# projecthorus/radiosonde_auto_rx

Measured on AMD Instinct MI355X. Metric: IQ Msamples/s (RS41 --IQ --lpIQ demod + framesync + ECC), concurrent real-time 2.4 Msps channels = value/2.4, higher is better.
Workload: dtype f32; 1 GPU; RS41 2.4 Msps cs16 IQ, rs41mod --ecc2 --IQ fq --lpIQ (BASELINE configs[1]) x 512 channels per GPU (per-GPU share of configs[4]), 1 s of signal per channel per step, input resident in HBM; channels_per_gpu=512, frames_decoded=507392, frames_ecc_ok=457842, frames_ecc_failed=49550, frames_repaired=200182, symbols_repaired=1815512

## Files before the change

### include/sonde_hip.h

```cpp
#ifndef SONDE_HIP_H
#define SONDE_HIP_H

#include <stdint.h>
#include <stddef.h>

#ifdef __cplusplus
extern "C" {
#endif

#define SONDE_ABI_VERSION 3

#define SONDE_E_ARG      (-1)
#define SONDE_E_NOGPU    (-2)
#define SONDE_E_NOMEM    (-3)
#define SONDE_E_RANGE    (-4)
#define SONDE_E_OVERFLOW (-5)

#define SONDE_RS41  41
#define SONDE_FRONTEND 0
#define SONDE_DFM09  9
#define SONDE_M10    10
#define SONDE_M20    20

#define SONDE_RD94RD41 94
#define SONDE_LMS6   6
#define SONDE_RS92   92
#define SONDE_IMET54 54
#define SONDE_MIXED  100
#define SONDE_GENERIC 99

#define SONDE_IN_IQ    0
#define SONDE_IN_AUDIO 1
#define SONDE_IN_IFIQ0 2
#define SONDE_IN_IFIQ2 3
#define SONDE_IN_IFIQ3 4

#define SONDE_LP_IQ 1
#define SONDE_LP_FM 2

#define SONDE_TAP_DECIM 0
#define SONDE_TAP_IFIQ  1
#define SONDE_TAP_FM    2
#define SONDE_TAP_BUFS  3
#define SONDE_TAP_CORR  4

typedef struct sonde_engine sonde_engine_t;

typedef struct {
    int32_t abi_version;
    int32_t device;
    int32_t n_channels;
    int32_t sample_rate;
    int32_t bits;
    int32_t sonde_type;
    int32_t opt_lp;
    int32_t opt_dc;
    int32_t opt_min;
    int32_t lpiq_bw;
    int32_t ecc_level;
    float   thres;
    int32_t max_chunk;
    int32_t max_frames;
    int32_t keep_soft;
    int32_t pipeline;
    int32_t input;
    int32_t audio_channels;
    int32_t audio_select;
    int32_t if_rate;
    int32_t opt_iqdc;
    int32_t opt_inv;
    int32_t opt_nolut;
    int32_t m10_noskip;
    int32_t opt_auto;
    int32_t if_tune;
} sonde_cfg_t;

typedef struct {
    int32_t  channel;
    int32_t  len;
    int32_t  ecc;
    uint32_t mv_pos;
    float    mv;
    int32_t  nbytes;
    uint8_t  frame[518];
    uint8_t  pad[2];
} sonde_frame_t;

typedef struct {
    int32_t  channel;
    int32_t  frame_in_hit;
    int32_t  ecc[3];
    uint32_t mv_pos;
    float    mv;
    uint8_t  conf[7], dat1[13], dat2[13];
    uint8_t  pad[3];
    float    frm_count;
    int32_t  inv;
    uint8_t  rawbits[35];
    uint8_t  pad2;
} sonde_dfm_frame_t;

typedef struct {
    int32_t if_sr, decM, dectaps, lut_len, lpiq_taps, lpfm_taps;
    int32_t L, M, K, N, delay;
    float   sps;
    int32_t ring_len;
    int32_t reserved[3];
} sonde_info_t;

int  sonde_engine_create(const sonde_cfg_t *cfg, const double *fq, sonde_engine_t **out);
typedef struct {
    char    header[68];
    float   baud, bt, h;
    int32_t symlen, symhd;
    int32_t hdmax, bitofs;
    int32_t nbits, skip_bits;
    float   l_win;
    int32_t lpiq_bw, lpfm_bw;
    float   slice_baud;
    int32_t reserved[3];
} sonde_generic_t;
int  sonde_engine_create_generic(const sonde_cfg_t *cfg, const double *fq, const sonde_generic_t *gen, sonde_engine_t **out);
typedef struct {
    int32_t sonde_type;
    int32_t ecc_level;
    int32_t lpiq_bw, opt_inv, opt_auto, m10_noskip;
    float   thres;
    int32_t reserved;
} sonde_group_t;
int  sonde_engine_create_mixed(const sonde_cfg_t *cfg, const double *fq, const sonde_group_t *groups, int32_t n_groups, const int32_t *group_of_channel, sonde_engine_t **out);
int  sonde_engine_group_info(const sonde_engine_t *e, int32_t channel, int32_t *sonde_type, sonde_info_t *info);
void sonde_engine_destroy(sonde_engine_t *e);
int  sonde_engine_info(const sonde_engine_t *e, sonde_info_t *info);

int  sonde_engine_process_device(sonde_engine_t *e, const void *d_iq, int64_t ch_stride, int32_t n_samples);
int  sonde_engine_process_host(sonde_engine_t *e, const void *h_iq, int64_t ch_stride, int32_t n_samples);
int64_t sonde_engine_samples_to_dc_boundary(const sonde_engine_t *e);
int  sonde_engine_sync(sonde_engine_t *e);

typedef struct {
    uint32_t channel_id;
    uint8_t  type;
    uint8_t  inverted;
    uint16_t reserved;
    float    score;
    float    freq_offset_hz;
    uint64_t sample_pos;
    uint32_t frames;
    uint32_t frames_clean;
} sonde_summary_t;
int  sonde_engine_set_summary(sonde_engine_t *e, void *d_summary, uint32_t channel_base);
int  sonde_engine_set_summary_snapshots(sonde_engine_t *e, void *d_snap);

int  sonde_engine_fetch_frames(sonde_engine_t *e, sonde_frame_t *out, int32_t max);
int  sonde_engine_overflowed(sonde_engine_t *e);
long long sonde_engine_host_ecc_frames(sonde_engine_t *e);
int  sonde_engine_set_device_ecc(sonde_engine_t *e, int32_t on);
int  sonde_engine_set_search_rounds(sonde_engine_t *e, int32_t on);
int  sonde_engine_count_windows(sonde_engine_t *e, int32_t on, int64_t *out);
int  sonde_engine_tail_residency(sonde_engine_t *e, int32_t *out);
int  sonde_engine_read_sync_state(sonde_engine_t *e, uint32_t *out, int32_t max_channels);
int  sonde_engine_fetch_frames_lagged(sonde_engine_t *e, sonde_frame_t *out, int32_t max, int32_t lag);

typedef struct {
    int32_t  channel;
    int32_t  nbits;
    uint32_t mv_pos;
    float    mv;
} sonde_hit_t;
int  sonde_engine_fetch_hits(sonde_engine_t *e, sonde_hit_t *out, int32_t max, int32_t finish);
int  sonde_engine_set_sync(sonde_engine_t *e, int32_t hdmax, int32_t bitofs);
int  sonde_engine_fetch_soft1(sonde_engine_t *e, float *soft, int32_t max_frames);
int  sonde_engine_set_threshold(sonde_engine_t *e, float thres);

int  sonde_engine_fetch_dfm(sonde_engine_t *e, sonde_dfm_frame_t *out, int32_t max, int32_t finish);
int  sonde_engine_fetch_dfm_lagged(sonde_engine_t *e, sonde_dfm_frame_t *out, int32_t max, int32_t lag);
typedef struct {
    int32_t  channel;
    int32_t  nbits;
    int32_t  len;
    int32_t  cs_ok;
    uint32_t cs_calc;
    uint32_t mv_pos;
    float    mv;
    uint8_t  frame[124];
} sonde_m10_frame_t;
int  sonde_engine_fetch_m10(sonde_engine_t *e, sonde_m10_frame_t *out, int32_t max, int32_t finish);
int  sonde_engine_fetch_m10_lagged(sonde_engine_t *e, sonde_m10_frame_t *out, int32_t max, int32_t lag);
int  sonde_engine_set_m10_chk3(sonde_engine_t *e, int32_t on);
#define SONDE_M10_COLOR 0x100
int  sonde_m10_rawline(const sonde_m10_frame_t *f, int verbose, char *buf, size_t buflen);

typedef struct {
    int32_t  channel;
    int32_t  nbits;
    int32_t  len;
    int32_t  cs_ok;
    uint32_t cs_calc;
    int32_t  blk_ok;
    int32_t  fw;
    uint32_t mv_pos;
    float    mv;
    uint8_t  frame[172];
} sonde_m20_frame_t;
int  sonde_engine_fetch_m20(sonde_engine_t *e, sonde_m20_frame_t *out, int32_t max, int32_t finish);
int  sonde_m10_frame_finish(sonde_m10_frame_t *f);
int  sonde_m20_frame_finish(sonde_m20_frame_t *f);
#define SONDE_M20_COLOR 0x100
int  sonde_m20_rawline(const sonde_m20_frame_t *f, int verbose, char *buf, size_t buflen);

int  sonde_dfm_rawline(const sonde_dfm_frame_t *f, int ecc_level, char *buf, size_t buflen);

int  sonde_engine_finish(sonde_engine_t *e, sonde_frame_t *out, int32_t max);
int  sonde_engine_finish_channel(sonde_engine_t *e, int32_t channel);
int  sonde_engine_tune_channel(sonde_engine_t *e, int32_t channel, double fq);
int  sonde_engine_restart_channel(sonde_engine_t *e, int32_t channel);
int  sonde_engine_fetch_soft(sonde_engine_t *e, float *soft, int32_t max_frames);

int  sonde_engine_read_tap(sonde_engine_t *e, int32_t channel, int32_t tap, int64_t first, int32_t count, float *out);

void *sonde_engine_stream(sonde_engine_t *e);
int  sonde_engine_profile(sonde_engine_t *e, int enable);
int  sonde_engine_kernel_ms(sonde_engine_t *e, const char *kernel, double *avg_ms, int64_t *launches);

typedef struct sonde_softin sonde_softin_t;
int  sonde_softin_create(int32_t sonde_type, int32_t ecc_level, int32_t invert_stream, int32_t opt_inv, int32_t opt_auto, sonde_softin_t **out);
void sonde_softin_destroy(sonde_softin_t *s);
int  sonde_softin_push(sonde_softin_t *s, const float *soft, int32_t n);
int  sonde_softin_push_bits(sonde_softin_t *s, const uint8_t *bits, int32_t n);
int  sonde_softin_push_frame(sonde_softin_t *s, const uint8_t *bytes, int32_t len, int32_t xorhex);
int  sonde_softin_push_hexline(sonde_softin_t *s, const char *line, int32_t xorhex);
int  sonde_softin_finish(sonde_softin_t *s);
int  sonde_softin_fetch(sonde_softin_t *s, sonde_frame_t *out, int32_t max);
int  sonde_softin_fetch_soft(sonde_softin_t *s, float *soft, int32_t *nbits, int32_t *inv, int32_t max);
int  sonde_softin_fetch_dfm(sonde_softin_t *s, sonde_dfm_frame_t *out, int32_t max);
int  sonde_softin_push_dfm_rawhex(sonde_softin_t *s, const char *text, int32_t n);
int  sonde_softin_fetch_m10(sonde_softin_t *s, sonde_m10_frame_t *out, int32_t max);
int  sonde_softin_fetch_m20(sonde_softin_t *s, sonde_m20_frame_t *out, int32_t max);
int  sonde_softin_set_m10_skip(sonde_softin_t *s, int32_t skip);

int  sonde_rs41_rawline(const sonde_frame_t *f, char *buf, size_t buflen);

int  sonde_rs255_encode(uint8_t cw[255]);
int  sonde_rs255_decode(uint8_t cw[255]);
int  sonde_rs41_ecc_device(uint8_t *frames, const int32_t *flen, int32_t n, int32_t level, int32_t *ecc, int32_t *codes, uint8_t *synd);
int  sonde_crc16(const uint8_t *data, int len);

int  sonde_probe_read_gbps(const void *d_buf, size_t bytes, int32_t reps, double *gbps);

const char *sonde_strerror(int code);

#ifdef __cplusplus
}
#endif
#endif
```

### radiosonde_auto_rx_amd/csrc/sonde_dev.h

```cpp
#ifndef SONDE_DEV_H
#define SONDE_DEV_H
#include <hip/hip_runtime.h>
#include <stdint.h>
#include "../../include/sonde_hip.h"

struct MixDecArgs {
    const int16_t *iq;
    long long ch_stride;
    int n_ch, nblocks;
    int D, Q;
    int G;
    int wgs_per_ch;
    float wtab[64 * 8];
    const double *chan_f0;
    int lut_len;
    uint32_t lut_phase;
    const float2 *dc_avg;
    long long *dc_sums;
    const float2 *ptail_in;
    float2 *ptail_out;
    float2 *y;
    int ring_len;
    uint32_t m0;
    const float *wtab_g;
    int wtab_scaled;
    int DS;
    int phase_f64;
    double nd_base;
    const float2 *etab; int etab_len;
    const float2 *dc_avg_prev;
    int dc_since;
    const uint32_t *epoch_phase;
    const int32_t *dc_since_ch;
    const float2 *dc_seg; int dc_seg_n, dc_seg_off, dc_seg_blocks;
    int2 *bsum; long long bsum_stride;
    const int32_t *in_row;
};
struct ScanEdgeArgs {
    int n_ch, nblocks, D, Q, nseg;
    const float2 *dc_seg; int dc_seg_n, dc_seg_off, dc_seg_blocks;
    const float2 *dc_prev;
    int etab_len; uint32_t e0;
    const double *chan_f0; const float *wtab;
    float2 *corr;
};
extern "C" int  sonde_launch_mix_decimate50r(const MixDecArgs *a, hipStream_t s);
extern "C" void sonde_launch_dc_rows_to_segments(const int2 *bsum, long long bsum_stride, int n_ch, int nblocks, int seg_off, int seg_blocks, float maxcnt,
                                                 long long *seg_sums, long long *dc_sums, float2 *dc_avg, const float2 *dc_prev, float2 *dc_prev_out, float2 *dc_seg, int dc_seg_n, hipStream_t s);
extern "C" void sonde_launch_scan_dc_edges(const ScanEdgeArgs *a, hipStream_t s);
extern "C" void sonde_launch_md_etable64(const double *chan_f0, const float *wtab, int D, int Q, int P, int n_ch, float2 *etab, hipStream_t s);
extern "C" void sonde_launch_dc_segments(const int16_t *iq, long long ch_stride, int n_ch, int n_samples, unsigned dc_cnt0, unsigned dc_max,
                                         long long *seg_sums, long long *dc_sums, float2 *dc_avg, float2 *dc_seg, int dc_seg_n, hipStream_t s);

struct AfcState {
    double Df;
    double dc;
    int locked;
    uint32_t pad;
};

struct MixF32Args {
    const float2 *x; long long ch_stride; int n_ch, n;
    const double *chan_f0; int lut_len; uint32_t lut_phase; int phase_f64; double nd_base;
    const float2 *dc_avg; double *dc_sums;
    float2 *z; uint32_t zmask; uint64_t n0;
    int mix;
    const uint32_t *epoch;
    const float2 *dc_seg; int dc_seg_n; uint32_t dc_seg_off, dc_seg_len;
};
struct DecF32Args {
    const float2 *z; uint32_t zmask; uint64_t n0;
    const float *taps; int T, D, n_ch, nblocks;
    float2 *y; int ring_len; uint32_t m0;
};

struct AfcRotArgs {
    const float2 *y; float2 *yrot; const AfcState *afc; const uint32_t *start;
    int n_ch, ring_len, sr; uint32_t m_end;
};

struct IfArgs {
    const float2 *y; float2 *tap_ifiq; float *fm; float *bufs;
    const AfcState *afc; const uint32_t *start; float *fmraw; const float *w_iq0;
    int n_ch, ring_len, n; uint32_t m0;
    int lpiq_on, lpiq_taps, lpfm_on, lpfm_taps, tone_on, nwin;
    int fm_on;
    const float *w_iq, *w_fm;
    double rho;
    float sps;
    const uint32_t *epoch;
};

struct AudioChainArgs {
    const float *raw; float *fm, *bufs; const float *w;
    int n_ch, ring_len, n, taps; uint32_t m0;
};

struct SyncState {
    uint32_t s_in, k, mv_pos, mode;
    float mv; uint32_t inv;
    uint32_t pad[2];
};

struct WinItem {
    uint32_t pos;
    int32_t  state;
    int32_t  rc;
    float    mv; uint32_t mpos;
    uint32_t pad[3];
};
struct WinPlanArgs {
    const SyncState *state; WinItem *items;
    int n_ch, stride, W, K, L, delay; uint32_t frame_samples, avail;
    const uint32_t *epoch;
    uint32_t *work, *work_count; int round_parity;
};
struct WinFftArgs {
    const float *bufs; WinItem *items; const float2 *Fm, *tws;
    int n_ch, stride, W, K, L, ring_len;
    const uint32_t *work, *work_count; int round_parity;
    unsigned long long *prof;
};

struct CorrArgs {
    const float *bufs; float *corr; const float *match;
    const SyncState *state;
    const uint32_t *start;
    int delay; uint32_t frame_samples;
    uint32_t limit;
    int n_ch, ring_len, n, L; uint32_t m0;
    int ntypes, isps, nsym;
    const float *shapes;
    const int *sym_type;
    const float *sym_sign;
};

struct FrameRec {
    int32_t channel, len, nbytes; uint32_t mv_pos; float mv;
    int32_t ecc, ecc_done;
    uint8_t synd[48];
    uint8_t frame[520];
};

struct SyncArgs {
    const float *bufs, *corr; SyncState *state; FrameRec *frames; unsigned *frame_count; float *soft;
    float *soft1;
    const uint8_t *hdr, *hdr_bytes, *mask, *gf_exp, *gf_log;
    const uint4 *bitwin;
    const uint32_t *bitend;
    int n_ch, ring_len, max_frames; uint32_t avail;
    int K, L, delay, hdrlen, symhd, symlen, hdmax, bitofs, nbits; uint32_t frame_samples;
    float sps, thres, l_win;
    int rs41;
    int ecc_level;
    uint32_t *ecc_list; unsigned *ecc_count;
    int eof;
    int eof_ch;
    const uint32_t *epoch;
    int opt_auto;
    int opt_dc, opt_iq, lpiq_on, lpfm_taps, N, sr;
    float match_sum;
    const float *fm, *corr2; float2 *ifiq;
    AfcState *afc; uint32_t *start; unsigned *pending;
    sonde_summary_t *summary; uint32_t summary_base; int summary_type; uint64_t summary_epoch;
    const int32_t *summary_map;
    const WinItem *win; int win_W;
    uint32_t corr_limit;
    unsigned long long *prof;
};

struct SearchSyncArgs {
    SyncArgs sync;
    WinFftArgs win;
    unsigned long long *wcount;
};

#define SONDE_MAX_GROUPS 6
extern "C" {
int  sonde_launch_if_chain_multi(const IfArgs *a, int n_groups, hipStream_t s);
int  sonde_launch_sync_plan_multi(const WinPlanArgs *a, int n_groups, hipStream_t s);
int  sonde_launch_sync_window_fft_multi(const WinFftArgs *a, int n_groups, hipStream_t s);
int  sonde_launch_framesync_multi(const SyncArgs *a, int n_groups, hipStream_t s);
int  sonde_launch_mix_decimate(const MixDecArgs *a, hipStream_t s);
void sonde_launch_dc_update(int n_ch, long long *sums, float2 *avg, float maxcnt, hipStream_t s);
void sonde_launch_dc_update_keep(int n_ch, long long *sums, float2 *avg, float2 *avg_prev, float maxcnt, hipStream_t s);
void sonde_launch_publish_u32(const unsigned *src, unsigned *dst_mapped, hipStream_t s);
void sonde_launch_dc_update_pcs(int n_ch, long long *sums, float2 *avg, float2 *avg_prev, uint32_t *cnt, uint32_t *max, uint32_t lim, int32_t *since,
                                uint32_t n_samples, int nblocks, hipStream_t s);
void sonde_launch_md_etable(const double *chan_f0, const float *wtab, int D, int Q, int P, int n_ch, float2 *etab, hipStream_t s);
void sonde_launch_if_chain(const IfArgs *a, hipStream_t s);
void sonde_launch_mix_f32(const MixF32Args *a, hipStream_t s);
void sonde_launch_dc_segments_f32(const float2 *x, long long ch_stride, int n_ch, int n_samples, unsigned dc_cnt0, unsigned dc_max,
                                  double *seg_sums, double *dc_sums, float2 *dc_avg, float2 *dc_seg, int dc_seg_n, hipStream_t s);
void sonde_launch_decimate_f32(const DecF32Args *a, hipStream_t s);
void sonde_launch_dc_update_f64(int n_ch, double *sums, float2 *avg, float maxcnt, hipStream_t s);
void sonde_launch_afc_rotate(const AfcRotArgs *a, hipStream_t s, int n_max);
void sonde_launch_fill_u32(uint32_t *p, uint32_t v, int n, hipStream_t s);
void sonde_launch_audio_chain(const AudioChainArgs *a, hipStream_t s);
void sonde_launch_u8_to_s16(const uint8_t *in, long long in_stride, int16_t *out, long long out_stride, int n_ch, int n_bytes, hipStream_t s);
void sonde_launch_header_corr(const CorrArgs *a, hipStream_t s);
void sonde_launch_sync_plan(const WinPlanArgs *a, hipStream_t s);
void sonde_launch_sync_window_fft(const WinFftArgs *a, hipStream_t s);
void sonde_launch_framesync(const SyncArgs *a, hipStream_t s);
void sonde_launch_search_sync(const SearchSyncArgs *a, hipStream_t s);
int  sonde_if_chain_residency(const IfArgs *a);
int  sonde_search_sync_residency(void);
size_t sonde_if_chain_lds_bytes(int T1, int T2, int nwin, int tone_on, int fm_on, int *overlay);
int  sonde_if_chain_reserve(const IfArgs *a, int device);
}
#endif
```

### radiosonde_auto_rx_amd/csrc/sonde_engine.cpp

```cpp
#include "../../include/sonde_hip.h"
#include "sonde_dev.h"
#include "sonde_host.h"
#include "sonde_scan_dev.h"
#include <algorithm>
#include <cmath>
#include <cstdio>
#include <cstring>
#include <map>
#include <string>
#include <vector>

using namespace sonde;

#define HIPCHK(x) do { hipError_t e_ = (x); if (e_ != hipSuccess) { fprintf(stderr, "libsonde_hip: %s failed: %s\n", #x, hipGetErrorString(e_)); return SONDE_E_NOGPU; } } while (0)

struct KernelStat { double ms = 0; int64_t n = 0; };
struct PendingEvt { hipEvent_t a, b; const char *name; };

struct sonde_engine {
    sonde_cfg_t cfg{};
    sonde_info_t info{};
    hipStream_t stream = nullptr;
    hipStream_t stream_b = nullptr;
    unsigned long long *d_wfprof = nullptr;
    hipStream_t stream_c = nullptr;
    hipStream_t stream_e = nullptr;
    hipEvent_t ev_s = nullptr;
    sonde_dfm_frame_t *d_dfm_out = nullptr; sonde_m10_frame_t *d_m10_out = nullptr; unsigned *d_blk_done = nullptr; char *d_m10_bits = nullptr;
    std::vector<sonde_dfm_frame_t> h_dfm; std::vector<sonde_m10_frame_t> h_m10; bool soft_lazy = false; unsigned soft_lazy_start = 0;
    uint32_t *d_ecc_list = nullptr; unsigned *d_ecc_cnt = nullptr;
    hipEvent_t ev_a[4] = {}, ev_b[4] = {}, ev_if[4] = {};
    unsigned *h_count = nullptr;
    unsigned *h_count_dev = nullptr;
    FrameRec *h_recs = nullptr;
    int64_t call = 0;
    unsigned read_idx = 0;
    bool eof_pending = false;
    Decimator dec; int Q = 0, G = 8, DS = 0; float *d_wtab = nullptr;
    float2 *d_etab = nullptr, *d_dcavg_prev = nullptr; int etab_len = 0; int dc_since = 1 << 20;
    std::vector<float> w_iq, w_fm, match, wtab;
    float sps = 0, sps_design = 0, baud = 0, bt = 0, hmod = 0, thres = 0, l_win = -1;
    int symlen = 1, symhd = 1, hdmax = 0, bitofs = 0, nbits = 0, hdrlen = 0;
    uint32_t frame_samples = 0;
    double rho = 0;
    float *d_Bop = nullptr; double *d_chanf0 = nullptr; int lut_len = 0;
    float2 *d_dcavg = nullptr; long long *d_dcsums = nullptr;
    float2 *d_ptail[2] = { nullptr, nullptr }; int ptail_cur = 0;
    float2 *d_y = nullptr, *d_ifiq = nullptr; float *d_fm = nullptr, *d_bufs = nullptr, *d_corr = nullptr, *d_raw = nullptr;
    float *d_wiq = nullptr, *d_wfm = nullptr, *d_match = nullptr;
    uint32_t corr_limit = 0;
    WinItem *d_win = nullptr; float2 *d_Fm = nullptr, *d_tws = nullptr; int win_W = 0;
    uint32_t *d_work = nullptr, *d_work_count = nullptr; int sync_rounds = 0;
    bool search_rounds = false;
    bool count_windows = false; unsigned long long *d_wcount = nullptr; long long wcount_rounds[2] = { 0, 0 };
    sonde_summary_t *d_summary = nullptr; uint32_t summary_base = 0;
    sonde_summary_t *d_summary_snap = nullptr;
    int corr_types = 0, corr_isps = 0; float *d_shapes = nullptr, *d_symsign = nullptr; int *d_symtype = nullptr;
    SyncState *d_state = nullptr; FrameRec *d_frames = nullptr; unsigned *d_fcount = nullptr; float *d_soft = nullptr, *d_soft1 = nullptr;
    uint4 *d_bitwin = nullptr; uint32_t *d_bitend = nullptr;
    uint8_t *d_consts = nullptr;
    int16_t *d_stage = nullptr; size_t stage_bytes = 0;
    bool ifiq = false;
    int opt_iq = 5; float match_sum = 0.f;
    std::vector<float> w_iq0; float *d_wiq0 = nullptr;
    float2 *d_yrot = nullptr; float *d_fmraw = nullptr, *d_corr2 = nullptr;
    AfcState *d_afc = nullptr; uint32_t *d_start = nullptr; unsigned *d_pending = nullptr, *h_pending = nullptr;
    double *d_dcsums_f = nullptr; float2 *d_zring = nullptr; float *d_taps_f = nullptr; uint32_t zmask = 0;
    hipEvent_t ev_copy = nullptr;
    int16_t *d_conv = nullptr;
    float2 *d_conv32 = nullptr; bool f32_path = false, conv32 = false;
    int ring_len = 0, max_frames = 0;
    uint64_t samples_in = 0;
    uint32_t m_out = 0;
    uint32_t dc_cnt = 0, dc_max = 0, dc_lim = 0;
    bool pcs = false; std::vector<uint32_t> pcs_cnt, pcs_max; uint32_t dc_max0 = 0;
    uint32_t *d_epoch_phase = nullptr, *d_pcs_cnt = nullptr, *d_pcs_max = nullptr; int32_t *d_pcs_since = nullptr;
    std::vector<float> last_soft, last_soft1; int last_n = 0;
    std::vector<uint8_t> last_frame;
    std::vector<char> m10_bits;
    bool overflow = false;
    bool in_call = false, ecc_listed = false;
    bool dev_ecc = true;
    long long host_ecc_frames = 0;
    bool m10_chk3 = false;
    std::vector<uint32_t> epoch; uint32_t *d_epoch = nullptr; int eof_ch = -1;
    bool prof = false, prof_skip = false; int prof_level = 2; std::map<std::string, KernelStat> stats; std::vector<PendingEvt> pend;
    std::vector<sonde_engine *> groups; std::vector<int32_t> grp_of_ch, row_of_ch; std::vector<std::vector<int32_t>> ch_of_grp; int32_t *d_in_row = nullptr;
    bool front_only = false; int64_t snap_calls = 0;
    sonde_engine *front = nullptr; int front_row = 0; int32_t *d_sum_map = nullptr; bool is_group = false;
    bool merged = false, borrowed_b = false;
};
struct CreateLink { bool is_group, front_only; int min_ring; hipStream_t shared_b; };

template <class T> static int dalloc(T **p, size_t n, bool zero = true) {
    HIPCHK(hipMalloc((void **)p, n * sizeof(T)));
    if (zero) HIPCHK(hipMemset(*p, 0, n * sizeof(T)));
    return 0;
}

static void prof_begin(sonde_engine *e, const char *name, hipStream_t s) {
    if (!e->prof || (e->prof_level == 1 && strcmp(name, "mix_decimate") != 0)) { e->prof_skip = true; return; }
    e->prof_skip = false;
    PendingEvt p; p.name = name;
    hipEventCreate(&p.a); hipEventCreate(&p.b);
    hipEventRecord(p.a, s);
    e->pend.push_back(p);
}
static void prof_end(sonde_engine *e, hipStream_t s) { if (e->prof && !e->prof_skip) hipEventRecord(e->pend.back().b, s); }
static void prof_collect(sonde_engine *e) {
    for (auto &p : e->pend) {
        float ms = 0; hipEventSynchronize(p.b); hipEventElapsedTime(&ms, p.a, p.b);
        auto &s = e->stats[p.name]; s.ms += ms; s.n += 1;
        hipEventDestroy(p.a); hipEventDestroy(p.b);
    }
    e->pend.clear();
}

static int collect_records(sonde_engine *e, int lag, std::vector<FrameRec> &recs, std::vector<float> *soft, int max_take) {
    unsigned count = 0;
    if (lag > 0) {
        const int64_t target = e->call - 1 - lag;
        if (target < 0) { recs.clear(); if (soft) soft->clear(); return 0; }
        if (hipEventSynchronize(e->ev_b[target & 3]) != hipSuccess) return SONDE_E_NOGPU;
        count = e->h_count[target & 3];
    } else {
        if (hipStreamSynchronize(e->stream_b) != hipSuccess) return SONDE_E_NOGPU;
        if (e->stream_e && hipStreamSynchronize(e->stream_e) != hipSuccess) return SONDE_E_NOGPU;
        if (e->call > 0 && !e->eof_pending) count = e->h_count[(e->call - 1) & 3];
        else if (hipMemcpy(&count, e->d_fcount, sizeof count, hipMemcpyDeviceToHost) != hipSuccess) return SONDE_E_NOGPU;
        e->eof_pending = false;
        prof_collect(e);
    }
    if ((int32_t)(count - e->read_idx) < 0) count = e->read_idx;
    hipStream_t cs = (lag > 0 && e->stream_c) ? e->stream_c : e->stream_b;
    unsigned n = count - e->read_idx;
    if (n > (unsigned)e->max_frames) { e->overflow = true; e->read_idx = count - (unsigned)e->max_frames; n = (unsigned)e->max_frames; }
    if (max_take >= 0 && n > (unsigned)max_take) n = (unsigned)max_take;
    recs.resize(n);
    if (soft) soft->resize((size_t)n * e->nbits);
    unsigned done = 0;
    while (done < n) {
        const unsigned idx = (e->read_idx + done) % (unsigned)e->max_frames;
        const unsigned run = std::min<unsigned>(n - done, (unsigned)e->max_frames - idx);
        if (hipMemcpyAsync(e->h_recs + done, e->d_frames + idx, (size_t)run * sizeof(FrameRec), hipMemcpyDeviceToHost, cs) != hipSuccess) return SONDE_E_NOGPU;
        if (soft && e->d_soft && hipMemcpyAsync(soft->data() + (size_t)done * e->nbits, e->d_soft + (size_t)idx * e->nbits,
                                                (size_t)run * e->nbits * sizeof(float), hipMemcpyDeviceToHost, cs) != hipSuccess) return SONDE_E_NOGPU;
        done += run;
    }
    if (n && hipStreamSynchronize(cs) != hipSuccess) return SONDE_E_NOGPU;
    if (n) memcpy(recs.data(), e->h_recs, (size_t)n * sizeof(FrameRec));
    e->read_idx += n;
    return (int)n;
}

static void launch_framesync_impl(sonde_engine *e, int eof);
static SyncArgs fill_sync(sonde_engine *e, int eof);
static void fill_round(sonde_engine *e, int W, WinPlanArgs &p, WinFftArgs &f);
static inline uint32_t rel_pos(const sonde_engine *e, const FrameRec &r) { return e->epoch.empty() ? r.mv_pos : r.mv_pos - e->epoch[r.channel]; }
extern "C" void sonde_launch_dfm_hits(const FrameRec *frames, const float *soft, int nbits, int max_frames, const unsigned *fcount, unsigned *done, sonde_dfm_frame_t *out,
                                      int ecc_level, int grid, hipStream_t s);
extern "C" void sonde_launch_m10_hits(const FrameRec *frames, const float *soft, const float *soft1, int chk3, int nbits, int max_frames, const unsigned *fcount, unsigned *done,
                                      char *chan_bits, sonde_m10_frame_t *out, int grid, hipStream_t s);
static bool blockcodes_on_device(const sonde_engine *e);
static void launch_blockcodes(sonde_engine *e) {
    if (!blockcodes_on_device(e)) return;
    const int grid = std::max(1, std::min(e->cfg.n_channels, 1024));
    if (e->cfg.sonde_type == SONDE_DFM09)
        sonde_launch_dfm_hits(e->d_frames, e->d_soft, e->nbits, e->max_frames, e->d_fcount, e->d_blk_done, e->d_dfm_out, e->cfg.ecc_level, grid, e->stream_b);
    else
        sonde_launch_m10_hits(e->d_frames, e->d_soft, e->d_soft1, e->m10_chk3 ? 1 : 0, e->nbits, e->max_frames, e->d_fcount, e->d_blk_done, e->d_m10_bits, e->d_m10_out, grid, e->stream_b);
}
static void launch_framesync(sonde_engine *e, int eof) { launch_framesync_impl(e, eof); launch_blockcodes(e); if (eof) e->eof_pending = true; }
static void sync_round(sonde_engine *e, int W);
static void launch_search_sync(sonde_engine *e);

static bool blockcodes_on_device(const sonde_engine *e) {
    return e->dev_ecc && e->d_soft && e->d_blk_done && ((e->cfg.sonde_type == SONDE_DFM09 && e->d_dfm_out) || (e->cfg.sonde_type == SONDE_M10 && e->d_m10_out));
}
template <class T> static int copy_decoded(sonde_engine *e, const T *d_out, std::vector<T> &h, unsigned start, int n, int per, int lag = 0) {
    h.resize((size_t)n * per);
    hipStream_t cs = (lag > 0 && e->stream_c) ? e->stream_c : e->stream_b;
    unsigned done = 0;
    while (done < (unsigned)n) {
        const unsigned idx = (start + done) % (unsigned)e->max_frames;
        const unsigned run = std::min<unsigned>((unsigned)n - done, (unsigned)e->max_frames - idx);
        if (hipMemcpyAsync(h.data() + (size_t)done * per, d_out + (size_t)idx * per, (size_t)run * per * sizeof(T), hipMemcpyDeviceToHost, cs) != hipSuccess) return SONDE_E_NOGPU;
        done += run;
    }
    if (n && hipStreamSynchronize(cs) != hipSuccess) return SONDE_E_NOGPU;
    return 0;
}

template <class F, class FN> static int mixed_fetch(sonde_engine *e, int type, F *out, int32_t max, int lag, FN fn) {
    if (!e || !out || max < 0) return SONDE_E_ARG;
    if (lag > 0 && e->snap_calls > 0) {
        const int64_t target = e->call - 1 - lag;
        if (target >= 0 && target < e->snap_calls && hipEventSynchronize(e->ev_b[target & 3]) != hipSuccess) return SONDE_E_NOGPU;
    }
    int n = 0;
    for (size_t gi = 0; gi < e->groups.size(); gi++) {
        sonde_engine *g = e->groups[gi];
        if (g->cfg.sonde_type != type) continue;
        const int k = fn(g, out + n, max - n);
        if (k < 0) return k;
        for (int i = 0; i < k; i++) out[n + i].channel = e->ch_of_grp[gi][(size_t)out[n + i].channel];
        n += k;
    }
    return n;
}

extern "C" {

const char *sonde_strerror(int code) {
    switch (code) {
        case 0: return "ok";
        case SONDE_E_ARG: return "bad argument or unsupported option";
        case SONDE_E_NOGPU: return "HIP device/runtime error";
        case SONDE_E_NOMEM: return "out of memory";
        case SONDE_E_RANGE: return "chunk size out of range or not a multiple of the decimation";
        case SONDE_E_OVERFLOW: return "frame queue overflow";
        default: return "unknown error";
    }
}

extern "C" void sonde_launch_rs41_ecc_frames(FrameRec *frames, const uint32_t *list, unsigned *count, unsigned *done, int max_frames, int level,
                                             const uint8_t *gf_exp, const uint8_t *gf_log, int grid, hipStream_t s);
extern "C" void sonde_launch_rs41_ecc_batch(uint8_t *frames, const int32_t *flen, int n, int level, int32_t *ecc, int32_t *codes, uint8_t *synd,
                                            const uint8_t *gf_exp, const uint8_t *gf_log, hipStream_t s);

int sonde_rs41_ecc_device(uint8_t *frames, const int32_t *flen, int32_t n, int32_t level, int32_t *ecc, int32_t *codes, uint8_t *synd) {
    if (!frames || !flen || !ecc || n < 0 || level < 1 || level > 2) return SONDE_E_ARG;
    if (n == 0) return 0;
    for (int i = 0; i < n; i++) if (flen[i] < 0 || flen[i] > 518) return SONDE_E_ARG;
    uint8_t *d_fr = nullptr, *d_syn = nullptr, *d_gf = nullptr; int32_t *d_len = nullptr, *d_ecc = nullptr, *d_codes = nullptr;
    int rc = 0;
    auto ok = [&](hipError_t e) { if (e != hipSuccess && rc == 0) { fprintf(stderr, "libsonde_hip: sonde_rs41_ecc_device: %s\n", hipGetErrorString(e)); rc = SONDE_E_NOGPU; } return rc == 0; };
    if (ok(hipMalloc((void **)&d_fr, (size_t)n * 518)) && ok(hipMalloc((void **)&d_syn, (size_t)n * 48)) && ok(hipMalloc((void **)&d_gf, 768))
        && ok(hipMalloc((void **)&d_len, (size_t)n * 4)) && ok(hipMalloc((void **)&d_ecc, (size_t)n * 4)) && ok(hipMalloc((void **)&d_codes, (size_t)n * 8))
        && ok(hipMemcpy(d_fr, frames, (size_t)n * 518, hipMemcpyHostToDevice)) && ok(hipMemcpy(d_len, flen, (size_t)n * 4, hipMemcpyHostToDevice))
        && ok(hipMemcpy(d_gf, gf_exp_table(), 512, hipMemcpyHostToDevice)) && ok(hipMemcpy(d_gf + 512, gf_log_table(), 256, hipMemcpyHostToDevice))) {
        sonde_launch_rs41_ecc_batch(d_fr, d_len, n, level, d_ecc, d_codes, d_syn, d_gf, d_gf + 512, nullptr);
        ok(hipGetLastError());
        ok(hipMemcpy(frames, d_fr, (size_t)n * 518, hipMemcpyDeviceToHost));
        ok(hipMemcpy(ecc, d_ecc, (size_t)n * 4, hipMemcpyDeviceToHost));
        if (codes) ok(hipMemcpy(codes, d_codes, (size_t)n * 8, hipMemcpyDeviceToHost));
        if (synd) ok(hipMemcpy(synd, d_syn, (size_t)n * 48, hipMemcpyDeviceToHost));
    }
    hipFree(d_fr); hipFree(d_syn); hipFree(d_gf); hipFree(d_len); hipFree(d_ecc); hipFree(d_codes);
    return rc;
}

int sonde_engine_create(const sonde_cfg_t *cfg, const double *fq, sonde_engine_t **out) { return sonde_engine_create_generic(cfg, fq, nullptr, out); }

static int create_impl(const sonde_cfg_t *cfg, const double *fq, const sonde_generic_t *gen, const CreateLink *lk, sonde_engine_t **out);
static int fetch_dfm_impl(sonde_engine_t *e, sonde_dfm_frame_t *out, int32_t max, int32_t finish, int lag);
static int fetch_m10_impl(sonde_engine_t *e, sonde_m10_frame_t *out, int32_t max, int32_t finish, int lag);
int sonde_engine_create_generic(const sonde_cfg_t *cfg, const double *fq, const sonde_generic_t *gen, sonde_engine_t **out) { return create_impl(cfg, fq, gen, nullptr, out); }

}

static IfArgs fill_if(sonde_engine *e, int n_if, uint32_t m_first);
static int create_impl(const sonde_cfg_t *cfg, const double *fq, const sonde_generic_t *gen, const CreateLink *lk, sonde_engine_t **out) {
    if (!cfg || !fq || !out || cfg->abi_version != SONDE_ABI_VERSION) return SONDE_E_ARG;
    if (cfg->sonde_type == SONDE_GENERIC && !gen) return SONDE_E_ARG;
    float baud_override = 0.f;
    if (gen && cfg->sonde_type != SONDE_GENERIC) { if (!(gen->baud > 0.f)) return SONDE_E_ARG; baud_override = gen->baud; gen = nullptr; }
    if (gen) {
        const size_t hl = strnlen(gen->header, sizeof gen->header);
        if (hl < 8 || hl > 64 || !(gen->baud > 0.f) || !(gen->bt > 0.f) || !(gen->h > 0.f) || gen->symlen < 1 || gen->symlen > 2 || gen->symhd < 1 || gen->symhd > gen->symlen ||
            hl % gen->symhd || gen->hdmax < 0 || gen->bitofs < -8 || gen->bitofs > 64 || gen->nbits < 1 || gen->nbits > 8192 || gen->skip_bits < 0 || gen->slice_baud < 0.f) return SONDE_E_ARG;
    }
    if (cfg->n_channels < 1 || cfg->sample_rate < 1 || (cfg->bits != 16 && cfg->bits != 8 && cfg->bits != 32)) return SONDE_E_ARG;
    sonde_cfg_t cfg_own = *cfg;
    if (cfg->input == SONDE_IN_IQ && cfg->opt_dc && cfg->sonde_type != SONDE_FRONTEND) cfg_own.opt_lp |= SONDE_LP_FM;
    cfg = &cfg_own;
    if ((cfg->sonde_type != SONDE_RS41 && cfg->sonde_type != SONDE_DFM09 && cfg->sonde_type != SONDE_M10 && cfg->sonde_type != SONDE_M20 && cfg->sonde_type != SONDE_FRONTEND && cfg->sonde_type != SONDE_GENERIC) ) return SONDE_E_ARG;
    if (cfg->opt_dc && cfg->sonde_type == SONDE_FRONTEND) return SONDE_E_ARG;
    if (cfg->opt_nolut && (cfg->opt_dc || cfg->input != SONDE_IN_IQ)) return SONDE_E_ARG;
    if (cfg->if_tune && (cfg->input < SONDE_IN_IFIQ0 || cfg->bits != 32 || cfg->opt_dc)) return SONDE_E_ARG;
    if (cfg->sonde_type == SONDE_FRONTEND && cfg->input != SONDE_IN_IQ) return SONDE_E_ARG;
    if (cfg->input < SONDE_IN_IQ || cfg->input > SONDE_IN_IFIQ3) return SONDE_E_ARG;
    int ndev = 0;
    if (hipGetDeviceCount(&ndev) != hipSuccess || ndev < 1 || cfg->device >= ndev) {
        fprintf(stderr, "libsonde_hip: no usable HIP device (the engine has no CPU fallback)\n");
        return SONDE_E_NOGPU;
    }
    HIPCHK(hipSetDevice(cfg->device));
    sonde_engine *e = new sonde_engine();
    e->cfg = *cfg;
    const int C = cfg->n_channels;
    const bool is_group = lk && lk->is_group, front_only = lk && lk->front_only;
    e->is_group = is_group; e->front_only = front_only;

    std::string header;
    int lpiq_def, lpfm_bw;
    int skip_last = -1;
    if (gen) {
        e->baud = gen->baud; e->bt = gen->bt; e->hmod = gen->h; e->symlen = gen->symlen; e->symhd = gen->symhd; e->hdmax = gen->hdmax; e->bitofs = gen->bitofs;
        e->nbits = gen->nbits; e->l_win = gen->l_win > 0.f ? gen->l_win : -1.0f; e->thres = cfg->thres > 0 ? cfg->thres : 0.7f;
        header = std::string(gen->header, strnlen(gen->header, sizeof gen->header)); lpiq_def = gen->lpiq_bw; lpfm_bw = gen->lpfm_bw;
        if (gen->skip_bits > gen->nbits) skip_last = gen->skip_bits - 1;
    } else if (cfg->sonde_type == SONDE_RS41 || cfg->sonde_type == SONDE_FRONTEND) {
        e->baud = 4800.f; e->bt = 0.5f; e->hmod = 0.6f; e->symlen = 1; e->symhd = 1; e->hdmax = 4; e->bitofs = 2;
        e->nbits = 510 * 8; e->l_win = 2.0f; e->thres = cfg->thres > 0 ? cfg->thres : 0.7f;
        header = kRs41Header; lpiq_def = 7400; lpfm_bw = 6000;
    } else if (cfg->sonde_type == SONDE_M10) {
        e->baud = 9615.f; e->bt = 1.8f; e->hmod = 0.9f; e->symlen = 2; e->symhd = 1; e->hdmax = 2; e->bitofs = 0;
        e->nbits = (101 + 20) * 8; e->l_win = 4.0f; e->thres = cfg->thres > 0 ? cfg->thres : 0.76f;
        header = kM10RawHeader; lpiq_def = 24000; lpfm_bw = 10000;
    } else if (cfg->sonde_type == SONDE_M20) {
        e->baud = 9600.f; e->bt = 1.8f; e->hmod = 0.9f; e->symlen = 2; e->symhd = 1; e->hdmax = 2; e->bitofs = 0;
        e->nbits = (101 + 64) * 8; e->l_win = 4.0f; e->thres = cfg->thres > 0 ? cfg->thres : 0.76f;
        header = kM10RawHeader; lpiq_def = 24000; lpfm_bw = 10000;
    } else {
        e->baud = 2500.f; e->bt = 0.5f; e->hmod = 1.8f; e->symlen = 2; e->symhd = 2; e->hdmax = 2; e->bitofs = 2;
        e->nbits = 264 + 7 * 280; e->l_win = 4.0f; e->thres = cfg->thres > 0 ? cfg->thres : 0.65f;
        header = kDfmRawHeader; lpiq_def = 12000; lpfm_bw = 4000;
    }
    if (baud_override > 0.f) e->baud = baud_override;
    e->hdrlen = (int)header.size();
    const int lpiq_bw = cfg->lpiq_bw > 0 ? cfg->lpiq_bw : lpiq_def;

    const bool audio = cfg->input == SONDE_IN_AUDIO;
    const bool ifiq = cfg->input >= SONDE_IN_IFIQ0;
    if (audio) { e->dec.if_sr = cfg->sample_rate; e->dec.decM = 1; e->l_win = -1.0f; }
    else if (ifiq) { e->dec.if_sr = cfg->sample_rate; e->dec.decM = 1; if (cfg->input != SONDE_IN_IFIQ3) e->l_win = -1.0f; }
    else if (cfg->sonde_type == SONDE_FRONTEND) e->dec = design_decimator_if(cfg->sample_rate, cfg->if_rate > 0 ? cfg->if_rate : 48000, cfg->opt_min != 0);
    else e->dec = design_decimator(cfg->sample_rate, cfg->opt_min != 0);
    const int D = e->dec.decM, sr = e->dec.if_sr;
    if (D == 1) e->dec.taps.assign(1, 1.0f);
    const int T = (int)e->dec.taps.size();
    e->sps = (float)cfg->sample_rate / e->baud;
    e->sps /= (float)D;
    e->Q = (T + D - 1) / D;
    const bool wide = e->Q > 8;
    if (D > 1024 || (wide && (audio || ifiq || lk || cfg->input != SONDE_IN_IQ))) { delete e; return SONDE_E_ARG; }
    e->f32_path = cfg->bits == 32 || wide; e->conv32 = wide && cfg->bits != 32;
    if ((cfg->opt_lp & SONDE_LP_IQ) && !audio) {
        float f_lp = (float)(24e3 / (float)sr / 2.0);
        if (lpiq_bw) f_lp = (float)(lpiq_bw / (float)sr / 2.0);
        int taps = (int)(4 * sr / 4e3); if (taps % 2 == 0) taps++;
        e->w_iq = design_lowpass(f_lp, taps);
        if (cfg->opt_dc) e->w_iq0 = design_lowpass((float)(1.5 * f_lp), taps);
    }
    if (cfg->opt_lp & SONDE_LP_FM) {
        float f_lp = (float)(10e3 / (float)sr);
        if (lpfm_bw > 0) f_lp = lpfm_bw / (float)sr;
        int taps = (int)(4 * sr / 2e3); if (taps % 2 == 0) taps++;
        e->w_fm = design_lowpass(f_lp, taps);
    }
    e->match = design_match(header, e->sps, e->bt);
    const int L = (int)e->match.size();
    int M = 3 * L, p2 = 1;
    const int delay = L / 16;
    while (p2 < M) p2 <<= 1;
    while (p2 < 0x2000) p2 <<= 1;
    M = p2;
    const int K = M - L - delay;
    { const float nh = -e->hmod; const float hs = nh * sr; const double f1 = hs / (2.0 * e->sps); e->rho = -f1 / (double)sr; }
    e->sps_design = e->sps;
    if (gen && gen->slice_baud > 0.f) {
        e->sps = (float)sr / gen->slice_baud;
    }
    {
        const int last = skip_last >= 0 ? skip_last : ((cfg->sonde_type == SONDE_M10 || cfg->sonde_type == SONDE_M20) && !cfg->m10_noskip) ? 5 * 808 - 1 : e->nbits - 1;
        uint32_t q0, q1; double mid; bit_window(last, e->symlen - 1, e->symlen, e->sps, q0, q1, mid); e->frame_samples = q1;
    }

    if (!audio && !front_only) {
        const IfArgs ia = fill_if(e, 0, 0);
        const int rc = sonde_if_chain_reserve(&ia, cfg->device);
        if (rc) { delete e; return rc == -1 ? SONDE_E_ARG : SONDE_E_NOGPU; }
    }

    const int max_if = (cfg->max_chunk + D - 1) / D;
    int ring = 1; while (ring < max_if + (int)e->frame_samples + 2 * M + 4096 || ring < 4 * M || (cfg->pipeline && ring < 2 * max_if + 4096)) ring <<= 1;
    if (lk && ring < lk->min_ring) ring = lk->min_ring;
    e->ring_len = ring;
    e->max_frames = cfg->max_frames > 0 ? cfg->max_frames : 4 * C;

    sonde_info_t &I = e->info;
    I.if_sr = sr; I.decM = D; I.dectaps = (D == 1) ? 0 : T; I.lpiq_taps = (int)e->w_iq.size(); I.lpfm_taps = (int)e->w_fm.size();
    I.L = L; I.M = M; I.K = K; I.N = M; I.delay = delay; I.sps = e->sps_design; I.ring_len = ring;

    if (wide) e->wtab.assign((size_t)std::max(64, D) * 8, 0.f);
    else {
        const int pad = e->Q * D - T;
        std::vector<float> wpad((size_t)e->Q * D, 0.f);
        for (int k = 0; k < T; k++) wpad[pad + k] = e->dec.taps[k];
        e->wtab.assign((size_t)std::max(64, D) * 8, 0.f);
        for (int r = 0; r < D; r++) for (int q = 0; q < e->Q; q++) e->wtab[(size_t)r * 8 + q] = wpad[(size_t)D * q + r];
        if (D > 64) {
            for (int k = 64; k >= 4; k--) if (D % k == 0) { e->DS = k; break; }
            if (!e->DS || e->Q < 5) { delete e; return SONDE_E_ARG; }
        }
        {
            std::vector<float> both(e->wtab);
            if (D <= 64) for (size_t i = 0; i < e->wtab.size(); i++) both.push_back(e->wtab[i] * 3.0517578125e-05f);
            if (dalloc(&e->d_wtab, both.size(), false)) { delete e; return SONDE_E_NOMEM; }
            HIPCHK(hipMemcpy(e->d_wtab, both.data(), both.size() * sizeof(float), hipMemcpyHostToDevice));
        }
    }
    {
        std::vector<double> f0s(C);
        for (int c = 0; c < C; c++) {
            const Mixer m = design_mixer(-std::max(-0.5, std::min(0.5, fq[c])), cfg->sample_rate);
            f0s[c] = m.f0; e->lut_len = m.lut_len;
            if (cfg->opt_nolut || cfg->if_tune) f0s[c] = -std::max(-0.5, std::min(0.5, fq[c]));
        }
        I.lut_len = e->lut_len;
        if (dalloc(&e->d_chanf0, (size_t)C, false)) { delete e; return SONDE_E_NOMEM; }
        HIPCHK(hipMemcpy(e->d_chanf0, f0s.data(), f0s.size() * sizeof(double), hipMemcpyHostToDevice));
    }
    if (D == 50 && e->Q == 7 && !audio && cfg->bits != 32 && cfg->sonde_type != SONDE_FRONTEND && !cfg->opt_nolut && e->lut_len % D == 0
        && cfg->input == SONDE_IN_IQ && !is_group) {
        e->etab_len = e->lut_len / D;
        if (dalloc(&e->d_etab, (size_t)C * e->etab_len, false) || dalloc(&e->d_dcavg_prev, C)) { sonde_engine_destroy(e); return SONDE_E_NOMEM; }
        sonde_launch_md_etable(e->d_chanf0, e->d_wtab, D, e->Q, e->etab_len, C, e->d_etab, nullptr);
        HIPCHK(hipDeviceSynchronize());
    }
    int bad = 0;
    bad |= dalloc(&e->d_dcavg, C); bad |= dalloc(&e->d_dcsums, 2 * (size_t)C);
    bad |= dalloc(&e->d_ptail[0], (size_t)C * 64); bad |= dalloc(&e->d_ptail[1], (size_t)C * 64);
    if (audio) bad |= dalloc(&e->d_raw, (size_t)C * ring);
    else { if (!is_group) bad |= dalloc(&e->d_y, (size_t)C * ring); if (!front_only) bad |= dalloc(&e->d_ifiq, (size_t)C * ring); }
    if (!front_only) { bad |= dalloc(&e->d_fm, (size_t)C * ring); bad |= dalloc(&e->d_bufs, (size_t)C * ring); bad |= dalloc(&e->d_corr, (size_t)C * ring); }
    bad |= dalloc(&e->d_state, C); bad |= dalloc(&e->d_frames, e->max_frames); bad |= dalloc(&e->d_fcount, 1 + 4);
    if (cfg->keep_soft || cfg->sonde_type != SONDE_RS41) bad |= dalloc(&e->d_soft, (size_t)e->max_frames * e->nbits);
    if (cfg->keep_soft == 2) bad |= dalloc(&e->d_soft1, (size_t)e->max_frames * e->nbits);
    if (cfg->sonde_type == SONDE_DFM09) { bad |= dalloc(&e->d_dfm_out, (size_t)e->max_frames * 8); bad |= dalloc(&e->d_blk_done, 2); }
    if (cfg->sonde_type == SONDE_M10) { bad |= dalloc(&e->d_m10_out, (size_t)e->max_frames); bad |= dalloc(&e->d_blk_done, 2); bad |= dalloc(&e->d_m10_bits, (size_t)C * ((101 + 20) * 8 + 8)); }
    bad |= dalloc(&e->d_match, L, false);
    if (!e->w_iq.empty()) bad |= dalloc(&e->d_wiq, e->w_iq.size(), false);
    if (!e->w_fm.empty()) bad |= dalloc(&e->d_wfm, e->w_fm.size(), false);
    bad |= dalloc(&e->d_consts, 1024, true);
    if (bad) { sonde_engine_destroy(e); return SONDE_E_NOMEM; }
    HIPCHK(hipMemcpy(e->d_match, e->match.data(), L * sizeof(float), hipMemcpyHostToDevice));
    e->dev_ecc = getenv("SONDE_HOST_ECC") == nullptr;
    {
        if (!cfg->opt_dc && M == 8192 && K + L <= M) {
            std::vector<float> m(2 * (size_t)M, 0.f);
            for (int i = 0; i < L; i++) m[2 * (size_t)(L - 1 - i)] = e->match[i];
            ref_dft_8192(m);
            const std::vector<float> tw = ref_twiddle_table();
            e->win_W = 8;
            m.resize(4 * (size_t)M);
            for (int i = 0; i < M; i++) {
                int r = 0; for (int b = 0; b < 13; b++) if (i >> b & 1) r |= 1 << (12 - b);
                m[2 * (size_t)(M + i)] = m[2 * (size_t)r]; m[2 * (size_t)(M + i) + 1] = m[2 * (size_t)r + 1];
            }
            if (dalloc(&e->d_Fm, 2 * (size_t)M, false) || dalloc(&e->d_tws, tw.size() / 2, false) || dalloc(&e->d_win, (size_t)C * e->win_W) ||
                dalloc(&e->d_work, (size_t)C * e->win_W) || dalloc(&e->d_work_count, 2)) { sonde_engine_destroy(e); return SONDE_E_NOMEM; }
            HIPCHK(hipMemcpy(e->d_Fm, m.data(), m.size() * sizeof(float), hipMemcpyHostToDevice));
            HIPCHK(hipMemcpy(e->d_tws, tw.data(), tw.size() * sizeof(float), hipMemcpyHostToDevice));
        }
    }
    if (e->d_wiq) HIPCHK(hipMemcpy(e->d_wiq, e->w_iq.data(), e->w_iq.size() * sizeof(float), hipMemcpyHostToDevice));
    if (e->d_wfm) HIPCHK(hipMemcpy(e->d_wfm, e->w_fm.data(), e->w_fm.size() * sizeof(float), hipMemcpyHostToDevice));
    {
        uint8_t cb[1024]; memset(cb, 0, sizeof cb);
        memcpy(cb, header.data(), header.size()); memcpy(cb + 64, kRs41HeaderBytes, 8); memcpy(cb + 72, kRs41Mask, 64);
        memcpy(cb + 136, gf_exp_table(), 512); memcpy(cb + 648, gf_log_table(), 256);
        HIPCHK(hipMemcpy(e->d_consts, cb, sizeof cb, hipMemcpyHostToDevice));
    }
    {
        const int isps = (int)e->sps_design, nsym = e->hdrlen / e->symhd;
        if ((float)isps == e->sps_design && e->symhd == 1 && isps * nsym == L && isps >= 2 && isps <= 16 && isps % 2 == 0) {
            std::vector<float> shapes; std::vector<int> type(nsym); std::vector<float> sign(nsym);
            std::vector<int> key;
            bool ok = true;
            for (int k = 0; k < nsym && ok; k++) {
                const int b = (header[k] & 1) ? 1 : -1;
                const int l = (k > 0) ? ((header[k - 1] & 1) ? 1 : -1) * b : 0;
                const int r = (k < nsym - 1) ? ((header[k + 1] & 1) ? 1 : -1) * b : 0;
                const int ky = (l + 1) * 3 + (r + 1);
                int t = -1;
                for (size_t q = 0; q < key.size(); q++) if (key[q] == ky) t = (int)q;
                if (t < 0) {
                    t = (int)key.size(); key.push_back(ky);
                    for (int d = 0; d < isps; d++) shapes.push_back((float)b * e->match[(size_t)isps * k + d]);
                } else {
                    for (int d = 0; d < isps; d++) ok &= (shapes[(size_t)t * isps + d] == (float)b * e->match[(size_t)isps * k + d]);
                }
                type[k] = t; sign[k] = (float)b;
            }
            if (ok && key.size() <= 9) {
                e->corr_types = (int)key.size(); e->corr_isps = isps;
                bad = 0;
                bad |= dalloc(&e->d_shapes, shapes.size(), false); bad |= dalloc(&e->d_symtype, nsym, false); bad |= dalloc(&e->d_symsign, nsym, false);
                if (bad) { sonde_engine_destroy(e); return SONDE_E_NOMEM; }
                HIPCHK(hipMemcpy(e->d_shapes, shapes.data(), shapes.size() * sizeof(float), hipMemcpyHostToDevice));
                HIPCHK(hipMemcpy(e->d_symtype, type.data(), nsym * sizeof(int), hipMemcpyHostToDevice));
                HIPCHK(hipMemcpy(e->d_symsign, sign.data(), nsym * sizeof(float), hipMemcpyHostToDevice));
            }
        }
    }
    {
        std::vector<uint32_t> win((size_t)e->nbits * 4), end(e->nbits);
        for (int bp = 0; bp < e->nbits; bp++) {
            uint32_t q0, q1, qa, qb; double mid;
            if (e->symlen == 2) { bit_window(bp, 0, 2, e->sps, q0, q1, mid); slice_range(q0, q1, mid, e->l_win, qa, qb); }
            else { qa = qb = 0; }
            win[4 * bp] = qa; win[4 * bp + 1] = qb;
            bit_window(bp, e->symlen - 1, e->symlen, e->sps, q0, q1, mid);
            slice_range(q0, q1, mid, e->l_win, qa, qb);
            win[4 * bp + 2] = qa; win[4 * bp + 3] = qb; end[bp] = q1;
        }
        bad = 0;
        bad |= dalloc(&e->d_bitwin, (size_t)e->nbits, false); bad |= dalloc(&e->d_bitend, (size_t)e->nbits, false);
        if (bad) { sonde_engine_destroy(e); return SONDE_E_NOMEM; }
        HIPCHK(hipMemcpy(e->d_bitwin, win.data(), win.size() * sizeof(uint32_t), hipMemcpyHostToDevice));
        HIPCHK(hipMemcpy(e->d_bitend, end.data(), end.size() * sizeof(uint32_t), hipMemcpyHostToDevice));
    }
    e->dc_lim = (uint32_t)sr; e->dc_max = e->dc_lim / 32;
    if (D > 1) { e->dc_lim *= D; e->dc_max *= D; }
    if (e->dc_max == 0 || e->dc_max % D) { sonde_engine_destroy(e); return SONDE_E_ARG; }
    e->dc_max0 = e->dc_max;
    e->ifiq = ifiq;
    if (e->f32_path) {
        bad = dalloc(&e->d_dcsums_f, 2 * (size_t)C);
        if (e->conv32) bad |= dalloc(&e->d_conv32, (size_t)C * (size_t)cfg->max_chunk, false);
        if (!audio && !ifiq) {
            uint32_t zl = 1; while (zl < (uint32_t)cfg->max_chunk + (uint32_t)T + (uint32_t)D + 64u) zl <<= 1;
            e->zmask = zl - 1;
            bad |= dalloc(&e->d_zring, (size_t)C * zl); bad |= dalloc(&e->d_taps_f, (size_t)T, false);
            if (!bad) HIPCHK(hipMemcpy(e->d_taps_f, e->dec.taps.data(), (size_t)T * sizeof(float), hipMemcpyHostToDevice));
        }
        if (bad) { sonde_engine_destroy(e); return SONDE_E_NOMEM; }
    }
    if (cfg->opt_inv) {
        std::vector<SyncState> st0(C); for (auto &q : st0) { memset(&q, 0, sizeof q); q.inv = 1; }
        HIPCHK(hipMemcpy(e->d_state, st0.data(), st0.size() * sizeof(SyncState), hipMemcpyHostToDevice));
    }
    e->opt_iq = audio ? 0 : ifiq ? (cfg->input == SONDE_IN_IFIQ0 ? 1 : cfg->input == SONDE_IN_IFIQ2 ? 2 : 3) : 5;
    { double sm = 0.0; for (float v : e->match) sm += (double)v; e->match_sum = (float)sm; }
    if (cfg->opt_dc) {
        bad = 0;
        bad |= dalloc(&e->d_afc, C); bad |= dalloc(&e->d_start, C); bad |= dalloc(&e->d_pending, 1);
        if (!audio) { bad |= dalloc(&e->d_yrot, (size_t)C * ring); bad |= dalloc(&e->d_fmraw, (size_t)C * ring); }
        if (e->opt_iq >= 2) bad |= dalloc(&e->d_corr2, (size_t)C * ring);
        if (!e->w_iq0.empty()) bad |= dalloc(&e->d_wiq0, e->w_iq0.size(), false);
        if (bad) { sonde_engine_destroy(e); return SONDE_E_NOMEM; }
        if (e->d_wiq0) HIPCHK(hipMemcpy(e->d_wiq0, e->w_iq0.data(), e->w_iq0.size() * sizeof(float), hipMemcpyHostToDevice));
        HIPCHK(hipHostMalloc((void **)&e->h_pending, sizeof(unsigned), hipHostMallocDefault));
    }
    e->last_frame.assign((size_t)C * 518, 0);
    for (int c = 0; c < C; c++) memcpy(e->last_frame.data() + (size_t)c * 518, kRs41HeaderBytes, 8);
    HIPCHK(hipStreamCreateWithFlags(&e->stream, hipStreamNonBlocking));
    if (cfg->pipeline && audio) { sonde_engine_destroy(e); return SONDE_E_ARG; }
    if (lk && lk->shared_b) { e->stream_b = lk->shared_b; e->borrowed_b = is_group; }
    else if (cfg->pipeline) {
        int lo = 0, hi = 0;
        if (hipDeviceGetStreamPriorityRange(&lo, &hi) == hipSuccess && hi != lo)
            HIPCHK(hipStreamCreateWithPriority(&e->stream_b, hipStreamNonBlocking, hi));
        else HIPCHK(hipStreamCreateWithFlags(&e->stream_b, hipStreamNonBlocking));
    }
    else e->stream_b = e->stream;
    HIPCHK(hipStreamCreateWithFlags(&e->stream_c, hipStreamNonBlocking));
    if (cfg->sonde_type == SONDE_RS41 && cfg->ecc_level >= 1 && cfg->ecc_level <= 2 && getenv("SONDE_ECC_INLINE") == nullptr) {
        int lo = 0, hi = 0;
        if (hipDeviceGetStreamPriorityRange(&lo, &hi) == hipSuccess && hi != lo) HIPCHK(hipStreamCreateWithPriority(&e->stream_e, hipStreamNonBlocking, hi));
        else HIPCHK(hipStreamCreateWithFlags(&e->stream_e, hipStreamNonBlocking));
    }
    HIPCHK(hipEventCreateWithFlags(&e->ev_s, hipEventDisableTiming));
    if (cfg->sonde_type == SONDE_RS41) {
        HIPCHK(hipMalloc((void **)&e->d_ecc_list, 2 * (size_t)e->max_frames * sizeof(uint32_t)));
        HIPCHK(hipMalloc((void **)&e->d_ecc_cnt, 4 * sizeof(unsigned)));
        HIPCHK(hipMemset(e->d_ecc_cnt, 0, 4 * sizeof(unsigned)));
    }
    for (int i = 0; i < 4; i++) { HIPCHK(hipEventCreateWithFlags(&e->ev_a[i], hipEventDisableTiming)); HIPCHK(hipEventCreateWithFlags(&e->ev_b[i], hipEventDisableTiming)); HIPCHK(hipEventCreateWithFlags(&e->ev_if[i], hipEventDisableTiming)); }
    HIPCHK(hipEventCreateWithFlags(&e->ev_copy, hipEventDisableTiming));
    HIPCHK(hipHostMalloc((void **)&e->h_count, 4 * sizeof(unsigned), hipHostMallocMapped));
    memset(e->h_count, 0, 4 * sizeof(unsigned));
    HIPCHK(hipHostGetDevicePointer((void **)&e->h_count_dev, e->h_count, 0));
    HIPCHK(hipHostMalloc((void **)&e->h_recs, (size_t)e->max_frames * sizeof(FrameRec), hipHostMallocDefault));
    *out = e;
    return 0;
}

extern "C" {

void sonde_engine_destroy(sonde_engine_t *e) {
    if (!e) return;
    for (sonde_engine *g : e->groups) sonde_engine_destroy(g);
    e->groups.clear();
    if (e->is_group) e->d_y = nullptr;
    if (e->stream) hipStreamSynchronize(e->stream);
    if (e->stream_b) hipStreamSynchronize(e->stream_b);
    if (e->stream_e) hipStreamSynchronize(e->stream_e);
    prof_collect(e);
    if (e->d_wfprof) {
        unsigned long long h[32] = {0};
        if (hipMemcpy(h, e->d_wfprof, sizeof h, hipMemcpyDeviceToHost) == hipSuccess && h[31]) {
            static const char *nm[7] = {"setup", "search", "headcmp", "slot", "slice", "syndromes+record", "exit"};
            unsigned long long tot = 0; for (int i = 0; i < 7; i++) tot += h[16 + i];
            fprintf(stderr, "framesync prof (channel 0, %llu launches, %llu frames, %.0f cycles per launch):", h[31], h[30], (double)tot / (double)h[31]);
            for (int i = 0; i < 7; i++) fprintf(stderr, " %s %.1f%%", nm[i], 100.0 * (double)h[16 + i] / (double)std::max(1ull, tot));
            fprintf(stderr, "\n");
        }
        if (h[15]) {
            static const char *nm[6] = {"load", "fft1", "mul", "fft2", "argmax", "norm"};
            unsigned long long tot = 0; for (int i = 0; i < 6; i++) tot += h[i];
            fprintf(stderr, "window fft prof (workgroup 0, %llu windows, %.0f cycles each):", h[15], (double)tot / (double)h[15]);
            for (int i = 0; i < 6; i++) fprintf(stderr, " %s %.1f%%", nm[i], 100.0 * (double)h[i] / (double)std::max(1ull, tot));
            fprintf(stderr, "\n");
        }
        hipFree(e->d_wfprof);
    }
    { hipStream_t sa = e->stream; if (sa) hipStreamDestroy(sa); }
    if (e->stream_b && e->stream_b != e->stream && !e->borrowed_b) hipStreamDestroy(e->stream_b);
    if (e->stream_c) hipStreamDestroy(e->stream_c);
    if (e->stream_e) hipStreamDestroy(e->stream_e);
    if (e->ev_s) hipEventDestroy(e->ev_s);
    hipFree(e->d_dfm_out); hipFree(e->d_m10_out); hipFree(e->d_blk_done); hipFree(e->d_m10_bits);
    hipFree(e->d_ecc_list); hipFree(e->d_ecc_cnt);
    for (int i = 0; i < 4; i++) { if (e->ev_a[i]) hipEventDestroy(e->ev_a[i]); if (e->ev_b[i]) hipEventDestroy(e->ev_b[i]); if (e->ev_if[i]) hipEventDestroy(e->ev_if[i]); }
    if (e->ev_copy) hipEventDestroy(e->ev_copy);
    if (e->h_pending) hipHostFree(e->h_pending);
    if (e->h_count) hipHostFree(e->h_count);
    if (e->h_recs) hipHostFree(e->h_recs);
    void *ptrs[] = { e->d_Bop, e->d_chanf0, e->d_dcavg, e->d_dcsums, e->d_ptail[0], e->d_ptail[1], e->d_y, e->d_ifiq, e->d_fm,
                     e->d_bufs, e->d_corr, e->d_wiq, e->d_wfm, e->d_match, e->d_state, e->d_frames, e->d_fcount, e->d_soft, e->d_soft1,
                     e->d_epoch, e->d_work, e->d_work_count, e->d_consts, e->d_stage, e->d_shapes, e->d_symtype, e->d_symsign, e->d_bitwin, e->d_bitend, e->d_raw, e->d_wtab, e->d_conv, e->d_conv32,
                     e->d_dcsums_f, e->d_zring, e->d_taps_f, e->d_wiq0, e->d_yrot, e->d_fmraw, e->d_corr2, e->d_afc, e->d_start, e->d_pending,
                     e->d_etab, e->d_dcavg_prev, e->d_win, e->d_Fm, e->d_tws, e->d_epoch_phase, e->d_pcs_cnt, e->d_pcs_max, e->d_pcs_since, e->d_in_row, e->d_sum_map, e->d_wcount };
    for (void *p : ptrs) if (p) hipFree(p);
    delete e;
}

int sonde_engine_info(const sonde_engine_t *e, sonde_info_t *info) {
    if (!e || !info) return SONDE_E_ARG;
    *info = e->info;
    return 0;
}

static uint32_t pcs_room(const sonde_engine *e) {
    uint32_t r = 0xffffffffu;
    for (size_t c = 0; c < e->pcs_cnt.size(); c++) r = std::min(r, e->pcs_max[c] - e->pcs_cnt[c]);
    return r;
}
int64_t sonde_engine_samples_to_dc_boundary(const sonde_engine_t *e) {
    if (!e) return SONDE_E_ARG;
    return e->pcs ? (int64_t)pcs_room(e) : (int64_t)(e->dc_max - e->dc_cnt);
}

void *sonde_engine_stream(sonde_engine_t *e) { return e ? (void *)e->stream : nullptr; }

}

static void tail_begin(sonde_engine *t, hipStream_t fs) {
    t->in_call = true; t->ecc_listed = false;
    if (t->stream_e && t->call >= 2) hipStreamWaitEvent(t->stream_b, t->ev_b[(t->call - 2) & 3], 0);
    if (t->d_ecc_cnt) { hipMemsetAsync(t->d_ecc_cnt + (t->call & 1), 0, sizeof(unsigned), t->stream_b); hipMemsetAsync(t->d_ecc_cnt + 2 + (t->call & 1), 0, sizeof(unsigned), t->stream_b); }
    if (t->stream_b != fs && t->call >= 2) hipStreamWaitEvent(fs, t->ev_if[(t->call - 2) & 3], 0);
}
static int tail_enqueue(sonde_engine *e, int32_t n_samples, uint32_t m_first, hipStream_t fs, hipEvent_t front_done);
static int tail_enqueue_merged(sonde_engine *e, int32_t n_samples, uint32_t m_first);
static int tail_finish(sonde_engine *e);
static int sync_rounds_of(const sonde_engine *e, int n_if);
static IfArgs fill_if(sonde_engine *e, int n_if, uint32_t m_first);

extern "C" {

int sonde_engine_process_device(sonde_engine_t *e, const void *d_iq, int64_t ch_stride, int32_t n_samples) {
    if (!e || !d_iq || e->is_group) return SONDE_E_ARG;
    const int D = e->info.decM, C = e->cfg.n_channels;
    if (n_samples <= 0 || n_samples > e->cfg.max_chunk || n_samples % D || (ch_stride != 0 && ch_stride < n_samples)) return SONDE_E_RANGE;
    if (e->cfg.bits == 8) {
        const int epf = e->cfg.input == SONDE_IN_AUDIO ? std::max(1, e->cfg.audio_channels) : 2;
        if (!e->d_conv) HIPCHK(hipMalloc((void **)&e->d_conv, (size_t)C * e->cfg.max_chunk * epf * 2));
        sonde_launch_u8_to_s16((const uint8_t *)d_iq, ch_stride * epf, e->d_conv, (long long)n_samples * epf, ch_stride == 0 ? 1 : C, n_samples * epf, e->stream);
        d_iq = e->d_conv; if (ch_stride != 0) ch_stride = n_samples;
    }
    const uint32_t m_first = e->m_out;
    int done = 0;
    const bool mixed = !e->groups.empty();
    if (mixed) { for (sonde_engine *g : e->groups) tail_begin(g, e->stream); }
    else tail_begin(e, e->stream);
    if (e->cfg.input == SONDE_IN_AUDIO) {
        AudioConvArgs c0{}; c0.pcm = (const int16_t *)d_iq; c0.ch_stride = ch_stride; c0.n_ch = C; c0.n = n_samples;
        c0.nch = std::max(1, e->cfg.audio_channels); c0.sel = std::min(std::max(0, e->cfg.audio_select), c0.nch - 1);
        c0.fm = e->d_raw; c0.ring_len = e->ring_len; c0.m0 = e->m_out; c0.f32 = (e->cfg.bits == 32);
        sonde_launch_audio_convert(&c0, e->stream);
        AudioChainArgs c1{}; c1.raw = e->d_raw; c1.fm = e->d_fm; c1.bufs = e->d_bufs; c1.w = e->d_wfm; c1.n_ch = C; c1.ring_len = e->ring_len;
        c1.n = n_samples; c1.taps = (int)e->w_fm.size(); c1.m0 = e->m_out;
        prof_begin(e, "if_chain", e->stream); sonde_launch_audio_chain(&c1, e->stream); prof_end(e, e->stream);
        e->samples_in += (uint64_t)n_samples; e->m_out += (uint32_t)n_samples; done = n_samples;
    }
    if (e->conv32) {
        sonde_launch_s16_to_f32((const int16_t *)d_iq, ch_stride, e->d_conv32, (long long)n_samples, ch_stride == 0 ? 1 : C, n_samples, e->stream);
        d_iq = e->d_conv32; if (ch_stride != 0) ch_stride = n_samples;
    }
    while (done < n_samples && e->f32_path && e->cfg.input != SONDE_IN_AUDIO) {
        const bool dc = !e->ifiq || e->cfg.opt_iqdc != 0;
        const int take = dc ? (int)std::min<uint32_t>((uint32_t)(n_samples - done), e->dc_max - e->dc_cnt) : n_samples - done;
        MixF32Args a{}; a.x = (const float2 *)d_iq + (size_t)done; a.ch_stride = ch_stride; a.n_ch = C; a.n = take;
        a.chan_f0 = e->d_chanf0; a.lut_len = e->lut_len; a.lut_phase = (uint32_t)(e->samples_in % (uint64_t)e->lut_len);
        a.phase_f64 = (e->cfg.sonde_type == SONDE_FRONTEND); a.dc_avg = e->d_dcavg; a.dc_sums = e->d_dcsums_f;
        if (e->cfg.opt_nolut) { a.phase_f64 = 1; a.lut_len = 1 << 30; a.lut_phase = 0; a.nd_base = (double)e->samples_in; }
        if (e->ifiq) {
            a.mix = 0; a.z = e->d_y; a.zmask = (uint32_t)e->ring_len - 1; a.n0 = e->m_out;
            if (e->cfg.if_tune) {
                a.mix = 1; a.phase_f64 = 1; a.lut_len = 1 << 30; a.lut_phase = 0; a.nd_base = (double)e->samples_in; a.epoch = e->d_epoch;
            }
        }
        else { a.mix = 1; a.z = e->d_zring; a.zmask = e->zmask; a.n0 = e->samples_in; }
        prof_begin(e, "mix_decimate", e->stream);
        sonde_launch_mix_f32(&a, e->stream);
        if (!e->ifiq) {
            DecF32Args d{}; d.z = e->d_zring; d.zmask = e->zmask; d.n0 = e->samples_in; d.taps = e->d_taps_f; d.T = (int)e->dec.taps.size(); d.D = D;
            d.n_ch = C; d.nblocks = take / D; d.y = e->d_y; d.ring_len = e->ring_len; d.m0 = e->m_out;
            sonde_launch_decimate_f32(&d, e->stream);
        }
        prof_end(e, e->stream);
        e->samples_in += (uint64_t)take; e->m_out += (uint32_t)(take / D); done += take;
        if (dc) {
            e->dc_cnt += (uint32_t)take;
            if (e->dc_cnt == e->dc_max) {
                sonde_launch_dc_update_f64(C, e->d_dcsums_f, e->d_dcavg, (float)e->dc_max, e->stream);
                e->dc_cnt = 0;
                if (e->dc_max < e->dc_lim) e->dc_max *= 2;
            }
        }
    }
    while (done < n_samples && e->ifiq) {
        const bool dc = e->cfg.opt_iqdc != 0;
        const int take = dc ? (int)std::min<uint32_t>((uint32_t)(n_samples - done), e->dc_max - e->dc_cnt) : n_samples - done;
        IqConvArgs a{}; a.iq = (const int16_t *)d_iq + 2 * (size_t)done; a.ch_stride = ch_stride; a.n_ch = C; a.n = take;
        a.dc_avg = e->d_dcavg; a.dc_sums = e->d_dcsums; a.y = e->d_y; a.ring_len = e->ring_len; a.m0 = e->m_out;
        prof_begin(e, "iq_convert", e->stream); sonde_launch_iq_convert(&a, e->stream); prof_end(e, e->stream);
        e->samples_in += (uint64_t)take; e->m_out += (uint32_t)take; done += take;
        if (dc) {
            e->dc_cnt += (uint32_t)take;
            if (e->dc_cnt == e->dc_max) {
                sonde_launch_dc_update(C, e->d_dcsums, e->d_dcavg, (float)e->dc_max, e->stream);
                e->dc_cnt = 0;
                if (e->dc_max < e->dc_lim) e->dc_max *= 2;
            }
        }
    }
    while (done < n_samples) {
        const int take = (int)std::min<uint32_t>((uint32_t)(n_samples - done), e->pcs ? pcs_room(e) : e->dc_max - e->dc_cnt);
        MixDecArgs a{};
        a.iq = (const int16_t *)d_iq + 2 * (size_t)done; a.ch_stride = ch_stride; a.n_ch = C; a.nblocks = take / D;
        a.D = D; a.Q = e->Q; a.G = e->G;
        memcpy(a.wtab, e->wtab.data(), sizeof a.wtab); a.wtab_g = e->d_wtab; a.DS = e->DS; a.chan_f0 = e->d_chanf0; a.lut_len = e->lut_len;
        a.lut_phase = (uint32_t)(e->samples_in % (uint64_t)e->lut_len);
        a.dc_avg = e->d_dcavg; a.dc_sums = e->d_dcsums;
        a.ptail_in = e->d_ptail[e->ptail_cur]; a.ptail_out = e->d_ptail[e->ptail_cur ^ 1];
        a.y = e->d_y; a.ring_len = e->ring_len; a.m0 = e->m_out;
        a.phase_f64 = (e->cfg.sonde_type == SONDE_FRONTEND);
        if (e->cfg.opt_nolut) { a.phase_f64 = 1; a.lut_len = 1 << 30; a.lut_phase = 0; a.nd_base = (double)e->samples_in; }
        { long long tiles = (long long)C * ((a.nblocks + 63) / 64); int G = (int)(tiles / 12288); a.G = G < 1 ? 1 : (G > 16 ? 16 : G); }
        {
            const char *g = getenv("SONDE_MD_G"); const int gv = g ? atoi(g) : 0; if (gv >= 1 && gv <= 16) a.G = gv;
        }
        a.etab = e->d_etab; a.etab_len = e->etab_len; a.in_row = e->d_in_row;
        a.dc_avg_prev = (e->d_etab && e->dc_since < e->Q - 1) ? e->d_dcavg_prev : nullptr; a.dc_since = e->dc_since;
        if (e->dc_since < (1 << 20)) e->dc_since += take / D;
        if (e->pcs) { a.epoch_phase = e->d_epoch_phase; a.dc_since_ch = e->d_pcs_since; a.dc_avg_prev = e->d_etab ? e->d_dcavg_prev : nullptr; }
        prof_begin(e, "mix_decimate", e->stream); const int lrc = sonde_launch_mix_decimate(&a, e->stream); prof_end(e, e->stream);
        if (lrc < 0) { e->in_call = false; e->ecc_listed = false; for (sonde_engine *g : e->groups) { g->in_call = false; g->ecc_listed = false; } return lrc == -2 ? SONDE_E_NOGPU : SONDE_E_ARG; }
        e->ptail_cur ^= 1;
        e->samples_in += (uint64_t)take; e->m_out += (uint32_t)(take / D); e->dc_cnt += (uint32_t)take; done += take;
        if (e->pcs) {
            sonde_launch_dc_update_pcs(C, e->d_dcsums, e->d_dcavg, e->d_dcavg_prev, e->d_pcs_cnt, e->d_pcs_max, e->dc_lim, e->d_pcs_since, (uint32_t)take, take / D, e->stream);
            for (int c2 = 0; c2 < C; c2++) {
                e->pcs_cnt[c2] += (uint32_t)take;
                if (e->pcs_cnt[c2] >= e->pcs_max[c2]) { e->pcs_cnt[c2] = 0; if (e->pcs_max[c2] < e->dc_lim) e->pcs_max[c2] *= 2; }
            }
            e->dc_cnt = 0;
            continue;
        }
        if (e->dc_cnt == e->dc_max) {
            if (e->d_etab) e->dc_since = 0;
            sonde_launch_dc_update_keep(C, e->d_dcsums, e->d_dcavg, e->d_etab ? e->d_dcavg_prev : nullptr, (float)e->dc_max, e->stream);
            e->dc_cnt = 0;
            if (e->dc_max < e->dc_lim) e->dc_max *= 2;
        }
    }
    const int slot = (int)(e->call & 3);
    int rc = 0;
    if (mixed) {
        hipEventRecord(e->ev_a[slot], e->stream);
        for (sonde_engine *g : e->groups) { g->samples_in = e->samples_in; g->m_out = e->m_out; }
        if (e->merged) rc = tail_enqueue_merged(e, n_samples, m_first);
        else for (sonde_engine *g : e->groups) {
            const int r2 = tail_enqueue(g, n_samples, m_first, e->stream, e->ev_a[slot]);
            if (r2 && !rc) rc = r2;
        }
        if (e->d_summary && e->d_summary_snap) {
            for (sonde_engine *g : e->groups) hipStreamWaitEvent(e->stream_b, g->ev_b[slot], 0);
            hipMemcpyAsync(e->d_summary_snap + (size_t)(e->call & 1) * C, e->d_summary, (size_t)C * sizeof(sonde_summary_t), hipMemcpyDeviceToDevice, e->stream_b);
            hipEventRecord(e->ev_b[slot], e->stream_b);
            e->snap_calls = e->call + 1;
        }
        e->call += 1;
    } else {
        if (e->stream_b != e->stream) hipEventRecord(e->ev_a[slot], e->stream);
        rc = tail_enqueue(e, n_samples, m_first, e->stream, e->ev_a[slot]);
    }
    return rc;
}

}

static IfArgs fill_if(sonde_engine *e, int n_if, uint32_t m_first) {
    IfArgs b{};
    const bool fe = e->cfg.sonde_type == SONDE_FRONTEND;
    b.y = e->d_y; b.tap_ifiq = (e->cfg.keep_soft || fe) ? e->d_ifiq : nullptr; b.fm = e->d_fm; b.bufs = e->d_bufs; b.n_ch = e->cfg.n_channels; b.ring_len = e->ring_len;
    b.n = n_if; b.m0 = m_first;
    b.lpiq_on = !e->w_iq.empty(); b.lpiq_taps = (int)e->w_iq.size(); b.lpfm_on = !e->w_fm.empty(); b.lpfm_taps = (int)e->w_fm.size();
    b.tone_on = (e->cfg.input != SONDE_IN_IFIQ0); b.nwin = (int)e->sps;
    b.fm_on = (e->cfg.keep_soft || fe || !e->w_fm.empty() || !b.tone_on) ? 1 : 0;
    b.w_iq = e->d_wiq; b.w_fm = e->d_wfm; b.rho = e->rho; b.sps = e->sps; b.epoch = e->d_epoch;
    if (e->cfg.opt_dc && e->cfg.input != SONDE_IN_AUDIO) b.fm_on = 1;
    return b;
}
static int tail_enqueue(sonde_engine *e, int32_t n_samples, uint32_t m_first, hipStream_t fs, hipEvent_t front_done) {
    const int D = e->info.decM, C = e->cfg.n_channels;
    const int n_if = n_samples / D;
    const bool fe = e->cfg.sonde_type == SONDE_FRONTEND;
    IfArgs b = fill_if(e, n_if, m_first);
    const int slot = (int)(e->call & 3);
    if (e->stream_b != fs) hipStreamWaitEvent(e->stream_b, front_done, 0);
    CorrArgs c{};
    c.bufs = e->d_bufs; c.corr = e->d_corr; c.match = e->d_match; c.n_ch = C; c.ring_len = e->ring_len; c.n = n_if; c.L = e->info.L; c.m0 = m_first;
    c.state = e->d_state; c.delay = e->info.delay; c.frame_samples = e->frame_samples;
    c.ntypes = e->corr_types; c.isps = e->corr_isps; c.nsym = e->hdrlen / e->symhd; c.shapes = e->d_shapes; c.sym_type = e->d_symtype; c.sym_sign = e->d_symsign;
    if (e->cfg.opt_dc && e->cfg.input != SONDE_IN_AUDIO) {
        hipStream_t sb = e->stream_b;
        sonde_launch_fill_u32(e->d_start, m_first, C, sb);
        b.y = e->d_yrot; b.tap_ifiq = e->d_ifiq; b.afc = e->d_afc; b.start = e->d_start; b.fmraw = e->d_fmraw; b.w_iq0 = e->d_wiq0;
        c.start = e->d_start;
        AfcRotArgs r{}; r.y = e->d_y; r.yrot = e->d_yrot; r.afc = e->d_afc; r.start = e->d_start; r.n_ch = C; r.ring_len = e->ring_len;
        r.sr = e->info.if_sr; r.m_end = e->m_out;
        for (int it = 0; it < n_if / std::max(1, e->info.K - 4) + 4; it++) {
            hipMemsetAsync(e->d_pending, 0, sizeof(unsigned), sb);
            sonde_launch_afc_rotate(&r, sb, n_if);
            prof_begin(e, "if_chain", sb); sonde_launch_if_chain(&b, sb); prof_end(e, sb);
            prof_begin(e, "header_corr", sb); sonde_launch_header_corr(&c, sb); prof_end(e, sb);
            if (e->opt_iq >= 2) { CorrArgs c2 = c; c2.bufs = e->d_fm; c2.corr = e->d_corr2; sonde_launch_header_corr(&c2, sb); }
            launch_framesync(e, 0);
            hipMemcpyAsync(e->h_pending, e->d_pending, sizeof(unsigned), hipMemcpyDeviceToHost, sb);
            HIPCHK(hipStreamSynchronize(sb));
            if (*e->h_pending == 0) break;
        }
        if (e->stream_b != fs) hipEventRecord(e->ev_if[slot], e->stream_b);
    } else {
        if (e->cfg.input != SONDE_IN_AUDIO) { prof_begin(e, "if_chain", e->stream_b); sonde_launch_if_chain(&b, e->stream_b); prof_end(e, e->stream_b); }
        if (e->stream_b != fs) hipEventRecord(e->ev_if[slot], e->stream_b);
        if (!fe && e->d_win && !e->search_rounds) {
            launch_search_sync(e);
        } else if (!fe && e->d_win) {
            const int rounds = sync_rounds_of(e, n_if);
            for (int round = 0; round < rounds; round++) {
                sync_round(e, round == 0 ? 2 : e->win_W);
                if (e->count_windows) {
                    uint32_t n = 0;
                    hipMemcpyAsync(&n, e->d_work_count + ((e->sync_rounds - 1) & 1), sizeof n, hipMemcpyDeviceToHost, e->stream_b);
                    hipStreamSynchronize(e->stream_b);
                    e->wcount_rounds[round == 0 ? 0 : 1] += n;
                }
            }
        } else if (!fe) {
            const uint32_t lim = (n_if > 3 * e->info.K) ? (uint32_t)(2 * e->info.K + 64) : 0u;
            if (lim) {
                c.limit = lim; e->corr_limit = lim;
                prof_begin(e, "header_corr", e->stream_b); sonde_launch_header_corr(&c, e->stream_b); prof_end(e, e->stream_b);
                launch_framesync(e, 0);
                c.limit = 0; e->corr_limit = 0;
            }
            prof_begin(e, "header_corr", e->stream_b); sonde_launch_header_corr(&c, e->stream_b); prof_end(e, e->stream_b);
            launch_framesync(e, 0);
        }
    }
    if (e->d_summary && e->d_summary_snap && !e->is_group)
        hipMemcpyAsync(e->d_summary_snap + (size_t)(e->call & 1) * C, e->d_summary, (size_t)C * sizeof(sonde_summary_t), hipMemcpyDeviceToDevice, e->stream_b);
    return tail_finish(e);
}

static int tail_enqueue_merged(sonde_engine *e, int32_t n_samples, uint32_t m_first) {
    const int n_if = n_samples / e->info.decM, G = (int)e->groups.size();
    hipStream_t sb = e->stream_b;
    const int slot = (int)(e->call & 3);
    hipStreamWaitEvent(sb, e->ev_a[slot], 0);
    IfArgs ia[SONDE_MAX_GROUPS]; WinPlanArgs pa[SONDE_MAX_GROUPS]; WinFftArgs fa[SONDE_MAX_GROUPS]; SyncArgs sa[SONDE_MAX_GROUPS];
    for (int g = 0; g < G; g++) ia[g] = fill_if(e->groups[(size_t)g], n_if, m_first);
    prof_begin(e, "if_chain", sb); sonde_launch_if_chain_multi(ia, G, sb); prof_end(e, sb);
    for (sonde_engine *g : e->groups) hipEventRecord(g->ev_if[slot], sb);
    int rounds = 0;
    for (sonde_engine *g : e->groups) rounds = std::max(rounds, sync_rounds_of(g, n_if));
    for (int round = 0; round < rounds; round++) {
        for (int g = 0; g < G; g++) fill_round(e->groups[(size_t)g], round == 0 ? 2 : e->groups[(size_t)g]->win_W, pa[g], fa[g]);
        prof_begin(e, "header_corr", sb);
        sonde_launch_sync_plan_multi(pa, G, sb);
        sonde_launch_sync_window_fft_multi(fa, G, sb);
        prof_end(e, sb);
        for (int g = 0; g < G; g++) sa[g] = fill_sync(e->groups[(size_t)g], 0);
        prof_begin(e, "framesync", sb); sonde_launch_framesync_multi(sa, G, sb); prof_end(e, sb);
        for (sonde_engine *g : e->groups) launch_blockcodes(g);
    }
    int rc = 0;
    for (sonde_engine *g : e->groups) { const int r2 = tail_finish(g); if (r2 && !rc) rc = r2; }
    return rc;
}

static int sync_rounds_of(const sonde_engine *e, int n_if) {
    const int kw = std::max(1, e->info.K - 4);
    return 2 + n_if / (kw + (int)e->frame_samples) + n_if / (e->win_W * kw);
}

static int tail_finish(sonde_engine *e) {
    const int C = e->cfg.n_channels;
    const int slot = (int)(e->call & 3);
    hipStream_t se = e->stream_b;
    hipMemcpyAsync(e->d_fcount + 1 + slot, e->d_fcount, sizeof(unsigned), hipMemcpyDeviceToDevice, e->stream_b);
    if (e->ecc_listed) {
        if (e->stream_e) { hipEventRecord(e->ev_s, e->stream_b); hipStreamWaitEvent(e->stream_e, e->ev_s, 0); se = e->stream_e; }
        const int par = (int)(e->call & 1);
        prof_begin(e, "rs_ecc", se);
        sonde_launch_rs41_ecc_frames(e->d_frames, e->d_ecc_list + (size_t)par * e->max_frames, e->d_ecc_cnt + par, e->d_ecc_cnt + 2 + par, e->max_frames,
                                     e->cfg.ecc_level, e->d_consts + 136, e->d_consts + 648, std::min(512, std::max(1, C)), se);
        prof_end(e, se);
    }
    sonde_launch_publish_u32(e->d_fcount + 1 + slot, e->h_count_dev + slot, se);
    hipEventRecord(e->ev_b[slot], se);
    e->in_call = false;
    e->call += 1;
    if (hipPeekAtLastError() != hipSuccess) { fprintf(stderr, "libsonde_hip: launch failed: %s\n", hipGetErrorString(hipGetLastError())); return SONDE_E_NOGPU; }
    return 0;
}


extern "C" {

static void fill_winfft(sonde_engine *e, WinFftArgs &f) {
    f = WinFftArgs{}; f.bufs = e->d_bufs; f.items = e->d_win; f.Fm = e->d_Fm; f.tws = e->d_tws; f.n_ch = e->cfg.n_channels; f.stride = e->win_W;
    f.K = e->info.K; f.L = e->info.L; f.ring_len = e->ring_len;
    static const bool want_prof = getenv("SONDE_WF_PROF") != nullptr;
    if (want_prof && !e->d_wfprof) { if (hipMalloc((void **)&e->d_wfprof, 32 * sizeof(unsigned long long)) == hipSuccess) hipMemset(e->d_wfprof, 0, 32 * sizeof(unsigned long long)); }
    f.prof = e->d_wfprof;
}
static void fill_round(sonde_engine *e, int W, WinPlanArgs &p, WinFftArgs &f) {
    const int C = e->cfg.n_channels;
    p = WinPlanArgs{}; p.state = e->d_state; p.items = e->d_win; p.n_ch = C; p.stride = e->win_W; p.W = W; p.K = e->info.K; p.L = e->info.L;
    p.delay = e->info.delay; p.frame_samples = e->frame_samples; p.avail = e->m_out; p.epoch = e->d_epoch;
    p.work = e->d_work; p.work_count = e->d_work_count; p.round_parity = e->sync_rounds & 1;
    fill_winfft(e, f); f.W = W;
    f.work = e->d_work; f.work_count = e->d_work_count; f.round_parity = e->sync_rounds & 1;
    e->sync_rounds++;
}
static void sync_round(sonde_engine *e, int W) {
    hipStream_t sb = e->stream_b;
    WinPlanArgs p; WinFftArgs f;
    fill_round(e, W, p, f);
    prof_begin(e, "header_corr", sb);
    sonde_launch_sync_plan(&p, sb);
    sonde_launch_sync_window_fft(&f, sb);
    prof_end(e, sb);
    launch_framesync(e, 0);
}

static SyncArgs fill_sync(sonde_engine *e, int eof) {
    const int C = e->cfg.n_channels;
    SyncArgs s{};
    s.eof = eof; s.eof_ch = e->eof_ch; s.epoch = e->d_epoch; s.rs41 = (e->cfg.sonde_type == SONDE_RS41); s.ecc_level = (s.rs41 && e->dev_ecc && e->cfg.ecc_level >= 1 && e->cfg.ecc_level <= 2) ? e->cfg.ecc_level : 0;
    if (s.ecc_level && !eof && e->in_call && e->d_ecc_list) { s.ecc_list = e->d_ecc_list + (size_t)(e->call & 1) * e->max_frames; s.ecc_count = e->d_ecc_cnt + (e->call & 1); e->ecc_listed = true; }
    s.bufs = e->d_bufs; s.corr = e->d_corr; s.state = e->d_state; s.frames = e->d_frames; s.frame_count = e->d_fcount; s.soft = e->d_soft; s.soft1 = e->d_soft1;
    s.hdr = e->d_consts; s.hdr_bytes = e->d_consts + 64; s.mask = e->d_consts + 72; s.gf_exp = e->d_consts + 136; s.gf_log = e->d_consts + 648;
    s.bitwin = e->d_bitwin; s.bitend = e->d_bitend;
    s.n_ch = C; s.ring_len = e->ring_len; s.max_frames = e->max_frames; s.avail = e->m_out;
    s.K = e->info.K; s.L = e->info.L; s.delay = e->info.delay; s.hdrlen = e->hdrlen; s.symhd = e->symhd; s.symlen = e->symlen;
    s.hdmax = e->hdmax; s.bitofs = e->bitofs; s.nbits = e->nbits; s.frame_samples = e->frame_samples;
    s.sps = e->sps; s.thres = e->thres; s.l_win = e->l_win;
    s.opt_auto = e->cfg.opt_auto != 0 || e->cfg.sonde_type == SONDE_M10 || e->cfg.sonde_type == SONDE_M20;
    s.opt_dc = e->cfg.opt_dc != 0; s.opt_iq = e->opt_iq; s.lpiq_on = !e->w_iq.empty(); s.lpfm_taps = (int)e->w_fm.size(); s.N = e->info.N; s.sr = e->info.if_sr;
    s.match_sum = e->match_sum; s.fm = e->d_fm; s.corr2 = e->d_corr2; s.ifiq = e->d_ifiq; s.afc = e->d_afc; s.start = e->d_start; s.pending = e->d_pending;
    s.corr_limit = e->corr_limit;
    s.win = e->d_win; s.win_W = e->win_W;
    s.prof = e->d_wfprof ? e->d_wfprof + 16 : nullptr;
    s.summary = e->d_summary; s.summary_base = e->summary_base; s.summary_map = e->d_sum_map; s.summary_type = e->cfg.sonde_type; s.summary_epoch = e->samples_in / (uint64_t)std::max(1, e->info.decM);
    return s;
}
static void launch_framesync_impl(sonde_engine *e, int eof) {
    const SyncArgs s = fill_sync(e, eof);
    prof_begin(e, "framesync", e->stream_b); sonde_launch_framesync(&s, e->stream_b); prof_end(e, e->stream_b);
}
static void launch_search_sync(sonde_engine *e) {
    SearchSyncArgs a{};
    a.sync = fill_sync(e, 0); a.sync.win = nullptr; a.sync.win_W = 0;
    fill_winfft(e, a.win);
    a.wcount = e->count_windows ? e->d_wcount : nullptr;
    prof_begin(e, "framesync", e->stream_b); sonde_launch_search_sync(&a, e->stream_b); prof_end(e, e->stream_b);
    launch_blockcodes(e);
}

int sonde_engine_process_host(sonde_engine_t *e, const void *h_iq, int64_t ch_stride, int32_t n_samples) {
    if (!e || !h_iq) return SONDE_E_ARG;
    const int C = e->cfg.n_channels;
    if (n_samples <= 0 || n_samples > e->cfg.max_chunk || (ch_stride != 0 && ch_stride < n_samples)) return SONDE_E_RANGE;
    const size_t unit = (e->cfg.input == SONDE_IN_AUDIO ? (size_t)std::max(1, e->cfg.audio_channels) : 2) * (size_t)(e->cfg.bits / 8);
    const int rows = ch_stride == 0 ? 1 : C;
    const size_t need = (size_t)rows * n_samples * unit;
    if (need > e->stage_bytes) {
        if (e->d_stage) { hipStreamSynchronize(e->stream); hipFree(e->d_stage); e->d_stage = nullptr; }
        HIPCHK(hipMalloc((void **)&e->d_stage, need)); e->stage_bytes = need;
    }
    HIPCHK(hipMemcpy2DAsync(e->d_stage, (size_t)n_samples * unit, h_iq, (size_t)std::max<int64_t>(ch_stride, n_samples) * unit, (size_t)n_samples * unit, rows,
                            hipMemcpyHostToDevice, e->stream));
    HIPCHK(hipEventRecord(e->ev_copy, e->stream));
    HIPCHK(hipEventSynchronize(e->ev_copy));
    return sonde_engine_process_device(e, e->d_stage, ch_stride == 0 ? 0 : n_samples, n_samples);
}

int sonde_engine_sync(sonde_engine_t *e) {
    if (!e) return SONDE_E_ARG;
    for (sonde_engine *g : e->groups) { const int rc = sonde_engine_sync(g); if (rc) return rc; }
    HIPCHK(hipStreamSynchronize(e->stream));
    HIPCHK(hipStreamSynchronize(e->stream_b));
    if (e->stream_e) HIPCHK(hipStreamSynchronize(e->stream_e));
    prof_collect(e);
    return 0;
}

static int fetch_rs41(sonde_engine_t *e, sonde_frame_t *out, int32_t max, int lag) {
    if (!e || !out || max < 0 || e->cfg.sonde_type != SONDE_RS41) return SONDE_E_ARG;
    std::vector<FrameRec> recs;
    const int n = collect_records(e, lag, recs, e->d_soft ? &e->last_soft : nullptr, max);
    if (n < 0) return n;
    for (int i = 0; i < n; i++) {
        const FrameRec &r = recs[i];
        sonde_frame_t &f = out[i];
        memset(&f, 0, sizeof f);
        f.channel = r.channel; f.len = r.len; f.mv = r.mv; f.mv_pos = rel_pos(e, r); f.nbytes = r.nbytes;
        uint8_t *keepf = e->last_frame.data() + (size_t)r.channel * 518;
        if (r.nbytes >= 518) {
            memcpy(f.frame, r.frame, 518);
            f.ecc = 0;
            if (e->cfg.ecc_level > 0) {
                bool clean = true;
                for (int k = 0; k < 48; k++) clean &= (r.synd[k] == 0);
                if (r.ecc_done == 1) f.ecc = r.ecc;
                else if (clean) { for (int k = f.len; k < 518; k++) f.frame[k] = 0; }
                else { f.ecc = rs41_ecc(f.frame, f.len, e->cfg.ecc_level, r.synd); e->host_ecc_frames++; }
            }
        } else {
            memcpy(f.frame, keepf, 518);
            memcpy(f.frame, r.frame, (size_t)r.nbytes);
            if (r.nbytes < 0x93) for (int k = r.nbytes; k < 518; k++) f.frame[k] = 0;
            f.len = (rs41_frametype(f.frame) >= 0) ? 320 : 518;
            f.ecc = e->cfg.ecc_level > 0 ? rs41_ecc(f.frame, f.len, e->cfg.ecc_level, nullptr) : 0;
        }
        memcpy(keepf, f.frame, 518);
    }
    e->last_n = n;
    return n;
}

int sonde_engine_set_summary(sonde_engine_t *e, void *d_summary, uint32_t channel_base) {
    if (!e) return SONDE_E_ARG;
    e->d_summary = (sonde_summary_t *)d_summary; e->summary_base = channel_base;
    for (sonde_engine *g : e->groups) { g->d_summary = e->d_summary; g->summary_base = channel_base; }
    return 0;
}

int sonde_engine_set_summary_snapshots(sonde_engine_t *e, void *d_snap) {
    if (!e) return SONDE_E_ARG;
    e->d_summary_snap = (sonde_summary_t *)d_snap;
    return (int)(e->call & 1);
}

long long sonde_engine_host_ecc_frames(sonde_engine_t *e) {
    if (!e) return SONDE_E_ARG;
    long long n = e->host_ecc_frames;
    for (sonde_engine *g : e->groups) n += g->host_ecc_frames;
    return n;
}
int sonde_engine_set_search_rounds(sonde_engine_t *e, int32_t on) {
    if (!e) return SONDE_E_ARG;
    for (sonde_engine *g : e->groups) { const int rc = sonde_engine_set_search_rounds(g, on); if (rc) return rc; }
    e->search_rounds = on != 0;
    return 0;
}
int sonde_engine_count_windows(sonde_engine_t *e, int32_t on, int64_t *out) {
    if (!e || !e->groups.empty()) return SONDE_E_ARG;
    if (on && !e->d_wcount && e->d_win && dalloc(&e->d_wcount, 1)) return SONDE_E_NOMEM;
    if (hipStreamSynchronize(e->stream_b) != hipSuccess) return SONDE_E_NOGPU;
    e->count_windows = on != 0;
    if (out) {
        unsigned long long n = 0;
        if (e->d_wcount && hipMemcpy(&n, e->d_wcount, sizeof n, hipMemcpyDeviceToHost) != hipSuccess) return SONDE_E_NOGPU;
        out[0] = e->wcount_rounds[0]; out[1] = e->wcount_rounds[1]; out[2] = (int64_t)n;
    }
    return 0;
}
int sonde_engine_tail_residency(sonde_engine_t *e, int32_t *out) {
    if (!e || !out || !e->groups.empty()) return SONDE_E_ARG;
    const IfArgs b = fill_if(e, 0, 0);
    out[0] = e->cfg.input != SONDE_IN_AUDIO ? sonde_if_chain_residency(&b) : 0;
    out[1] = (e->cfg.sonde_type != SONDE_FRONTEND && e->d_win && !e->cfg.opt_dc) ? sonde_search_sync_residency() : 0;
    return (out[0] < 0 || out[1] < 0) ? SONDE_E_NOGPU : 0;
}
int sonde_engine_read_sync_state(sonde_engine_t *e, uint32_t *out, int32_t max_channels) {
    if (!e || !out || !e->groups.empty() || !e->d_state) return SONDE_E_ARG;
    const int n = std::min<int>(max_channels, e->cfg.n_channels);
    if (n <= 0) return 0;
    if (hipStreamSynchronize(e->stream_b) != hipSuccess) return SONDE_E_NOGPU;
    if (hipMemcpy(out, e->d_state, (size_t)n * sizeof(SyncState), hipMemcpyDeviceToHost) != hipSuccess) return SONDE_E_NOGPU;
    return n;
}
int sonde_engine_set_device_ecc(sonde_engine_t *e, int32_t on) {
    if (!e) return SONDE_E_ARG;
    for (sonde_engine *g : e->groups) { const int rc = sonde_engine_set_device_ecc(g, on); if (rc) return rc; }
    if ((on != 0) == e->dev_ecc) return 0;
    if (e->d_blk_done) {
        if (hipStreamSynchronize(e->stream_b) != hipSuccess) return SONDE_E_NOGPU;
        unsigned count = 0;
        if (hipMemcpy(&count, e->d_fcount, sizeof count, hipMemcpyDeviceToHost) != hipSuccess) return SONDE_E_NOGPU;
        if (count != e->read_idx) return SONDE_E_ARG;
        const unsigned dn[2] = { count, 0u };
        if (on && hipMemcpy(e->d_blk_done, dn, sizeof dn, hipMemcpyHostToDevice) != hipSuccess) return SONDE_E_NOGPU;
    }
    e->dev_ecc = on != 0;
    return 0;
}

int sonde_engine_overflowed(sonde_engine_t *e) {
    if (!e) return SONDE_E_ARG;
    bool ovf = e->overflow; e->overflow = false;
    for (sonde_engine *g : e->groups) { ovf |= g->overflow; g->overflow = false; }
    return ovf ? 1 : 0;
}

int sonde_engine_fetch_frames(sonde_engine_t *e, sonde_frame_t *out, int32_t max) { return sonde_engine_fetch_frames_lagged(e, out, max, 0); }

int sonde_engine_fetch_frames_lagged(sonde_engine_t *e, sonde_frame_t *out, int32_t max, int32_t lag) {
    if (lag < 0) lag = 0;
    if (e && !e->groups.empty()) return mixed_fetch(e, SONDE_RS41, out, max, lag, [lag](sonde_engine *g, sonde_frame_t *o, int32_t m) { return fetch_rs41(g, o, m, lag); });
    return fetch_rs41(e, out, max, lag);
}

int sonde_engine_fetch_dfm(sonde_engine_t *e, sonde_dfm_frame_t *out, int32_t max, int32_t finish) {
    if (e && !e->groups.empty()) return mixed_fetch(e, SONDE_DFM09, out, max, 0, [finish](sonde_engine *g, sonde_dfm_frame_t *o, int32_t m) { return fetch_dfm_impl(g, o, m, finish, 0); });
    return fetch_dfm_impl(e, out, max, finish, 0);
}
int sonde_engine_fetch_dfm_lagged(sonde_engine_t *e, sonde_dfm_frame_t *out, int32_t max, int32_t lag) {
    if (lag < 0) lag = 0;
    if (e && !e->groups.empty()) return mixed_fetch(e, SONDE_DFM09, out, max, lag, [lag](sonde_engine *g, sonde_dfm_frame_t *o, int32_t m) { return fetch_dfm_impl(g, o, m, 0, lag); });
    return fetch_dfm_impl(e, out, max, 0, lag);
}
int sonde_engine_fetch_m10(sonde_engine_t *e, sonde_m10_frame_t *out, int32_t max, int32_t finish) {
    if (e && !e->groups.empty()) return mixed_fetch(e, SONDE_M10, out, max, 0, [finish](sonde_engine *g, sonde_m10_frame_t *o, int32_t m) { return fetch_m10_impl(g, o, m, finish, 0); });
    return fetch_m10_impl(e, out, max, finish, 0);
}
int sonde_engine_fetch_m10_lagged(sonde_engine_t *e, sonde_m10_frame_t *out, int32_t max, int32_t lag) {
    if (lag < 0) lag = 0;
    if (e && !e->groups.empty()) return mixed_fetch(e, SONDE_M10, out, max, lag, [lag](sonde_engine *g, sonde_m10_frame_t *o, int32_t m) { return fetch_m10_impl(g, o, m, 0, lag); });
    return fetch_m10_impl(e, out, max, 0, lag);
}

static int fetch_dfm_impl(sonde_engine_t *e, sonde_dfm_frame_t *out, int32_t max, int32_t finish, int lag) {
    if (!e || !out || max < 0 || e->cfg.sonde_type != SONDE_DFM09) return SONDE_E_ARG;
    if (finish) { launch_framesync(e, 1); lag = 0; }
    std::vector<FrameRec> recs;
    std::vector<float> soft;
    const bool on_dev = blockcodes_on_device(e);
    const int nh = collect_records(e, lag, recs, on_dev ? nullptr : &soft, max / 8);
    if (nh < 0) return nh;
    e->last_n = nh;
    if (on_dev) {
        const unsigned start = e->read_idx - (unsigned)nh;
        e->soft_lazy = true; e->soft_lazy_start = start;
        if (copy_decoded(e, e->d_dfm_out, e->h_dfm, start, nh, 8, lag)) return SONDE_E_NOGPU;
        int n = 0;
        for (int h = 0; h < nh; h++) {
            const FrameRec &r = recs[h];
            for (int f = 0; f < 8 && n < max; f++) {
                const sonde_dfm_frame_t &d = e->h_dfm[(size_t)h * 8 + f];
                if (d.frame_in_hit != f) break;
                sonde_dfm_frame_t &o = out[n++];
                o = d;
                o.mv_pos = rel_pos(e, r);
                o.frm_count = (float)(rel_pos(e, r) / (2.0 * e->sps * 280) + f);
            }
        }
        return n;
    }
    e->last_soft = soft; e->soft_lazy = false;
    int n = 0;
    for (int h = 0; h < nh; h++) {
        const FrameRec &r = recs[h];
        const float *sb = soft.data() + (size_t)h * e->nbits;
        for (int f = 0; f < 8 && n < max; f++) {
            const int first = f == 0 ? 0 : 264 + 280 * (f - 1), skip = f == 0 ? 16 : 0;
            if (first + (280 - skip) > r.nbytes) break;
            uint8_t hb[280]; float sf[280];
            memset(hb, 0, sizeof hb); memset(sf, 0, sizeof sf);
            for (int i = skip; i < 280; i++) {
                const int b = first + i - skip;
                hb[i] = (r.frame[b >> 3] >> (b & 7)) & 1; sf[i] = sb[b];
            }
            sonde_dfm_frame_t &o = out[n++];
            memset(&o, 0, sizeof o);
            o.channel = r.channel; o.frame_in_hit = f; o.mv = r.mv; o.mv_pos = rel_pos(e, r);
            o.frm_count = (float)(rel_pos(e, r) / (2.0 * e->sps * 280) + f);
            o.inv = r.mv < 0.f;
            for (int i = 0; i < 280; i++) o.rawbits[i >> 3] |= (uint8_t)(hb[i] << (i & 7));
            o.ecc[0] = dfm_block(e->cfg.ecc_level, hb + 16, sf + 16, 7, o.conf);
            o.ecc[1] = dfm_block(e->cfg.ecc_level, hb + 72, sf + 72, 13, o.dat1);
            o.ecc[2] = dfm_block(e->cfg.ecc_level, hb + 176, sf + 176, 13, o.dat2);
        }
    }
    return n;
}

static int mxx_bytes(sonde_engine *e, const FrameRec &r, int nbytes_max, uint8_t *frame) {
    const int NB = nbytes_max * 8;
    if (e->m10_bits.empty()) e->m10_bits.assign((size_t)e->cfg.n_channels * (NB + 8), 0);
    char *fb = e->m10_bits.data() + (size_t)r.channel * (NB + 8);
    const int nv = std::min(r.nbytes, NB);
    int bit0 = '0';
    for (int p = 0; p < nv; p++) { const int bit = (r.frame[p >> 3] >> (p & 7)) & 1; fb[p] = (char)(0x31 ^ (bit0 ^ bit)); bit0 = bit; }
    fb[nv] = 0;
    for (int i = 0; i < nbytes_max; i++) {
        int v = 0;
        for (int k = 0; k < 8; k++) if (fb[8 * i + 7 - k] == '1') v |= 1 << k;
        frame[i] = (uint8_t)v;
    }
    return nv;
}

int sonde_engine_fetch_m20(sonde_engine_t *e, sonde_m20_frame_t *out, int32_t max, int32_t finish) {
    if (e && !e->groups.empty()) return mixed_fetch(e, SONDE_M20, out, max, 0, [finish](sonde_engine *g, sonde_m20_frame_t *o, int32_t m) { return sonde_engine_fetch_m20(g, o, m, finish); });
    if (!e || !out || max < 0 || e->cfg.sonde_type != SONDE_M20) return SONDE_E_ARG;
    if (finish) launch_framesync(e, 1);
    std::vector<FrameRec> recs;
    std::vector<float> soft;
    const int n = collect_records(e, 0, recs, &soft, max);
    if (n < 0) return n;
    e->last_soft = soft; e->last_n = n; e->soft_lazy = false;
    for (int h = 0; h < n; h++) {
        const FrameRec &r = recs[h];
        sonde_m20_frame_t &o = out[h];
        memset(&o, 0, sizeof o);
        o.nbits = mxx_bytes(e, r, 101 + 64, o.frame);
        o.channel = r.channel; o.mv = r.mv; o.mv_pos = rel_pos(e, r);
        sonde_m20_frame_finish(&o);
    }
    return n;
}

static int fetch_m10_impl(sonde_engine_t *e, sonde_m10_frame_t *out, int32_t max, int32_t finish, int lag) {
    if (!e || !out || max < 0 || e->cfg.sonde_type != SONDE_M10) return SONDE_E_ARG;
    if (finish) { launch_framesync(e, 1); lag = 0; }
    std::vector<FrameRec> recs;
    std::vector<float> soft;
    const bool on_dev = blockcodes_on_device(e);
    const int n = collect_records(e, lag, recs, on_dev ? nullptr : &soft, max);
    if (n < 0) return n;
    e->last_n = n;
    if (on_dev) {
        const unsigned start = e->read_idx - (unsigned)n;
        e->soft_lazy = true; e->soft_lazy_start = start;
        if (copy_decoded(e, e->d_m10_out, e->h_m10, start, n, 1, lag)) return SONDE_E_NOGPU;
        for (int h = 0; h < n; h++) { out[h] = e->h_m10[h]; out[h].mv_pos = rel_pos(e, recs[h]); }
        return n;
    }
    e->last_soft = soft; e->soft_lazy = false;
    if (e->m10_chk3 && e->d_soft1 && !soft.empty()) {
        const unsigned start = e->read_idx - (unsigned)n;
        std::vector<float> s1((size_t)e->nbits);
        for (int h = 0; h < n; h++) {
            const unsigned idx = (start + (unsigned)h) % (unsigned)e->max_frames;
            if (hipMemcpy(s1.data(), e->d_soft1 + (size_t)idx * e->nbits, (size_t)e->nbits * sizeof(float), hipMemcpyDeviceToHost) != hipSuccess) return SONDE_E_NOGPU;
            FrameRec &r = recs[h];
            const int nv = std::min(r.nbytes, e->nbits);
            for (int p = 0; p < nv; p++) {
                const int bit = ((double)soft[(size_t)h * e->nbits + p] + 0.25 * (double)s1[p]) >= 0.0;
                r.frame[p >> 3] = (uint8_t)((r.frame[p >> 3] & ~(1u << (p & 7))) | ((unsigned)bit << (p & 7)));
            }
        }
    }
    for (int h = 0; h < n; h++) {
        const FrameRec &r = recs[h];
        sonde_m10_frame_t &o = out[h];
        memset(&o, 0, sizeof o);
        const int nv = mxx_bytes(e, r, 101 + 20, o.frame);
        o.channel = r.channel; o.nbits = nv; o.mv = r.mv; o.mv_pos = rel_pos(e, r);
        sonde_m10_frame_finish(&o);
    }
    return n;
}

int sonde_engine_fetch_hits(sonde_engine_t *e, sonde_hit_t *out, int32_t max, int32_t finish) {
    if (!e || !e->groups.empty() || !out || max < 0 || !e->d_soft || e->cfg.sonde_type == SONDE_FRONTEND) return SONDE_E_ARG;
    if (finish) launch_framesync(e, 1);
    std::vector<FrameRec> recs;
    std::vector<float> soft;
    const int n = collect_records(e, 0, recs, &soft, max);
    if (n < 0) return n;
    e->last_soft = soft; e->last_n = n; e->soft_lazy = false;
    if (e->d_soft1) {
        const unsigned start = e->read_idx - (unsigned)n;
        e->last_soft1.resize((size_t)n * e->nbits);
        for (int i = 0; i < n; i++) {
            const unsigned idx = (start + (unsigned)i) % (unsigned)e->max_frames;
            if (hipMemcpy(e->last_soft1.data() + (size_t)i * e->nbits, e->d_soft1 + (size_t)idx * e->nbits, (size_t)e->nbits * sizeof(float), hipMemcpyDeviceToHost) != hipSuccess) return SONDE_E_NOGPU;
        }
    }
    for (int i = 0; i < n; i++) {
        const FrameRec &r = recs[i];
        out[i].channel = r.channel; out[i].mv = r.mv; out[i].mv_pos = rel_pos(e, r);
        out[i].nbits = e->cfg.sonde_type == SONDE_RS41 ? 8 * (r.nbytes - 8) : r.nbytes;
    }
    return n;
}

int sonde_engine_set_m10_chk3(sonde_engine_t *e, int32_t on) {
    if (!e || e->cfg.sonde_type != SONDE_M10 || (on && (!e->d_soft1 || e->cfg.input == SONDE_IN_AUDIO))) return SONDE_E_ARG;
    e->m10_chk3 = on != 0;
    return 0;
}

int sonde_engine_set_sync(sonde_engine_t *e, int32_t hdmax, int32_t bitofs) {
    if (!e || !e->groups.empty() || hdmax < 0 || hdmax > 64 || bitofs < -8 || bitofs > 64 || e->call > 0) return SONDE_E_ARG;
    e->hdmax = hdmax; e->bitofs = bitofs;
    return 0;
}

int sonde_engine_set_threshold(sonde_engine_t *e, float thres) {
    if (!e || !e->groups.empty() || !(thres > 0.f) || thres >= 1.f) return SONDE_E_ARG;
    e->thres = thres;
    return 0;
}

int sonde_engine_finish(sonde_engine_t *e, sonde_frame_t *out, int32_t max) {
    if (!e || !out) return SONDE_E_ARG;
    if (!e->groups.empty())
        return mixed_fetch(e, SONDE_RS41, out, max, 0, [](sonde_engine *g, sonde_frame_t *o, int32_t m) { return sonde_engine_finish(g, o, m); });
    launch_framesync(e, 1);
    return sonde_engine_fetch_frames(e, out, max);
}

int sonde_engine_finish_channel(sonde_engine_t *e, int32_t channel) {
    if (!e || channel < 0 || channel >= e->cfg.n_channels) return SONDE_E_ARG;
    if (!e->groups.empty()) { const int gi = e->grp_of_ch[(size_t)channel]; return sonde_engine_finish_channel(e->groups[(size_t)gi], e->row_of_ch[(size_t)channel] - e->groups[(size_t)gi]->front_row); }
    e->eof_ch = channel;
    launch_framesync(e, 1);
    e->eof_ch = -1;
    return 0;
}

int sonde_engine_restart_channel(sonde_engine_t *e, int32_t channel) {
    if (!e || !e->groups.empty() || channel < 0 || channel >= e->cfg.n_channels) return SONDE_E_ARG;
    const bool base = e->cfg.input == SONDE_IN_IQ;
    if ((!base && e->info.decM != 1) || e->cfg.opt_dc || e->cfg.opt_iqdc || e->cfg.pipeline || e->cfg.sonde_type == SONDE_FRONTEND) return SONDE_E_ARG;
    if (base && (e->f32_path || e->cfg.opt_nolut || e->lut_len <= 0 || e->lut_len % e->info.decM)) return SONDE_E_ARG;
    HIPCHK(hipStreamSynchronize(e->stream));
    HIPCHK(hipStreamSynchronize(e->stream_b));
    if (e->stream_e) HIPCHK(hipStreamSynchronize(e->stream_e));
    const int C = e->cfg.n_channels;
    if (base) {
        if (!e->pcs) {
            e->pcs_cnt.assign((size_t)C, e->dc_cnt); e->pcs_max.assign((size_t)C, e->dc_max);
            std::vector<uint32_t> zero((size_t)C, 0u); std::vector<int32_t> since((size_t)C, e->dc_since);
            if (dalloc(&e->d_epoch_phase, (size_t)C) || dalloc(&e->d_pcs_cnt, (size_t)C) || dalloc(&e->d_pcs_max, (size_t)C) || dalloc(&e->d_pcs_since, (size_t)C)) return SONDE_E_NOMEM;
            HIPCHK(hipMemcpy(e->d_pcs_cnt, e->pcs_cnt.data(), (size_t)C * sizeof(uint32_t), hipMemcpyHostToDevice));
            HIPCHK(hipMemcpy(e->d_pcs_max, e->pcs_max.data(), (size_t)C * sizeof(uint32_t), hipMemcpyHostToDevice));
            HIPCHK(hipMemcpy(e->d_pcs_since, since.data(), (size_t)C * sizeof(int32_t), hipMemcpyHostToDevice));
            if (e->d_etab && !e->d_dcavg_prev) return SONDE_E_ARG;
            e->pcs = true;
        }
        const uint32_t ph = (uint32_t)(e->samples_in % (uint64_t)e->lut_len), zero = 0u, m0 = e->dc_max0; const int32_t far = 1 << 20;
        HIPCHK(hipMemcpy(e->d_epoch_phase + channel, &ph, sizeof ph, hipMemcpyHostToDevice));
        HIPCHK(hipMemcpy(e->d_pcs_cnt + channel, &zero, sizeof zero, hipMemcpyHostToDevice));
        HIPCHK(hipMemcpy(e->d_pcs_max + channel, &m0, sizeof m0, hipMemcpyHostToDevice));
        HIPCHK(hipMemcpy(e->d_pcs_since + channel, &far, sizeof far, hipMemcpyHostToDevice));
        e->pcs_cnt[channel] = 0; e->pcs_max[channel] = m0;
        HIPCHK(hipMemset(e->d_dcavg + channel, 0, sizeof(float2)));
        if (e->d_dcavg_prev) HIPCHK(hipMemset(e->d_dcavg_prev + channel, 0, sizeof(float2)));
        HIPCHK(hipMemset(e->d_dcsums + 2 * (size_t)channel, 0, 2 * sizeof(long long)));
        for (int k = 0; k < 2; k++) if (e->d_ptail[k]) HIPCHK(hipMemset(e->d_ptail[k] + (size_t)channel * 64, 0, 64 * sizeof(float2)));
    }
    const size_t ring = (size_t)e->ring_len, row = (size_t)channel * ring;
    if (e->d_y)    HIPCHK(hipMemset(e->d_y + row, 0, ring * sizeof(float2)));
    if (e->d_ifiq) HIPCHK(hipMemset(e->d_ifiq + row, 0, ring * sizeof(float2)));
    if (e->d_fm)   HIPCHK(hipMemset(e->d_fm + row, 0, ring * sizeof(float)));
    if (e->d_bufs) HIPCHK(hipMemset(e->d_bufs + row, 0, ring * sizeof(float)));
    if (e->d_corr) HIPCHK(hipMemset(e->d_corr + row, 0, ring * sizeof(float)));
    if (e->d_raw)  HIPCHK(hipMemset(e->d_raw + row, 0, ring * sizeof(float)));
    if (e->epoch.empty()) {
        e->epoch.assign((size_t)C, 0u);
        if (dalloc(&e->d_epoch, (size_t)C)) return SONDE_E_NOMEM;
    }
    e->epoch[channel] = e->m_out;
    HIPCHK(hipMemcpy(e->d_epoch, e->epoch.data(), (size_t)C * sizeof(uint32_t), hipMemcpyHostToDevice));
    SyncState st; memset(&st, 0, sizeof st);
    st.s_in = e->m_out; st.mv_pos = e->m_out; st.inv = e->cfg.opt_inv ? 1u : 0u;
    HIPCHK(hipMemcpy(e->d_state + channel, &st, sizeof st, hipMemcpyHostToDevice));
    if (!e->last_frame.empty()) { memset(e->last_frame.data() + (size_t)channel * 518, 0, 518); memcpy(e->last_frame.data() + (size_t)channel * 518, kRs41HeaderBytes, 8); }
    if (!e->m10_bits.empty()) { const size_t per = e->m10_bits.size() / (size_t)C; memset(e->m10_bits.data() + (size_t)channel * per, 0, per); }
    if (e->d_m10_bits) { const size_t per = (101 + 20) * 8 + 8; HIPCHK(hipStreamSynchronize(e->stream_b)); HIPCHK(hipMemset(e->d_m10_bits + (size_t)channel * per, 0, per)); }
    return 0;
// ... 200 lines not shown
```

### radiosonde_auto_rx_amd/csrc/sonde_kernels.hip

```cpp
#include <hip/hip_runtime.h>
#include <stdint.h>
#include "sonde_dev.h"
#include "md_fast_gen.h"
#include "sonde_rs_dev.h"
#include <cstdlib>
#include <cstdio>
#include <algorithm>

typedef short  short2v __attribute__((ext_vector_type(2)));

#define WAVE 64

#define MD_ROWS   64
#define MD_NVMAX  16

struct __attribute__((packed, aligned(4))) u32x4_u { uint32_t x, y, z, w; };

typedef float float2v __attribute__((ext_vector_type(2)));

__device__ __forceinline__ float2v cmul_pk(float2v u, float2v cs) {
    float2v t, z;
    asm("s_nop 0\n\tv_pk_mul_f32 %0, %1, %2 op_sel:[1,1] op_sel_hi:[1,0] neg_lo:[0,1]" : "=&v"(t) : "v"(u), "v"(cs));
    asm("v_pk_fma_f32 %0, %1, %2, %3 op_sel_hi:[0,1,1]" : "=&v"(z) : "v"(u), "v"(cs), "v"(t));
    return z;
// ... 2055 lines not shown
        if (wcount && threadIdx.x == 0) atomicAdd(wcount, 1ull);
        __syncthreads();
        mv = *s_mv; mpos = *s_mpos;
        return *s_rc;
    }
};
__global__ __launch_bounds__(WF_THREADS) WF_WAVES_ATTR
void k_search_sync(const SearchSyncArgs a) {
    extern __shared__ __attribute__((aligned(16))) float2 smem_ss[];
    float2 *x = smem_ss;
    float2 *tws = smem_ss + SC_XN;
    __shared__ float s_rf[WF_THREADS / WAVE + 1];
    __shared__ int s_ri[WF_THREADS / WAVE];
    __shared__ int s_rc; __shared__ float s_mv; __shared__ uint32_t s_mpos;
    for (int k = threadIdx.x; k < SC_TW_LDS; k += WF_THREADS) tws[k] = a.win.tws[k];
    const SearchWinEval ev{a.win, x, tws, s_rf, s_ri, &s_rc, &s_mv, &s_mpos, a.wcount};
    framesync_body<false, WF_THREADS>(a.sync, (int)blockIdx.x, ev);
}

extern "C" int sonde_launch_mix_decimate(const MixDecArgs *a, hipStream_t s) {
    if (a->D < 1 || a->Q < 1 || a->Q > 8) return -1;
    const int rows_per_wg = 4 * (MD_ROWS * a->G - (a->Q - 1));
    const int wgs_per_ch = (a->nblocks + rows_per_wg - 1) / rows_per_wg;
    MixDecArgs b = *a; b.wgs_per_ch = wgs_per_ch;
    const dim3 grid(((a->n_ch + 7) / 8) * 8 * wgs_per_ch), blk(256);
    if (a->D > 64) {
        if (!a->wtab_g || a->DS < 1 || a->DS > 64 || a->D % a->DS) return -1;
        const size_t ldsw = (size_t)4 * MD_ROWS * ((a->DS + 3) & ~3) * sizeof(uint32_t);
#define MDW_LAUNCH(QT) do { if (a->phase_f64) hipLaunchKernelGGL((k_mix_decimate_wide<QT, true>), grid, blk, ldsw, s, b); \
                          else hipLaunchKernelGGL((k_mix_decimate_wide<QT, false>), grid, blk, ldsw, s, b); } while (0)
        switch (a->Q) {
            case 5: MDW_LAUNCH(5); break;
            case 6: MDW_LAUNCH(6); break;
            case 7: MDW_LAUNCH(7); break;
            case 8: MDW_LAUNCH(8); break;
            default: return -1;
        }
#undef MDW_LAUNCH
        return 0;
    }
    const size_t lds = (size_t)4 * (MD_ROWS * a->D + 4) * sizeof(uint32_t);
#define MD_GO(K) do { if (lds > 64 * 1024 && hipFuncSetAttribute(reinterpret_cast<const void *>(K), hipFuncAttributeMaxDynamicSharedMemorySize, (int)lds) != hipSuccess) \
                          { (void)hipGetLastError(); return -2; } \
                      hipLaunchKernelGGL(K, grid, blk, lds, s, b); } while (0)
#define MD_LAUNCH(QT) do { if (a->phase_f64) MD_GO((k_mix_decimate<QT, true, 0, 0>)); else MD_GO((k_mix_decimate<QT, false, 0, 0>)); } while (0)
    if (a->Q == 7 && a->D == 50) {
        if (a->etab && !a->phase_f64 && a->nd_base == 0.0 && a->lut_phase % 50 == 0) {
            if (a->nblocks >= 64 && a->nblocks % 2 == 0) hipLaunchKernelGGL(k_mix_decimate50, grid, blk, lds, s, b);
            else hipLaunchKernelGGL((k_mix_decimate<7, false, 50, 1>), grid, blk, lds, s, b);
        }
        else if (a->etab) return -1;
        else if (a->phase_f64 && a->dc_seg && a->nd_base == 0.0 && !a->epoch_phase && a->lut_len % 50 == 0 && a->lut_phase % 50 == 0 && a->dc_seg_blocks > 0
                 && a->nblocks >= 64 && a->nblocks % 2 == 0 && a->wtab_scaled)
            hipLaunchKernelGGL(k_mix_decimate50s, grid, blk, lds, s, b);
        else if (a->phase_f64) hipLaunchKernelGGL((k_mix_decimate<7, true, 50, 0>), grid, blk, lds, s, b);
        else hipLaunchKernelGGL((k_mix_decimate<7, false, 50, 0>), grid, blk, lds, s, b);
        return 0;
    }
    switch (a->Q) {
        case 1: MD_LAUNCH(1); break;
        case 2: MD_LAUNCH(2); break;
        case 3: MD_LAUNCH(3); break;
        case 4: MD_LAUNCH(4); break;
        case 5: MD_LAUNCH(5); break;
        case 6: MD_LAUNCH(6); break;
        case 7: MD_LAUNCH(7); break;
        default: MD_LAUNCH(8); break;
    }
#undef MD_LAUNCH
#undef MD_GO
    return 0;
}
extern "C" void sonde_launch_dc_segments(const int16_t *iq, long long ch_stride, int n_ch, int n_samples, unsigned dc_cnt0, unsigned dc_max,
                                         long long *seg_sums, long long *dc_sums, float2 *dc_avg, float2 *dc_seg, int dc_seg_n, hipStream_t s) {
    const int nseg = (int)(((unsigned long long)dc_cnt0 + (unsigned)n_samples + dc_max - 1) / dc_max);
    const int ncomplete = (int)(((unsigned long long)dc_cnt0 + (unsigned)n_samples) / dc_max);
    hipLaunchKernelGGL(k_dc_seg_sums, dim3(nseg, n_ch), dim3(256), 0, s, iq, ch_stride, n_samples, dc_cnt0, dc_max, seg_sums, nseg);
    hipLaunchKernelGGL(k_dc_seg_means, dim3((n_ch + 255) / 256), dim3(256), 0, s, n_ch, nseg, ncomplete, (float)dc_max, seg_sums, dc_sums, dc_avg, dc_seg, dc_seg_n);
}
extern "C" int sonde_launch_mix_decimate50r(const MixDecArgs *a, hipStream_t s) {
    if (a->D != 50 || a->Q != 7 || a->lut_len % 50 || a->lut_phase % 50 || !a->wtab_scaled || !a->bsum || a->bsum_stride < a->nblocks || a->dc_seg) return -1;
    MixDecArgs b = *a;
    const int H = b.Q - 1, rps = 64 * b.G - H;
    if (b.G < 1 || rps < 1) return -1;
    const int segs = (b.nblocks + rps - 1) / rps;
    b.wgs_per_ch = (segs + 3) / 4;
    const int ch8 = (b.n_ch + 7) / 8;
    const size_t lds = (size_t)4 * (64 * b.D + 4) * sizeof(uint32_t);
    static bool attr = false;
    if (!attr) { if (hipFuncSetAttribute(reinterpret_cast<const void *>(k_mix_decimate50r), hipFuncAttributeMaxDynamicSharedMemorySize, (int)lds) != hipSuccess) return -2; attr = true; }
    hipLaunchKernelGGL(k_mix_decimate50r, dim3((unsigned)(ch8 * b.wgs_per_ch * 8)), dim3(256), lds, s, b);
    return 0;
}
extern "C" void sonde_launch_dc_rows_to_segments(const int2 *bsum, long long bsum_stride, int n_ch, int nblocks, int seg_off, int seg_blocks, float maxcnt,
                                                 long long *seg_sums, long long *dc_sums, float2 *dc_avg, const float2 *dc_prev, float2 *dc_prev_out, float2 *dc_seg, int dc_seg_n, hipStream_t s) {
    const int nseg = (seg_off + nblocks + seg_blocks - 1) / seg_blocks, ncomplete = (seg_off + nblocks) / seg_blocks;
    hipLaunchKernelGGL(k_dc_rows_to_segments, dim3(nseg, n_ch), dim3(256), 0, s, bsum, bsum_stride, nblocks, seg_off, seg_blocks, seg_sums, nseg);
    hipLaunchKernelGGL(k_dc_seg_means, dim3((n_ch + 255) / 256), dim3(256), 0, s, n_ch, nseg, ncomplete, maxcnt, seg_sums, dc_sums, dc_avg, dc_seg, dc_seg_n, dc_prev, dc_prev_out);
}
extern "C" void sonde_launch_scan_dc_edges(const ScanEdgeArgs *a, hipStream_t s) {
    if (a->nseg <= 0) return;
    hipLaunchKernelGGL(k_scan_dc_edges, dim3(a->nseg, a->n_ch), dim3(64), 0, s, *a);
}
extern "C" void sonde_launch_dc_segments_f32(const float2 *x, long long ch_stride, int n_ch, int n_samples, unsigned dc_cnt0, unsigned dc_max,
                                             double *seg_sums, double *dc_sums, float2 *dc_avg, float2 *dc_seg, int dc_seg_n, hipStream_t s) {
    const int nseg = (int)(((unsigned long long)dc_cnt0 + (unsigned)n_samples + dc_max - 1) / dc_max);
    const int ncomplete = (int)(((unsigned long long)dc_cnt0 + (unsigned)n_samples) / dc_max);
    hipLaunchKernelGGL(k_dc_seg_sums_f32, dim3(nseg, n_ch), dim3(256), 0, s, x, ch_stride, n_samples, dc_cnt0, dc_max, seg_sums, nseg);
    hipLaunchKernelGGL(k_dc_seg_means_f32, dim3((n_ch + 255) / 256), dim3(256), 0, s, n_ch, nseg, ncomplete, (float)dc_max, seg_sums, dc_sums, dc_avg, dc_seg, dc_seg_n);
}
extern "C" void sonde_launch_dc_update(int n_ch, long long *sums, float2 *avg, float maxcnt, hipStream_t s) {
    hipLaunchKernelGGL(k_dc_update, dim3((n_ch + 255) / 256), dim3(256), 0, s, n_ch, sums, avg, (float2 *)nullptr, maxcnt);
}
extern "C" void sonde_launch_dc_update_keep(int n_ch, long long *sums, float2 *avg, float2 *avg_prev, float maxcnt, hipStream_t s) {
    hipLaunchKernelGGL(k_dc_update, dim3((n_ch + 255) / 256), dim3(256), 0, s, n_ch, sums, avg, avg_prev, maxcnt);
}
extern "C" void sonde_launch_dc_update_pcs(int n_ch, long long *sums, float2 *avg, float2 *avg_prev, uint32_t *cnt, uint32_t *max, uint32_t lim, int32_t *since,
                                           uint32_t n_samples, int nblocks, hipStream_t s) {
    hipLaunchKernelGGL(k_dc_update_pcs, dim3((n_ch + 255) / 256), dim3(256), 0, s, n_ch, sums, avg, avg_prev, cnt, max, lim, since, n_samples, nblocks);
}
extern "C" void sonde_launch_publish_u32(const unsigned *src, unsigned *dst_mapped, hipStream_t s) {
    hipLaunchKernelGGL(k_publish_u32, dim3(1), dim3(64), 0, s, src, dst_mapped);
}
extern "C" void sonde_launch_md_etable(const double *chan_f0, const float *wtab, int D, int Q, int P, int n_ch, float2 *etab, hipStream_t s) {
    hipLaunchKernelGGL(k_md_etable, dim3((P + 255) / 256, n_ch), dim3(256), 0, s, chan_f0, wtab, D, Q, P, etab, 0);
}
extern "C" void sonde_launch_md_etable64(const double *chan_f0, const float *wtab, int D, int Q, int P, int n_ch, float2 *etab, hipStream_t s) {
    hipLaunchKernelGGL(k_md_etable, dim3((P + 255) / 256, n_ch), dim3(256), 0, s, chan_f0, wtab, D, Q, P, etab, 1);
}
extern "C" void sonde_launch_u8_to_s16(const uint8_t *in, long long in_stride, int16_t *out, long long out_stride, int n_ch, int n_bytes, hipStream_t s) {
    int gx = (n_bytes / 4 + 255) / 256; if (gx > 1024) gx = 1024; if (gx < 1) gx = 1;
    hipLaunchKernelGGL(k_u8_to_s16, dim3(gx, n_ch), dim3(256), 0, s, in, in_stride, out, out_stride, n_bytes);
}
extern "C" void sonde_launch_mix_f32(const MixF32Args *a, hipStream_t s) {
    const int gx = (a->n + MF32_CHUNK - 1) / MF32_CHUNK;
    if (gx < 1) return;
    hipLaunchKernelGGL(k_mix_f32, dim3(gx, a->n_ch), dim3(256), 0, s, *a);
}
extern "C" void sonde_launch_decimate_f32(const DecF32Args *a, hipStream_t s) {
    if (a->nblocks <= 0) return;
    int jper = DF32_J;
    auto lds_of = [&](int j) { return (size_t)(a->D * (j - 1) + a->T) * sizeof(float2) + (size_t)a->T * sizeof(float); };
    while (jper > 8 && lds_of(jper) > 64 * 1024) jper >>= 1;
    if (lds_of(jper) > 64 * 1024) { hipLaunchKernelGGL(k_decimate_f32_global, dim3((a->nblocks + 255) / 256, a->n_ch), dim3(256), 0, s, *a); return; }
    hipLaunchKernelGGL(k_decimate_f32, dim3((a->nblocks + jper - 1) / jper, a->n_ch), dim3(DF32_J), lds_of(jper), s, *a, jper);
}
extern "C" void sonde_launch_dc_update_f64(int n_ch, double *sums, float2 *avg, float maxcnt, hipStream_t s) {
    hipLaunchKernelGGL(k_dc_update_f64, dim3((n_ch + 255) / 256), dim3(256), 0, s, n_ch, sums, avg, maxcnt);
}
extern "C" void sonde_launch_afc_rotate(const AfcRotArgs *a, hipStream_t s, int n_max) {
    int gx = (n_max + 255) / 256; if (gx > 256) gx = 256; if (gx < 1) gx = 1;
    hipLaunchKernelGGL(k_afc_rotate, dim3(gx, a->n_ch), dim3(256), 0, s, *a);
}
extern "C" void sonde_launch_fill_u32(uint32_t *p, uint32_t v, int n, hipStream_t s) {
    hipLaunchKernelGGL(k_fill_u32, dim3((n + 255) / 256), dim3(256), 0, s, p, v, n);
}
extern "C" void sonde_launch_audio_chain(const AudioChainArgs *a, hipStream_t s) {
    int gx = (a->n + 255) / 256; if (gx > 256) gx = 256; if (gx < 1) gx = 1;
    hipLaunchKernelGGL(k_audio_chain, dim3(gx, a->n_ch), dim3(256), 0, s, *a);
}
extern "C" void sonde_launch_if_chain(const IfArgs *a, hipStream_t s) {
    hipLaunchKernelGGL(k_if_chain, dim3((a->n + IF_TILE - 1) / IF_TILE, a->n_ch), dim3(IF_THREADS), if_chain_lds(*a), s, *a);
}
template <class A> static MultiArgs<A> multi_pack(const A *a, const int *rows, int n_groups) {
    MultiArgs<A> m{};
    m.n_groups = n_groups; m.row0[0] = 0;
    for (int g = 0; g < n_groups; g++) { m.g[g] = a[g]; m.row0[g + 1] = m.row0[g] + rows[g]; }
    return m;
}
static_assert(sizeof(MultiArgs<IfArgs>) <= 4096, "MultiArgs<IfArgs> exceeds the kernel argument segment");
static_assert(sizeof(MultiArgs<WinPlanArgs>) <= 4096, "MultiArgs<WinPlanArgs> exceeds the kernel argument segment");
static_assert(sizeof(MultiArgs<WinFftArgs>) <= 4096, "MultiArgs<WinFftArgs> exceeds the kernel argument segment");
static_assert(sizeof(MultiArgs<SyncArgs>) <= 4096, "MultiArgs<SyncArgs> exceeds the kernel argument segment");
extern "C" int sonde_launch_if_chain_multi(const IfArgs *a, int n_groups, hipStream_t s) {
    if (n_groups < 1 || n_groups > SONDE_MAX_GROUPS) return -1;
    size_t lds = 0; int rows[SONDE_MAX_GROUPS], n = a[0].n;
    for (int g = 0; g < n_groups; g++) {
        const size_t l = if_chain_lds(a[g]);
        if (l > lds) lds = l;
        rows[g] = a[g].n_ch;
        if (a[g].n != n) return -1;
    }
    const MultiArgs<IfArgs> m = multi_pack(a, rows, n_groups);
    hipLaunchKernelGGL(k_if_chain_multi, dim3((n + IF_TILE - 1) / IF_TILE, m.row0[n_groups]), dim3(IF_THREADS), lds, s, m);
    return 0;
}
extern "C" int sonde_launch_sync_plan_multi(const WinPlanArgs *a, int n_groups, hipStream_t s) {
    if (n_groups < 1 || n_groups > SONDE_MAX_GROUPS) return -1;
    int rows[SONDE_MAX_GROUPS];
    for (int g = 0; g < n_groups; g++) rows[g] = a[g].n_ch;
    const MultiArgs<WinPlanArgs> m = multi_pack(a, rows, n_groups);
    hipLaunchKernelGGL(k_sync_plan_multi, dim3((m.row0[n_groups] + 255) / 256), dim3(256), 0, s, m);
    return 0;
}
extern "C" int sonde_launch_sync_window_fft_multi(const WinFftArgs *a, int n_groups, hipStream_t s) {
    if (n_groups < 1 || n_groups > SONDE_MAX_GROUPS) return -1;
    long long tot = 0; int rows[SONDE_MAX_GROUPS];
    for (int g = 0; g < n_groups; g++) tot += (long long)a[g].W * a[g].n_ch;
    const long long cap = tot > 512 ? 512 : tot;
    for (int g = 0; g < n_groups; g++) { const long long w = (long long)a[g].W * a[g].n_ch; rows[g] = (int)((w * cap + tot - 1) / tot); if (rows[g] < 1) rows[g] = 1; }
    const MultiArgs<WinFftArgs> m = multi_pack(a, rows, n_groups);
    hipLaunchKernelGGL(k_sync_window_fft_multi, dim3(m.row0[n_groups]), dim3(WF_THREADS), (size_t)(SC_XN + SC_TW_LDS + 1) * sizeof(float2), s, m);
    return 0;
}
extern "C" void sonde_launch_header_corr(const CorrArgs *a, hipStream_t s) {
    if (a->ntypes > 0) {
        const int nf = (HCF_TILE + a->isps * (a->nsym - 1) + 3) & ~3, nxp = (nf + a->isps + 3 + 3) & ~3;
        const size_t lds = (size_t)(nxp + a->ntypes * nf) * sizeof(float);
        hipLaunchKernelGGL(k_header_corr_fact, dim3((a->n + HCF_TILE - 1) / HCF_TILE, a->n_ch), dim3(HCF_THREADS), lds, s, *a);
        return;
    }
    const size_t lds = (size_t)(HC_TILE + 2 * a->L + 8) * sizeof(float);
    hipLaunchKernelGGL(k_header_corr, dim3((a->n + HC_TILE - 1) / HC_TILE, a->n_ch), dim3(HC_THREADS), lds, s, *a);
}
extern "C" void sonde_launch_sync_plan(const WinPlanArgs *a, hipStream_t s) {
    hipLaunchKernelGGL(k_sync_plan, dim3((a->n_ch + 255) / 256), dim3(256), 0, s, *a);
}
extern "C" void sonde_launch_sync_window_fft(const WinFftArgs *a, hipStream_t s) {
    const size_t lds = (size_t)(SC_XN + SC_TW_LDS + 1) * sizeof(float2);
    int grid = a->W * a->n_ch;
    if (grid > 512) grid = 512;
    hipLaunchKernelGGL(k_sync_window_fft, dim3(grid), dim3(WF_THREADS), lds, s, *a);
}
#define RSK_THREADS 256
struct RsEccLds { uint8_t frame[520], exp[512], log[256], cw[2][256], part[RSK_THREADS / 64][48], scr[2][64], S[48]; int res[4]; };
__device__ __forceinline__ void rs_ecc_tables(RsEccLds &L, const uint8_t *gf_exp, const uint8_t *gf_log, int tid) {
    for (int i = tid; i < 512; i += RSK_THREADS) L.exp[i] = gf_exp[i];
    if (tid < 256) L.log[tid] = gf_log[tid];
}
__global__ __launch_bounds__(RSK_THREADS)
void k_rs41_ecc_frames(FrameRec *frames, const uint32_t *list, unsigned *count, unsigned *done, int max_frames, int level,
                       const uint8_t *gf_exp, const uint8_t *gf_log) {
    __shared__ RsEccLds L;
    __shared__ unsigned s_last;
    const int tid = threadIdx.x;
    const unsigned n = min(*count, (unsigned)max_frames);
    if (n) rs_ecc_tables(L, gf_exp, gf_log, tid);
    for (unsigned w = blockIdx.x; w < n; w += gridDim.x) {
        FrameRec *rec = frames + list[w];
        __syncthreads();
        if (rec->ecc_done != 2) continue;
        const int flen = rec->len;
        for (int i = tid; i < 518; i += RSK_THREADS) L.frame[i] = i < flen ? rec->frame[i] : 0;
        if (tid < 48) L.S[tid] = rec->synd[tid];
        __syncthreads();
        const RsGf gf{L.exp, L.log};
        const int r = rs41_ecc_wg(L.frame, level, L.cw, L.part, L.res, L.scr, L.S, gf, tid, RSK_THREADS);
        for (int i = tid; i < 518; i += RSK_THREADS) rec->frame[i] = L.frame[i];
        __threadfence();
        __syncthreads();
        if (tid == 0) { rec->ecc = r; rec->ecc_done = 1; }
    }
    __syncthreads();
    if (tid == 0) { __threadfence(); s_last = atomicAdd(done, 1u); }
    __syncthreads();
    if (s_last == gridDim.x - 1 && tid == 0) { *count = 0; *done = 0; }
}
extern "C" void sonde_launch_rs41_ecc_frames(FrameRec *frames, const uint32_t *list, unsigned *count, unsigned *done, int max_frames, int level,
                                             const uint8_t *gf_exp, const uint8_t *gf_log, int grid, hipStream_t s) {
    hipLaunchKernelGGL(k_rs41_ecc_frames, dim3(grid), dim3(RSK_THREADS), 0, s, frames, list, count, done, max_frames, level, gf_exp, gf_log);
}

__global__ __launch_bounds__(RSK_THREADS)
void k_rs41_ecc_batch(uint8_t *frames, const int32_t *flen, int level, int32_t *ecc, int32_t *codes, uint8_t *synd, const uint8_t *gf_exp, const uint8_t *gf_log, const unsigned *count) {
    __shared__ RsEccLds L;
    const int tid = threadIdx.x, f = blockIdx.x;
    if (count && (unsigned)f >= *count) return;
    rs_ecc_tables(L, gf_exp, gf_log, tid);
    for (int i = tid; i < 518; i += RSK_THREADS) L.frame[i] = i < flen[f] ? frames[(size_t)f * 518 + i] : 0;
    __syncthreads();
    const RsGf gf{L.exp, L.log};
    for (int i = tid; i < 510; i += RSK_THREADS) { const int c = i / 255, n = i % 255; L.cw[c][n] = n < 24 ? L.frame[8 + 24 * c + n] : L.frame[56 + 2 * (n - 24) + c]; }
    __syncthreads();
    rs41_syndrome_partials(L.cw, L.part, gf, tid & 63, tid >> 6, RSK_THREADS / 64);
    __syncthreads();
    if (tid < 48) { uint8_t sy = 0; for (int w = 0; w < RSK_THREADS / 64; w++) sy ^= L.part[w][tid]; L.S[tid] = sy; synd[(size_t)f * 48 + tid] = sy; }
    __syncthreads();
    const int r = rs41_ecc_wg(L.frame, level, L.cw, L.part, L.res, L.scr, (f & 1) ? L.S : (const uint8_t *)nullptr, gf, tid, RSK_THREADS);
    for (int i = tid; i < 518; i += RSK_THREADS) frames[(size_t)f * 518 + i] = L.frame[i];
    if (tid == 0) { ecc[f] = r; codes[2 * f] = L.res[0]; codes[2 * f + 1] = L.res[1]; }
}
extern "C" void sonde_launch_rs41_ecc_batch(uint8_t *frames, const int32_t *flen, int n, int level, int32_t *ecc, int32_t *codes, uint8_t *synd,
                                            const uint8_t *gf_exp, const uint8_t *gf_log, hipStream_t s) {
    hipLaunchKernelGGL(k_rs41_ecc_batch, dim3(n), dim3(RSK_THREADS), 0, s, frames, flen, level, ecc, codes, synd, gf_exp, gf_log, (const unsigned *)nullptr);
}
extern "C" void sonde_launch_rs41_ecc_batch_n(uint8_t *frames, const int32_t *flen, const unsigned *count, int cap, int level, int32_t *ecc, int32_t *codes, uint8_t *synd,
                                              const uint8_t *gf_exp, const uint8_t *gf_log, hipStream_t s) {
    hipLaunchKernelGGL(k_rs41_ecc_batch, dim3(cap), dim3(RSK_THREADS), 0, s, frames, flen, level, ecc, codes, synd, gf_exp, gf_log, count);
}

extern "C" int sonde_launch_framesync_multi(const SyncArgs *a, int n_groups, hipStream_t s) {
    if (n_groups < 1 || n_groups > SONDE_MAX_GROUPS) return -1;
    int rows[SONDE_MAX_GROUPS];
    for (int g = 0; g < n_groups; g++) { rows[g] = a[g].n_ch; if (a[g].opt_dc) return -1; }
    const MultiArgs<SyncArgs> m = multi_pack(a, rows, n_groups);
    hipLaunchKernelGGL(k_framesync_multi, dim3(m.row0[n_groups]), dim3(1024), 0, s, m);
    return 0;
}
extern "C" void sonde_launch_framesync(const SyncArgs *a, hipStream_t s) {
    if (a->opt_dc) hipLaunchKernelGGL(k_framesync<true>, dim3(a->n_ch), dim3(FS_THREADS), 0, s, *a);
    else hipLaunchKernelGGL(k_framesync<false>, dim3(a->n_ch), dim3(FS_THREADS), 0, s, *a);
}
static constexpr size_t SEARCH_SYNC_LDS = (size_t)(SC_XN + SC_TW_LDS + 1) * sizeof(float2);
extern "C" void sonde_launch_search_sync(const SearchSyncArgs *a, hipStream_t s) {
    hipLaunchKernelGGL(k_search_sync, dim3(a->sync.n_ch), dim3(WF_THREADS), SEARCH_SYNC_LDS, s, *a);
}
extern "C" int sonde_if_chain_residency(const IfArgs *a) {
    int n = 0;
    return hipOccupancyMaxActiveBlocksPerMultiprocessor(&n, k_if_chain, IF_THREADS, if_chain_lds(*a)) == hipSuccess ? n : -1;
}
extern "C" size_t sonde_if_chain_lds_bytes(int T1, int T2, int nwin, int tone_on, int fm_on, int *overlay) {
    IfArgs a{};
    a.lpiq_on = 1; a.lpiq_taps = T1; a.lpfm_on = 1; a.lpfm_taps = T2; a.nwin = nwin; a.tone_on = tone_on; a.fm_on = fm_on;
    if (overlay) *overlay = if_chain_overlay(tone_on, T2, (T2 - 1) + std::max(1, nwin - 1) + (tone_on ? IF_RUN - 1 : 0)) ? 1 : 0;
    return if_chain_lds(a);
}
extern "C" int sonde_if_chain_reserve(const IfArgs *a, int device) {
    const size_t lds = if_chain_lds(*a);
    int lds_max = 0;
    if (hipDeviceGetAttribute(&lds_max, hipDeviceAttributeMaxSharedMemoryPerBlock, device) != hipSuccess) return -2;
    if (lds > (size_t)lds_max) {
        fprintf(stderr, "libsonde_hip: the IF chain with %d IF low-pass taps, %d FM low-pass taps and a tone window of %d samples needs %zu bytes of LDS per workgroup, the device has %d\n",
                a->lpiq_on ? a->lpiq_taps : 1, a->lpfm_on ? a->lpfm_taps : 1, a->nwin, lds, lds_max);
        return -1;
    }
    if (lds > 64 * 1024) {
        if (hipFuncSetAttribute(reinterpret_cast<const void *>(k_if_chain), hipFuncAttributeMaxDynamicSharedMemorySize, lds_max) != hipSuccess) return -2;
        if (hipFuncSetAttribute(reinterpret_cast<const void *>(k_if_chain_multi), hipFuncAttributeMaxDynamicSharedMemorySize, lds_max) != hipSuccess) return -2;
    }
    return 0;
}
extern "C" int sonde_search_sync_residency(void) {
    int n = 0;
    return hipOccupancyMaxActiveBlocksPerMultiprocessor(&n, k_search_sync, WF_THREADS, SEARCH_SYNC_LDS) == hipSuccess ? n : -1;
}
```

### radiosonde_auto_rx_amd/engine.py

```python
from __future__ import annotations

import ctypes as C
import os
import subprocess

import numpy as np

_HERE = os.path.dirname(os.path.abspath(__file__))
LIB_PATH = os.environ.get("SONDE_HIP_LIB", os.path.join(_HERE, "libsonde_hip.so"))

SONDE_RS41 = 41
SONDE_DFM09 = 9
SONDE_M10 = 10
SONDE_RD94RD41 = 94
SONDE_M20 = 20
SONDE_LMS6 = 6
SONDE_RS92 = 92
SONDE_IMET54 = 54
LP_IQ, LP_FM = 1, 2
TAP_DECIM, TAP_IFIQ, TAP_FM, TAP_BUFS, TAP_CORR = range(5)
ABI_VERSION = 3


class SondeCfg(C.Structure):
    _fields_ = [(n, C.c_int32) for n in ("abi_version", "device", "n_channels", "sample_rate", "bits", "sonde_type",
                                         "opt_lp", "opt_dc", "opt_min", "lpiq_bw", "ecc_level")] + \
               [("thres", C.c_float), ("max_chunk", C.c_int32), ("max_frames", C.c_int32), ("keep_soft", C.c_int32),
                ("pipeline", C.c_int32), ("input", C.c_int32), ("audio_channels", C.c_int32), ("audio_select", C.c_int32),
                ("if_rate", C.c_int32), ("opt_iqdc", C.c_int32), ("opt_inv", C.c_int32), ("opt_nolut", C.c_int32), ("m10_noskip", C.c_int32), ("opt_auto", C.c_int32), ("if_tune", C.c_int32)]


class SondeFrame(C.Structure):
    _fields_ = [("channel", C.c_int32), ("len", C.c_int32), ("ecc", C.c_int32), ("mv_pos", C.c_uint32),
                ("mv", C.c_float), ("nbytes", C.c_int32), ("frame", C.c_uint8 * 518), ("pad", C.c_uint8 * 2)]


class SondeDfmFrame(C.Structure):
    _fields_ = [("channel", C.c_int32), ("frame_in_hit", C.c_int32), ("ecc", C.c_int32 * 3), ("mv_pos", C.c_uint32),
                ("mv", C.c_float), ("conf", C.c_uint8 * 7), ("dat1", C.c_uint8 * 13), ("dat2", C.c_uint8 * 13), ("pad", C.c_uint8 * 3),
                ("frm_count", C.c_float), ("inv", C.c_int32), ("rawbits", C.c_uint8 * 35), ("pad2", C.c_uint8)]


class SondeM10Frame(C.Structure):
    _fields_ = [("channel", C.c_int32), ("nbits", C.c_int32), ("len", C.c_int32), ("cs_ok", C.c_int32), ("cs_calc", C.c_uint32),
                ("mv_pos", C.c_uint32), ("mv", C.c_float), ("frame", C.c_uint8 * 124)]


class SondeM20Frame(C.Structure):
    _fields_ = [("channel", C.c_int32), ("nbits", C.c_int32), ("len", C.c_int32), ("cs_ok", C.c_int32), ("cs_calc", C.c_uint32),
                ("blk_ok", C.c_int32), ("fw", C.c_int32), ("mv_pos", C.c_uint32), ("mv", C.c_float), ("frame", C.c_uint8 * 172)]


class SondeHit(C.Structure):
    _fields_ = [("channel", C.c_int32), ("nbits", C.c_int32), ("mv_pos", C.c_uint32), ("mv", C.c_float)]


class SondeGeneric(C.Structure):
    _fields_ = [("header", C.c_char * 68), ("baud", C.c_float), ("bt", C.c_float), ("h", C.c_float), ("symlen", C.c_int32), ("symhd", C.c_int32),
                ("hdmax", C.c_int32), ("bitofs", C.c_int32), ("nbits", C.c_int32), ("skip_bits", C.c_int32), ("l_win", C.c_float),
                ("lpiq_bw", C.c_int32), ("lpfm_bw", C.c_int32), ("slice_baud", C.c_float), ("reserved", C.c_int32 * 3)]


class SondeGroup(C.Structure):
    _fields_ = [("sonde_type", C.c_int32), ("ecc_level", C.c_int32), ("lpiq_bw", C.c_int32), ("opt_inv", C.c_int32), ("opt_auto", C.c_int32),
                ("m10_noskip", C.c_int32), ("thres", C.c_float), ("reserved", C.c_int32)]


class SondeInfo(C.Structure):
    _fields_ = [(n, C.c_int32) for n in ("if_sr", "decM", "dectaps", "lut_len", "lpiq_taps", "lpfm_taps",
                                         "L", "M", "K", "N", "delay")] + \
               [("sps", C.c_float), ("ring_len", C.c_int32), ("reserved", C.c_int32 * 3)]


def build_library(force: bool = False) -> str:
    src = os.path.join(_HERE, "csrc")
    if force and os.path.exists(LIB_PATH):
        os.remove(LIB_PATH)
    subprocess.check_call(["make", "-s", "-j8", "-C", src])
    return LIB_PATH


_lib = None


def lib() -> C.CDLL:
    global _lib
    if _lib is None:
        if not os.path.exists(LIB_PATH):
            raise RuntimeError(f"{LIB_PATH} missing: run `python -c 'import __graft_entry__ as g; g.build()'` "
                               "(the engine has no CPU fallback)")
        L = C.CDLL(LIB_PATH)
        L.sonde_strerror.restype = C.c_char_p
        L.sonde_engine_stream.restype = C.c_void_p
        L.sonde_engine_create.argtypes = [C.POINTER(SondeCfg), C.POINTER(C.c_double), C.POINTER(C.c_void_p)]
        L.sonde_engine_process_device.argtypes = [C.c_void_p, C.c_void_p, C.c_int64, C.c_int32]
        L.sonde_engine_process_host.argtypes = [C.c_void_p, C.c_void_p, C.c_int64, C.c_int32]
        L.sonde_engine_fetch_frames.argtypes = [C.c_void_p, C.POINTER(SondeFrame), C.c_int32]
        L.sonde_engine_fetch_frames_lagged.argtypes = [C.c_void_p, C.POINTER(SondeFrame), C.c_int32, C.c_int32]
        L.sonde_engine_finish.argtypes = [C.c_void_p, C.POINTER(SondeFrame), C.c_int32]
        L.sonde_engine_fetch_soft.argtypes = [C.c_void_p, C.c_void_p, C.c_int32]
        L.sonde_engine_fetch_dfm.argtypes = [C.c_void_p, C.POINTER(SondeDfmFrame), C.c_int32, C.c_int32]
        L.sonde_dfm_rawline.argtypes = [C.POINTER(SondeDfmFrame), C.c_int, C.c_char_p, C.c_size_t]
        L.sonde_engine_create_generic.argtypes = [C.POINTER(SondeCfg), C.POINTER(C.c_double), C.POINTER(SondeGeneric), C.POINTER(C.c_void_p)]
        L.sonde_engine_fetch_hits.argtypes = [C.c_void_p, C.POINTER(SondeHit), C.c_int32, C.c_int32]
        L.sonde_engine_set_threshold.argtypes = [C.c_void_p, C.c_float]
        L.sonde_engine_fetch_m10.argtypes = [C.c_void_p, C.POINTER(SondeM10Frame), C.c_int32, C.c_int32]
        L.sonde_engine_fetch_m10_lagged.argtypes = [C.c_void_p, C.POINTER(SondeM10Frame), C.c_int32, C.c_int32]
        L.sonde_engine_fetch_dfm_lagged.argtypes = [C.c_void_p, C.POINTER(SondeDfmFrame), C.c_int32, C.c_int32]
        L.sonde_engine_create_mixed.argtypes = [C.POINTER(SondeCfg), C.POINTER(C.c_double), C.POINTER(SondeGroup), C.c_int32, C.POINTER(C.c_int32), C.POINTER(C.c_void_p)]
        L.sonde_engine_group_info.argtypes = [C.c_void_p, C.c_int32, C.POINTER(C.c_int32), C.POINTER(SondeInfo)]
        L.sonde_engine_fetch_m20.argtypes = [C.c_void_p, C.POINTER(SondeM20Frame), C.c_int32, C.c_int32]
        L.sonde_m10_rawline.argtypes = [C.POINTER(SondeM10Frame), C.c_int, C.c_char_p, C.c_size_t]
        L.sonde_m20_rawline.argtypes = [C.POINTER(SondeM20Frame), C.c_int, C.c_char_p, C.c_size_t]
        L.sonde_engine_read_tap.argtypes = [C.c_void_p, C.c_int32, C.c_int32, C.c_int64, C.c_int32, C.c_void_p]
        L.sonde_engine_sync.argtypes = [C.c_void_p]
        L.sonde_engine_samples_to_dc_boundary.argtypes = [C.c_void_p]
        L.sonde_engine_samples_to_dc_boundary.restype = C.c_int64
        L.sonde_engine_destroy.argtypes = [C.c_void_p]
        L.sonde_engine_info.argtypes = [C.c_void_p, C.POINTER(SondeInfo)]
        L.sonde_engine_profile.argtypes = [C.c_void_p, C.c_int]
        L.sonde_engine_kernel_ms.argtypes = [C.c_void_p, C.c_char_p, C.POINTER(C.c_double), C.POINTER(C.c_int64)]
        L.sonde_engine_stream.argtypes = [C.c_void_p]
        L.sonde_rs41_rawline.argtypes = [C.POINTER(SondeFrame), C.c_char_p, C.c_size_t]
        L.sonde_engine_host_ecc_frames.argtypes = [C.c_void_p]
        L.sonde_engine_host_ecc_frames.restype = C.c_longlong
        L.sonde_engine_set_device_ecc.argtypes = [C.c_void_p, C.c_int32]
        L.sonde_engine_set_search_rounds.argtypes = [C.c_void_p, C.c_int32]
        L.sonde_engine_count_windows.argtypes = [C.c_void_p, C.c_int32, C.c_void_p]
        L.sonde_engine_read_sync_state.argtypes = [C.c_void_p, C.c_void_p, C.c_int32]
        L.sonde_rs41_ecc_device.argtypes = [C.c_void_p, C.c_void_p, C.c_int32, C.c_int32, C.c_void_p, C.c_void_p, C.c_void_p]
        _lib = L
    return _lib


def rs41_ecc_device(frames: np.ndarray, flen, level: int = 2):
    fr = np.ascontiguousarray(frames, dtype=np.uint8).reshape(-1, 518).copy()
    n = fr.shape[0]
    fl = np.ascontiguousarray(np.broadcast_to(np.asarray(flen, dtype=np.int32), (n,)))
    ecc, codes, synd = np.zeros(n, np.int32), np.zeros((n, 2), np.int32), np.zeros((n, 48), np.uint8)
    _chk(lib().sonde_rs41_ecc_device(fr.ctypes.data, fl.ctypes.data, n, level, ecc.ctypes.data, codes.ctypes.data, synd.ctypes.data))
    return fr, ecc, codes, synd


class SondeError(RuntimeError):
    pass


def snap_fq(fq: float, sr: int) -> float:
    return int(round(fq * sr / 16.0)) * 16 / sr


def _chk(rc: int) -> int:
    if rc < 0:
        raise SondeError(f"libsonde_hip: {lib().sonde_strerror(rc).decode()} ({rc})")
    return rc


class Engine:

    def __init__(self, fq, sample_rate: int, *, device: int = 0, lp_iq: bool = True, lp_fm: bool = False,
                 ecc: int = 2, thres: float = 0.0, max_chunk: int | None = None, max_frames: int = 0,
                 keep_soft: bool = False, opt_min: bool = False, lpiq_bw: int = 0, opt_dc: bool = False,
                 sonde: str = "rs41", pipeline: bool = False, audio: bool = False, audio_channels: int = 1, audio_select: int = 0,
                 if_rate: int = 0, bits: int = 16, iq_mode: int = 5, iqdc: bool = False, inv: bool = False, auto: bool = False, nolut: bool = False,
                 generic: dict | None = None, if_tune: bool = False):
        fq = np.atleast_1d(np.asarray(fq, dtype=np.float64))
        self.n_channels = len(fq)
        self.sample_rate = sample_rate
        self.sonde = sonde
        self.ecc = ecc
        self._per_sample = audio_channels if audio else 2
        self._dtype = {8: np.uint8, 32: np.float32}.get(bits, np.int16)
        cfg = SondeCfg(ABI_VERSION, device, self.n_channels, sample_rate, bits, {"rs41": SONDE_RS41, "dfm": SONDE_DFM09, "m10": 10, "m20": 20, "frontend": 0, "generic": 99}[sonde],
                       (LP_IQ if lp_iq else 0) | (LP_FM if lp_fm else 0), int(opt_dc), int(opt_min), lpiq_bw, ecc,
                       thres, max_chunk or sample_rate, max_frames, int(keep_soft), int(pipeline),
                       1 if audio else {5: 0, 1: 2, 2: 3, 3: 4}[iq_mode], audio_channels, audio_select, if_rate, int(iqdc), int(inv), int(nolut), 0, int(auto), int(if_tune))
        h = C.c_void_p()
        if sonde == "generic":
            g = SondeGeneric(**{k: (v.encode() if k == "header" else v) for k, v in (generic or {}).items()})
            cfg.keep_soft = 1
            _chk(lib().sonde_engine_create_generic(C.byref(cfg), fq.ctypes.data_as(C.POINTER(C.c_double)), C.byref(g), C.byref(h)))
        else:
            _chk(lib().sonde_engine_create(C.byref(cfg), fq.ctypes.data_as(C.POINTER(C.c_double)), C.byref(h)))
        self._h = h
        info = SondeInfo()
        _chk(lib().sonde_engine_info(h, C.byref(info)))
        self.info = {n: getattr(info, n) for n, _ in SondeInfo._fields_ if n != "reserved"}
        self.nbits = 4080 if sonde == "rs41" else generic["nbits"] if sonde == "generic" else {"m10": 968, "m20": 1320}.get(sonde, 2224)
        self._max_frames = max_frames or 4 * self.n_channels

    def close(self):
        if getattr(self, "_h", None):
            lib().sonde_engine_destroy(self._h)
            self._h = None

    __del__ = close

    def process_host(self, iq: np.ndarray, n_samples: int | None = None, shared: bool = False):
        if shared:
            iq = np.ascontiguousarray(iq, dtype=self._dtype).reshape(-1)
            n = iq.shape[0] // self._per_sample
            _chk(lib().sonde_engine_process_host(self._h, iq.ctypes.data_as(C.c_void_p), 0, n_samples or n))
            return
        iq = np.ascontiguousarray(iq, dtype=self._dtype).reshape(self.n_channels, -1)
        stride = iq.shape[1] // (self._per_sample)
        _chk(lib().sonde_engine_process_host(self._h, iq.ctypes.data_as(C.c_void_p), stride, n_samples or stride))

    def process_device(self, ptr: int, ch_stride: int, n_samples: int):
        _chk(lib().sonde_engine_process_device(self._h, C.c_void_p(ptr), ch_stride, n_samples))

    def finish_channel(self, ch: int):
        _chk(lib().sonde_engine_finish_channel(self._h, ch))

    def restart_channel(self, ch: int):
        _chk(lib().sonde_engine_restart_channel(self._h, ch))

    def tune_channel(self, ch: int, fq: float):
        lib().sonde_engine_tune_channel.argtypes = [C.c_void_p, C.c_int32, C.c_double]
        _chk(lib().sonde_engine_tune_channel(self._h, ch, float(fq)))

    def samples_to_dc_boundary(self) -> int:
        return int(lib().sonde_engine_samples_to_dc_boundary(self._h))

    def sync(self):
        _chk(lib().sonde_engine_sync(self._h))

    def set_summary(self, device_ptr: int, channel_base: int = 0):
        _chk(lib().sonde_engine_set_summary(self._h, C.c_void_p(device_ptr), channel_base))

    def set_summary_snapshots(self, device_ptr: int) -> int:
        return _chk(lib().sonde_engine_set_summary_snapshots(self._h, C.c_void_p(device_ptr)))

    def overflowed(self) -> bool:
        return bool(_chk(lib().sonde_engine_overflowed(self._h)))

    def host_ecc_frames(self) -> int:
        return int(lib().sonde_engine_host_ecc_frames(self._h))

    def set_device_ecc(self, on: bool):
        _chk(lib().sonde_engine_set_device_ecc(self._h, 1 if on else 0))

    def set_search_rounds(self, on: bool):
        _chk(lib().sonde_engine_set_search_rounds(self._h, 1 if on else 0))

    def count_windows(self, on: bool = True):
        out = np.zeros(3, dtype=np.int64)
        _chk(lib().sonde_engine_count_windows(self._h, 1 if on else 0, out.ctypes.data))
        return {"round0": int(out[0]), "rounds": int(out[1]), "search_sync": int(out[2])}

    def tail_residency(self):
        out = np.zeros(2, dtype=np.int32)
        f = lib().sonde_engine_tail_residency
        f.argtypes = [C.c_void_p, C.c_void_p]
        _chk(f(self._h, out.ctypes.data))
        return {"if_chain": int(out[0]), "search_sync": int(out[1])}

    def sync_state(self) -> np.ndarray:
        out = np.zeros((self.n_channels, 8), dtype=np.uint32)
        _chk(lib().sonde_engine_read_sync_state(self._h, out.ctypes.data, self.n_channels))
        return out

    def fetch_frames(self, max_frames: int | None = None, with_soft: bool = False, finish: bool = False):
        n = max_frames or self._max_frames
        buf = (SondeFrame * n)()
        fn = lib().sonde_engine_finish if finish else lib().sonde_engine_fetch_frames
        k = _chk(fn(self._h, buf, n))
        frames = []
        line = C.create_string_buffer(1200)
        for i in range(k):
            f = buf[i]
            ll = lib().sonde_rs41_rawline(C.byref(f), line, 1200)
            frames.append(dict(channel=f.channel, len=f.len, ecc=f.ecc, mv=f.mv, mv_pos=f.mv_pos, nbytes=f.nbytes,
                               frame=bytes(f.frame), line=line.raw[:ll].decode()))
        if with_soft:
            soft = np.zeros((max(k, 1), self.nbits), np.float32)
            _chk(lib().sonde_engine_fetch_soft(self._h, soft.ctypes.data_as(C.c_void_p), k))
            for i in range(k):
                frames[i]["soft"] = soft[i].copy()
        return frames

    def fetch_dfm(self, finish: bool = False, with_soft: bool = False):
        n = 8 * self._max_frames
        buf = (SondeDfmFrame * n)()
        k = _chk(lib().sonde_engine_fetch_dfm(self._h, buf, n, int(finish)))
        line = C.create_string_buffer(128)
        frames = []
        for i in range(k):
            f = buf[i]
            ll = lib().sonde_dfm_rawline(C.byref(f), self.ecc, line, 128)
            frames.append(dict(channel=f.channel, frame_in_hit=f.frame_in_hit, ecc=list(f.ecc), mv=f.mv, mv_pos=f.mv_pos,
                               conf=bytes(f.conf), dat1=bytes(f.dat1), dat2=bytes(f.dat2), frm_count=f.frm_count, inv=f.inv,
                               line=line.raw[:ll].decode()))
        if with_soft:
            soft = np.zeros((self._max_frames, self.nbits), np.float32)
            nh = _chk(lib().sonde_engine_fetch_soft(self._h, soft.ctypes.data_as(C.c_void_p), self._max_frames))
            return frames, soft[:nh]
        return frames

    def fetch_dfm_raw(self, finish: bool = False, lag: int = 0):
        n = 8 * self._max_frames
        if getattr(self, "_dfmbuf", None) is None:
            self._dfmbuf = (SondeDfmFrame * n)()
        if lag and not finish:
            return self._dfmbuf, _chk(lib().sonde_engine_fetch_dfm_lagged(self._h, self._dfmbuf, n, lag))
        return self._dfmbuf, _chk(lib().sonde_engine_fetch_dfm(self._h, self._dfmbuf, n, int(finish)))

    def fetch_m10_raw(self, finish: bool = False, lag: int = 0):
        n = 4 * self._max_frames
        if getattr(self, "_m10buf", None) is None:
            self._m10buf = (SondeM10Frame * n)()
        if lag and not finish:
            return self._m10buf, _chk(lib().sonde_engine_fetch_m10_lagged(self._h, self._m10buf, n, lag))
        return self._m10buf, _chk(lib().sonde_engine_fetch_m10(self._h, self._m10buf, n, int(finish)))

    def fetch_hits(self, finish: bool = False):
        n = self._max_frames
        buf = (SondeHit * n)()
        k = _chk(lib().sonde_engine_fetch_hits(self._h, buf, n, int(finish)))
        soft = np.zeros((max(k, 1), self.nbits), np.float32)
        if k:
            _chk(lib().sonde_engine_fetch_soft(self._h, soft.ctypes.data_as(C.c_void_p), k))
        return [dict(channel=buf[i].channel, nbits=buf[i].nbits, mv=buf[i].mv, mv_pos=buf[i].mv_pos, soft=soft[i, :buf[i].nbits].copy()) for i in range(k)]

    def fetch_mxx(self, finish: bool = False, verbose: int = 1):
        m20 = self.sonde == "m20"
        n = 4 * self._max_frames
        buf = ((SondeM20Frame if m20 else SondeM10Frame) * n)()
        L = lib()
        k = _chk((L.sonde_engine_fetch_m20 if m20 else L.sonde_engine_fetch_m10)(self._h, buf, n, int(finish)))
        line = C.create_string_buffer(420)
        frames = []
        for i in range(k):
            f = buf[i]
            ll = (L.sonde_m20_rawline if m20 else L.sonde_m10_rawline)(C.byref(f), verbose, line, 420)
            d = dict(channel=f.channel, nbits=f.nbits, len=f.len, cs_ok=f.cs_ok, cs_calc=f.cs_calc, mv=f.mv, mv_pos=f.mv_pos,
                     frame=bytes(f.frame), line=line.raw[:max(ll, 0)].decode())
            if m20:
                d.update(blk_ok=f.blk_ok, fw=f.fw)
            frames.append(d)
        return frames

    FRAME_DTYPE = np.dtype([("channel", "<i4"), ("len", "<i4"), ("ecc", "<i4"), ("mv_pos", "<u4"), ("mv", "<f4"),
                            ("nbytes", "<i4"), ("frame", "u1", (518,)), ("pad", "u1", (2,))])

    def fetch_frames_np(self, max_frames: int | None = None, lag: int = 0) -> np.ndarray:
        n = max_frames or self._max_frames
        if getattr(self, "_fbuf", None) is None or len(self._fbuf) < n:
            self._fbuf = np.zeros(n, self.FRAME_DTYPE)
        k = _chk(lib().sonde_engine_fetch_frames_lagged(self._h, self._fbuf.ctypes.data_as(C.POINTER(SondeFrame)), n, lag))
        return self._fbuf[:k].copy()

    def read_tap(self, channel: int, tap: int, first: int, count: int) -> np.ndarray:
        width = 2 if tap in (TAP_DECIM, TAP_IFIQ) else 1
        out = np.zeros((count, width), np.float32)
        _chk(lib().sonde_engine_read_tap(self._h, channel, tap, first, count, out.ctypes.data_as(C.c_void_p)))
        return out if width == 2 else out[:, 0]

    def profile(self, enable: bool | int = True):
        _chk(lib().sonde_engine_profile(self._h, 2 if enable is True else int(enable)))

    def kernel_ms(self, name: str):
        ms, n = C.c_double(), C.c_int64()
        _chk(lib().sonde_engine_kernel_ms(self._h, name.encode(), C.byref(ms), C.byref(n)))
        return ms.value, n.value

    @property
    def stream(self) -> int:
        return lib().sonde_engine_stream(self._h)


_KIND = {"rs41": SONDE_RS41, "dfm": SONDE_DFM09, "m10": SONDE_M10, "m20": SONDE_M20}
SONDE_MIXED = 100


class MixedEngine(Engine):

    def __init__(self, fq, kinds, sample_rate: int, *, device: int = 0, lp_iq: bool = True, ecc: dict | None = None, thres: dict | None = None,
                 max_chunk: int | None = None, max_frames: int = 0, opt_min: bool = False, bits: int = 16, pipeline: bool = True):
        fq = np.atleast_1d(np.asarray(fq, dtype=np.float64))
        kinds = list(kinds)
        assert len(kinds) == len(fq)
        ecc = {"rs41": 2, "dfm": 1, "m10": 0, "m20": 0, **(ecc or {})}
        thres = thres or {}
        self.kinds = kinds
        self.group_kinds = list(dict.fromkeys(kinds))
        self.n_channels = len(fq)
        self.sample_rate = sample_rate
        self.sonde = "mixed"
        self.ecc = ecc["dfm"]
        self._ecc = ecc
        self._per_sample = 2
        self._dtype = {8: np.uint8}.get(bits, np.int16)
        cfg = SondeCfg(ABI_VERSION, device, self.n_channels, sample_rate, bits, SONDE_MIXED, LP_IQ if lp_iq else 0, 0, int(opt_min), 0, 0,
                       0.0, max_chunk or sample_rate, max_frames, 0, int(pipeline), 0, 1, 0, 0, 0, 0, 0, 0, 0, 0)
        groups = (SondeGroup * len(self.group_kinds))()
        for i, k in enumerate(self.group_kinds):
            groups[i] = SondeGroup(_KIND[k], ecc[k], 0, 0, 0, 0, float(thres.get(k, 0.0)), 0)
        gof = np.asarray([self.group_kinds.index(k) for k in kinds], dtype=np.int32)
        h = C.c_void_p()
        _chk(lib().sonde_engine_create_mixed(C.byref(cfg), fq.ctypes.data_as(C.POINTER(C.c_double)), groups, len(self.group_kinds),
                                              gof.ctypes.data_as(C.POINTER(C.c_int32)), C.byref(h)))
        self._h = h
        info = SondeInfo()
        _chk(lib().sonde_engine_info(h, C.byref(info)))
        self.info = {n: getattr(info, n) for n, _ in SondeInfo._fields_ if n != "reserved"}
        self.nbits = 4080
        self._max_frames = max_frames or 4 * self.n_channels

    def group_info(self, channel: int):
        t, info = C.c_int32(), SondeInfo()
        _chk(lib().sonde_engine_group_info(self._h, channel, C.byref(t), C.byref(info)))
        return t.value, {n: getattr(info, n) for n, _ in SondeInfo._fields_ if n != "reserved"}

    def fetch_mxx(self, finish: bool = False, verbose: int = 1, m20: bool = False):
        self.sonde = "m20" if m20 else "m10"
        try:
            return Engine.fetch_mxx(self, finish=finish, verbose=verbose)
        finally:
            self.sonde = "mixed"
```

Before: 981,600 Msamples/s.

## Overlap IF chain with search-sync on a high-priority stream, optionally

Adds an optional tail-overlap mode. The IF chain for the next chunk runs on a separate high-priority stream while the search-sync kernel for the previous chunk finishes, with events chaining the dependencies two calls back. In this mode search-sync is launched with enough dynamic LDS to force one workgroup per CU, so the other CU slots stay free for the IF chain. The ring buffer is enlarged to cover the extra reach-back, and ring sizing and host design are split out into reusable helpers. The mode is enabled only with pipeline>=2, or with pipeline=1 plus an environment variable.

```diff
diff --git a/include/sonde_hip.h b/include/sonde_hip.h
--- a/include/sonde_hip.h
+++ b/include/sonde_hip.h
@@ -157,6 +157,8 @@
 long long sonde_engine_host_ecc_frames(sonde_engine_t *e);
 int  sonde_engine_set_device_ecc(sonde_engine_t *e, int32_t on);
 int  sonde_engine_set_search_rounds(sonde_engine_t *e, int32_t on);
+int  sonde_engine_set_tail_overlap(sonde_engine_t *e, int32_t on);
+int32_t sonde_engine_ring_need(const sonde_cfg_t *cfg, const sonde_generic_t *gen, sonde_info_t *info, int32_t *frame_samples);
 int  sonde_engine_count_windows(sonde_engine_t *e, int32_t on, int64_t *out);
 int  sonde_engine_tail_residency(sonde_engine_t *e, int32_t *out);
 int  sonde_engine_read_sync_state(sonde_engine_t *e, uint32_t *out, int32_t max_channels);
diff --git a/radiosonde_auto_rx_amd/csrc/sonde_dev.h b/radiosonde_auto_rx_amd/csrc/sonde_dev.h
--- a/radiosonde_auto_rx_amd/csrc/sonde_dev.h
+++ b/radiosonde_auto_rx_amd/csrc/sonde_dev.h
@@ -202,9 +202,10 @@
 void sonde_launch_sync_plan(const WinPlanArgs *a, hipStream_t s);
 void sonde_launch_sync_window_fft(const WinFftArgs *a, hipStream_t s);
 void sonde_launch_framesync(const SyncArgs *a, hipStream_t s);
-void sonde_launch_search_sync(const SearchSyncArgs *a, hipStream_t s);
+void sonde_launch_search_sync(const SearchSyncArgs *a, int one_per_cu, hipStream_t s);
+int  sonde_search_sync_reserve(int device);
 int  sonde_if_chain_residency(const IfArgs *a);
-int  sonde_search_sync_residency(void);
+int  sonde_search_sync_residency(int one_per_cu);
 size_t sonde_if_chain_lds_bytes(int T1, int T2, int nwin, int tone_on, int fm_on, int *overlay);
 int  sonde_if_chain_reserve(const IfArgs *a, int device);
 }
diff --git a/radiosonde_auto_rx_amd/csrc/sonde_engine.cpp b/radiosonde_auto_rx_amd/csrc/sonde_engine.cpp
--- a/radiosonde_auto_rx_amd/csrc/sonde_engine.cpp
+++ b/radiosonde_auto_rx_amd/csrc/sonde_engine.cpp
@@ -1,6 +1,7 @@
 #include "../../include/sonde_hip.h"
 #include "sonde_dev.h"
 #include "sonde_host.h"
+#include "sonde_ring.h"
 #include "sonde_scan_dev.h"
 #include <algorithm>
 #include <cmath>
@@ -30,6 +31,9 @@
     std::vector<sonde_dfm_frame_t> h_dfm; std::vector<sonde_m10_frame_t> h_m10; bool soft_lazy = false; unsigned soft_lazy_start = 0;
     uint32_t *d_ecc_list = nullptr; unsigned *d_ecc_cnt = nullptr;
     hipEvent_t ev_a[4] = {}, ev_b[4] = {}, ev_if[4] = {};
+    hipStream_t stream_if = nullptr;
+    hipEvent_t ev_ss[4] = {};
+    bool overlap_ok = false, tail_overlap = false;
     unsigned *h_count = nullptr;
     unsigned *h_count_dev = nullptr;
     FrameRec *h_recs = nullptr;
@@ -172,7 +176,7 @@
 }
 static void launch_framesync(sonde_engine *e, int eof) { launch_framesync_impl(e, eof); launch_blockcodes(e); if (eof) e->eof_pending = true; }
 static void sync_round(sonde_engine *e, int W);
-static void launch_search_sync(sonde_engine *e);
+static void launch_search_sync(sonde_engine *e, bool one_per_cu);
 
 static bool blockcodes_on_device(const sonde_engine *e) {
     return e->dev_ecc && e->d_soft && e->d_blk_done && ((e->cfg.sonde_type == SONDE_DFM09 && e->d_dfm_out) || (e->cfg.sonde_type == SONDE_M10 && e->d_m10_out));
@@ -260,8 +264,8 @@
 }
 
 static IfArgs fill_if(sonde_engine *e, int n_if, uint32_t m_first);
-static int create_impl(const sonde_cfg_t *cfg, const double *fq, const sonde_generic_t *gen, const CreateLink *lk, sonde_engine_t **out) {
-    if (!cfg || !fq || !out || cfg->abi_version != SONDE_ABI_VERSION) return SONDE_E_ARG;
+static int design_host(sonde_engine *e, const sonde_cfg_t *cfg, const sonde_generic_t *gen, const CreateLink *lk, std::string &header) {
+    if (!cfg || cfg->abi_version != SONDE_ABI_VERSION) return SONDE_E_ARG;
     if (cfg->sonde_type == SONDE_GENERIC && !gen) return SONDE_E_ARG;
     float baud_override = 0.f;
     if (gen && cfg->sonde_type != SONDE_GENERIC) { if (!(gen->baud > 0.f)) return SONDE_E_ARG; baud_override = gen->baud; gen = nullptr; }
@@ -280,19 +284,10 @@
     if (cfg->if_tune && (cfg->input < SONDE_IN_IFIQ0 || cfg->bits != 32 || cfg->opt_dc)) return SONDE_E_ARG;
     if (cfg->sonde_type == SONDE_FRONTEND && cfg->input != SONDE_IN_IQ) return SONDE_E_ARG;
     if (cfg->input < SONDE_IN_IQ || cfg->input > SONDE_IN_IFIQ3) return SONDE_E_ARG;
-    int ndev = 0;
-    if (hipGetDeviceCount(&ndev) != hipSuccess || ndev < 1 || cfg->device >= ndev) {
-        fprintf(stderr, "libsonde_hip: no usable HIP device (the engine has no CPU fallback)\n");
-        return SONDE_E_NOGPU;
-    }
-    HIPCHK(hipSetDevice(cfg->device));
-    sonde_engine *e = new sonde_engine();
     e->cfg = *cfg;
-    const int C = cfg->n_channels;
-    const bool is_group = lk && lk->is_group, front_only = lk && lk->front_only;
-    e->is_group = is_group; e->front_only = front_only;
-
-    std::string header;
+    cfg = &e->cfg;
+    e->is_group = lk && lk->is_group; e->front_only = lk && lk->front_only;
+
     int lpiq_def, lpfm_bw;
     int skip_last = -1;
     if (gen) {
@@ -334,7 +329,7 @@
     e->sps /= (float)D;
     e->Q = (T + D - 1) / D;
     const bool wide = e->Q > 8;
-    if (D > 1024 || (wide && (audio || ifiq || lk || cfg->input != SONDE_IN_IQ))) { delete e; return SONDE_E_ARG; }
+    if (D > 1024 || (wide && (audio || ifiq || lk || cfg->input != SONDE_IN_IQ))) return SONDE_E_ARG;
     e->f32_path = cfg->bits == 32 || wide; e->conv32 = wide && cfg->bits != 32;
     if ((cfg->opt_lp & SONDE_LP_IQ) && !audio) {
         float f_lp = (float)(24e3 / (float)sr / 2.0);
@@ -367,21 +362,51 @@
         uint32_t q0, q1; double mid; bit_window(last, e->symlen - 1, e->symlen, e->sps, q0, q1, mid); e->frame_samples = q1;
     }
 
+    e->overlap_ok = cfg->pipeline >= 2 && !lk && !audio && cfg->sonde_type != SONDE_FRONTEND && !cfg->opt_dc && M == 8192 && K + L <= M;
+    if (cfg->max_chunk < 1) return SONDE_E_ARG;
+    RingNeed rn{};
+    rn.max_if = (cfg->max_chunk + D - 1) / D; rn.frame_samples = (int32_t)e->frame_samples; rn.M = M; rn.L = L; rn.delay = delay;
+    rn.pipeline = cfg->pipeline != 0; rn.tail_overlap = e->overlap_ok;
+    int ring = ring_need(rn);
+    if (ring < 1) return SONDE_E_ARG;
+    if (lk && ring < lk->min_ring) ring = lk->min_ring;
+    e->ring_len = ring;
+    e->max_frames = cfg->max_frames > 0 ? cfg->max_frames : 4 * cfg->n_channels;
+
+    sonde_info_t &I = e->info;
+    I.if_sr = sr; I.decM = D; I.dectaps = (D == 1) ? 0 : T; I.lpiq_taps = (int)e->w_iq.size(); I.lpfm_taps = (int)e->w_fm.size();
+    I.L = L; I.M = M; I.K = K; I.N = M; I.delay = delay; I.sps = e->sps_design; I.ring_len = ring;
+    return 0;
+}
+
+static int create_impl(const sonde_cfg_t *cfg, const double *fq, const sonde_generic_t *gen, const CreateLink *lk, sonde_engine_t **out) {
+    if (!cfg || !fq || !out) return SONDE_E_ARG;
+    sonde_engine *e = new sonde_engine();
+    std::string header;
+    sonde_cfg_t cfg_env = *cfg;
+    if (cfg_env.pipeline == 1 && !lk && getenv("SONDE_TAIL_OVERLAP") != nullptr) cfg_env.pipeline = 2;
+    { const int rc = design_host(e, &cfg_env, gen, lk, header); if (rc) { delete e; return rc; } }
+    cfg = &e->cfg;
+    setenv("GPU_MAX_HW_QUEUES", "8", 0);
+    int ndev = 0;
+    if (hipGetDeviceCount(&ndev) != hipSuccess || ndev < 1 || cfg->device >= ndev) {
+        fprintf(stderr, "libsonde_hip: no usable HIP device (the engine has no CPU fallback)\n");
+        delete e;
+        return SONDE_E_NOGPU;
+    }
+    HIPCHK(hipSetDevice(cfg->device));
+    const int C = cfg->n_channels;
+    const bool is_group = e->is_group, front_only = e->front_only;
+    const bool audio = cfg->input == SONDE_IN_AUDIO, ifiq = cfg->input >= SONDE_IN_IFIQ0;
+    const int D = e->dec.decM, sr = e->dec.if_sr, T = (int)e->dec.taps.size(), L = (int)e->match.size(), M = e->info.M, K = e->info.K, ring = e->ring_len;
+    const bool wide = e->Q > 8;
+    sonde_info_t &I = e->info;
+
     if (!audio && !front_only) {
         const IfArgs ia = fill_if(e, 0, 0);
         const int rc = sonde_if_chain_reserve(&ia, cfg->device);
         if (rc) { delete e; return rc == -1 ? SONDE_E_ARG : SONDE_E_NOGPU; }
     }
-
-    const int max_if = (cfg->max_chunk + D - 1) / D;
-    int ring = 1; while (ring < max_if + (int)e->frame_samples + 2 * M + 4096 || ring < 4 * M || (cfg->pipeline && ring < 2 * max_if + 4096)) ring <<= 1;
-    if (lk && ring < lk->min_ring) ring = lk->min_ring;
-    e->ring_len = ring;
-    e->max_frames = cfg->max_frames > 0 ? cfg->max_frames : 4 * C;
-
-    sonde_info_t &I = e->info;
-    I.if_sr = sr; I.decM = D; I.dectaps = (D == 1) ? 0 : T; I.lpiq_taps = (int)e->w_iq.size(); I.lpfm_taps = (int)e->w_fm.size();
-    I.L = L; I.M = M; I.K = K; I.N = M; I.delay = delay; I.sps = e->sps_design; I.ring_len = ring;
 
     if (wide) e->wtab.assign((size_t)std::max(64, D) * 8, 0.f);
     else {
@@ -556,6 +581,14 @@
         else HIPCHK(hipStreamCreateWithFlags(&e->stream_b, hipStreamNonBlocking));
     }
     else e->stream_b = e->stream;
+    if (e->d_win && !lk && sonde_search_sync_reserve(cfg->device)) { sonde_engine_destroy(e); return SONDE_E_NOGPU; }
+    if (e->overlap_ok && e->d_win && e->stream_b != e->stream) {
+        int lo = 0, hi = 0;
+        if (hipDeviceGetStreamPriorityRange(&lo, &hi) == hipSuccess && hi != lo) HIPCHK(hipStreamCreateWithPriority(&e->stream_if, hipStreamNonBlocking, hi));
+        else HIPCHK(hipStreamCreateWithFlags(&e->stream_if, hipStreamNonBlocking));
+        for (int i = 0; i < 4; i++) HIPCHK(hipEventCreateWithFlags(&e->ev_ss[i], hipEventDisableTiming));
+        e->tail_overlap = true;
+    }
     HIPCHK(hipStreamCreateWithFlags(&e->stream_c, hipStreamNonBlocking));
     if (cfg->sonde_type == SONDE_RS41 && cfg->ecc_level >= 1 && cfg->ecc_level <= 2 && getenv("SONDE_ECC_INLINE") == nullptr) {
         int lo = 0, hi = 0;
@@ -588,6 +621,7 @@
     if (e->stream) hipStreamSynchronize(e->stream);
     if (e->stream_b) hipStreamSynchronize(e->stream_b);
     if (e->stream_e) hipStreamSynchronize(e->stream_e);
+    if (e->stream_if) hipStreamSynchronize(e->stream_if);
     prof_collect(e);
     if (e->d_wfprof) {
         unsigned long long h[32] = {0};
@@ -611,6 +645,8 @@
     if (e->stream_b && e->stream_b != e->stream && !e->borrowed_b) hipStreamDestroy(e->stream_b);
     if (e->stream_c) hipStreamDestroy(e->stream_c);
     if (e->stream_e) hipStreamDestroy(e->stream_e);
+    if (e->stream_if) hipStreamDestroy(e->stream_if);
+    for (int i = 0; i < 4; i++) if (e->ev_ss[i]) hipEventDestroy(e->ev_ss[i]);
     if (e->ev_s) hipEventDestroy(e->ev_s);
     hipFree(e->d_dfm_out); hipFree(e->d_m10_out); hipFree(e->d_blk_done); hipFree(e->d_m10_bits);
     hipFree(e->d_ecc_list); hipFree(e->d_ecc_cnt);
@@ -823,7 +859,10 @@
     const bool fe = e->cfg.sonde_type == SONDE_FRONTEND;
     IfArgs b = fill_if(e, n_if, m_first);
     const int slot = (int)(e->call & 3);
-    if (e->stream_b != fs) hipStreamWaitEvent(e->stream_b, front_done, 0);
+    const bool ovl = e->tail_overlap && e->stream_if && !fe && e->d_win && !e->search_rounds && !e->cfg.opt_dc && e->cfg.input != SONDE_IN_AUDIO;
+    hipStream_t si = ovl ? e->stream_if : e->stream_b;
+    if (si != fs) hipStreamWaitEvent(si, front_done, 0);
+    if (ovl && e->call >= 2) hipStreamWaitEvent(si, e->ev_ss[(e->call - 2) & 3], 0);
     CorrArgs c{};
     c.bufs = e->d_bufs; c.corr = e->d_corr; c.match = e->d_match; c.n_ch = C; c.ring_len = e->ring_len; c.n = n_if; c.L = e->info.L; c.m0 = m_first;
     c.state = e->d_state; c.delay = e->info.delay; c.frame_samples = e->frame_samples;
@@ -848,10 +887,12 @@
         }
         if (e->stream_b != fs) hipEventRecord(e->ev_if[slot], e->stream_b);
     } else {
-        if (e->cfg.input != SONDE_IN_AUDIO) { prof_begin(e, "if_chain", e->stream_b); sonde_launch_if_chain(&b, e->stream_b); prof_end(e, e->stream_b); }
-        if (e->stream_b != fs) hipEventRecord(e->ev_if[slot], e->stream_b);
+        if (e->cfg.input != SONDE_IN_AUDIO) { prof_begin(e, "if_chain", si); sonde_launch_if_chain(&b, si); prof_end(e, si); }
+        if (si != fs) hipEventRecord(e->ev_if[slot], si);
+        if (ovl) hipStreamWaitEvent(e->stream_b, e->ev_if[slot], 0);
         if (!fe && e->d_win && !e->search_rounds) {
-            launch_search_sync(e);
+            launch_search_sync(e, ovl);
+            if (e->stream_if) hipEventRecord(e->ev_ss[slot], e->stream_b);
         } else if (!fe && e->d_win) {
             const int rounds = sync_rounds_of(e, n_if);
             for (int round = 0; round < rounds; round++) {
@@ -987,12 +1028,12 @@
     const SyncArgs s = fill_sync(e, eof);
     prof_begin(e, "framesync", e->stream_b); sonde_launch_framesync(&s, e->stream_b); prof_end(e, e->stream_b);
 }
-static void launch_search_sync(sonde_engine *e) {
+static void launch_search_sync(sonde_engine *e, bool one_per_cu) {
     SearchSyncArgs a{};
     a.sync = fill_sync(e, 0); a.sync.win = nullptr; a.sync.win_W = 0;
     fill_winfft(e, a.win);
     a.wcount = e->count_windows ? e->d_wcount : nullptr;
-    prof_begin(e, "framesync", e->stream_b); sonde_launch_search_sync(&a, e->stream_b); prof_end(e, e->stream_b);
+    prof_begin(e, "framesync", e->stream_b); sonde_launch_search_sync(&a, one_per_cu ? 1 : 0, e->stream_b); prof_end(e, e->stream_b);
     launch_blockcodes(e);
 }
 
@@ -1020,6 +1061,7 @@
     HIPCHK(hipStreamSynchronize(e->stream));
     HIPCHK(hipStreamSynchronize(e->stream_b));
     if (e->stream_e) HIPCHK(hipStreamSynchronize(e->stream_e));
+    if (e->stream_if) HIPCHK(hipStreamSynchronize(e->stream_if));
     prof_collect(e);
     return 0;
 }
@@ -1083,6 +1125,26 @@
     e->search_rounds = on != 0;
     return 0;
 }
+int sonde_engine_set_tail_overlap(sonde_engine_t *e, int32_t on) {
+    if (!e) return SONDE_E_ARG;
+    if (!e->stream_if) return 0;
+    if ((on != 0) != e->tail_overlap) {
+        const int rc = sonde_engine_sync(e);
+        if (rc) return rc;
+        e->tail_overlap = on != 0;
+    }
+    return e->tail_overlap ? 1 : 0;
+}
+int32_t sonde_engine_ring_need(const sonde_cfg_t *cfg, const sonde_generic_t *gen, sonde_info_t *info, int32_t *frame_samples) {
+    sonde_engine *e = new sonde_engine();
+    std::string header;
+    const int rc = design_host(e, cfg, gen, nullptr, header);
+    const int32_t ring = rc ? rc : e->ring_len;
+    if (!rc && info) *info = e->info;
+    if (!rc && frame_samples) *frame_samples = (int32_t)e->frame_samples;
+    delete e;
+    return ring;
+}
 int sonde_engine_count_windows(sonde_engine_t *e, int32_t on, int64_t *out) {
     if (!e || !e->groups.empty()) return SONDE_E_ARG;
     if (on && !e->d_wcount && e->d_win && dalloc(&e->d_wcount, 1)) return SONDE_E_NOMEM;
@@ -1099,7 +1161,7 @@
     if (!e || !out || !e->groups.empty()) return SONDE_E_ARG;
     const IfArgs b = fill_if(e, 0, 0);
     out[0] = e->cfg.input != SONDE_IN_AUDIO ? sonde_if_chain_residency(&b) : 0;
-    out[1] = (e->cfg.sonde_type != SONDE_FRONTEND && e->d_win && !e->cfg.opt_dc) ? sonde_search_sync_residency() : 0;
+    out[1] = (e->cfg.sonde_type != SONDE_FRONTEND && e->d_win && !e->cfg.opt_dc) ? sonde_search_sync_residency(e->tail_overlap && !e->search_rounds ? 1 : 0) : 0;
     return (out[0] < 0 || out[1] < 0) ? SONDE_E_NOGPU : 0;
 }
 int sonde_engine_read_sync_state(sonde_engine_t *e, uint32_t *out, int32_t max_channels) {
diff --git a/radiosonde_auto_rx_amd/csrc/sonde_kernels.hip b/radiosonde_auto_rx_amd/csrc/sonde_kernels.hip
--- a/radiosonde_auto_rx_amd/csrc/sonde_kernels.hip
+++ b/radiosonde_auto_rx_amd/csrc/sonde_kernels.hip
@@ -2381,8 +2381,20 @@
     else hipLaunchKernelGGL(k_framesync<false>, dim3(a->n_ch), dim3(FS_THREADS), 0, s, *a);
 }
 static constexpr size_t SEARCH_SYNC_LDS = (size_t)(SC_XN + SC_TW_LDS + 1) * sizeof(float2);
-extern "C" void sonde_launch_search_sync(const SearchSyncArgs *a, hipStream_t s) {
-    hipLaunchKernelGGL(k_search_sync, dim3(a->sync.n_ch), dim3(WF_THREADS), SEARCH_SYNC_LDS, s, *a);
+static constexpr size_t SEARCH_SYNC_LDS_ONE = 80 * 1024 + 64;
+static_assert(SEARCH_SYNC_LDS_ONE >= SEARCH_SYNC_LDS && 2 * SEARCH_SYNC_LDS_ONE > 160 * 1024, "one workgroup per CU: more than half the CU's LDS, and the layout fits");
+#ifndef SEARCH_SYNC_ONE_PER_CU
+#define SEARCH_SYNC_ONE_PER_CU 0
+#endif
+static inline size_t search_sync_lds(int one_per_cu) { return (one_per_cu || SEARCH_SYNC_ONE_PER_CU) ? SEARCH_SYNC_LDS_ONE : SEARCH_SYNC_LDS; }
+extern "C" void sonde_launch_search_sync(const SearchSyncArgs *a, int one_per_cu, hipStream_t s) {
+    hipLaunchKernelGGL(k_search_sync, dim3(a->sync.n_ch), dim3(WF_THREADS), search_sync_lds(one_per_cu), s, *a);
+}
+extern "C" int sonde_search_sync_reserve(int device) {
+    (void)device;
+    const hipError_t rc = hipFuncSetAttribute(reinterpret_cast<const void *>(k_search_sync), hipFuncAttributeMaxDynamicSharedMemorySize, (int)SEARCH_SYNC_LDS_ONE);
+    if (rc != hipSuccess) { fprintf(stderr, "libsonde_hip: k_search_sync may not have %zu bytes of dynamic LDS: %s\n", SEARCH_SYNC_LDS_ONE, hipGetErrorString(rc)); return -2; }
+    return 0;
 }
 extern "C" int sonde_if_chain_residency(const IfArgs *a) {
     int n = 0;
@@ -2409,7 +2421,7 @@
     }
     return 0;
 }
-extern "C" int sonde_search_sync_residency(void) {
+extern "C" int sonde_search_sync_residency(int one_per_cu) {
     int n = 0;
-    return hipOccupancyMaxActiveBlocksPerMultiprocessor(&n, k_search_sync, WF_THREADS, SEARCH_SYNC_LDS) == hipSuccess ? n : -1;
-}
+    return hipOccupancyMaxActiveBlocksPerMultiprocessor(&n, k_search_sync, WF_THREADS, search_sync_lds(one_per_cu)) == hipSuccess ? n : -1;
+}
diff --git a/radiosonde_auto_rx_amd/csrc/sonde_ring.h b/radiosonde_auto_rx_amd/csrc/sonde_ring.h
--- /dev/null
+++ b/radiosonde_auto_rx_amd/csrc/sonde_ring.h
@@ -0,0 +1,31 @@
+#pragma once
+#include <cstdint>
+
+namespace sonde {
+
+struct RingNeed {
+    int32_t max_if;
+    int32_t frame_samples;
+    int32_t M, L, delay;
+    bool pipeline;
+    bool tail_overlap;
+};
+
+inline int64_t ring_reach_back(const RingNeed &r) { return (int64_t)r.frame_samples + r.M + r.L + r.delay; }
+
+inline int32_t ring_pow2(int64_t need) {
+    int64_t p = 1;
+    while (p < need && p < ((int64_t)1 << 30)) p <<= 1;
+    return p >= need ? (int32_t)p : 0;
+}
+
+inline int32_t ring_need(const RingNeed &r) {
+    if (r.max_if < 1 || r.frame_samples < 0 || r.M < 1 || r.L < 0 || r.delay < 0) return 0;
+    int64_t need = (int64_t)r.max_if + r.frame_samples + 2 * (int64_t)r.M + 4096;
+    if (need < 4 * (int64_t)r.M) need = 4 * (int64_t)r.M;
+    if (r.pipeline && need < 2 * (int64_t)r.max_if + 4096) need = 2 * (int64_t)r.max_if + 4096;
+    if (r.tail_overlap && need < ring_reach_back(r) + 2 * (int64_t)r.max_if) need = ring_reach_back(r) + 2 * (int64_t)r.max_if;
+    return ring_pow2(need);
+}
+
+}
diff --git a/radiosonde_auto_rx_amd/engine.py b/radiosonde_auto_rx_amd/engine.py
--- a/radiosonde_auto_rx_amd/engine.py
+++ b/radiosonde_auto_rx_amd/engine.py
@@ -161,7 +161,7 @@
     def __init__(self, fq, sample_rate: int, *, device: int = 0, lp_iq: bool = True, lp_fm: bool = False,
                  ecc: int = 2, thres: float = 0.0, max_chunk: int | None = None, max_frames: int = 0,
                  keep_soft: bool = False, opt_min: bool = False, lpiq_bw: int = 0, opt_dc: bool = False,
-                 sonde: str = "rs41", pipeline: bool = False, audio: bool = False, audio_channels: int = 1, audio_select: int = 0,
+                 sonde: str = "rs41", pipeline: bool | int = False, audio: bool = False, audio_channels: int = 1, audio_select: int = 0,
                  if_rate: int = 0, bits: int = 16, iq_mode: int = 5, iqdc: bool = False, inv: bool = False, auto: bool = False, nolut: bool = False,
                  generic: dict | None = None, if_tune: bool = False):
         fq = np.atleast_1d(np.asarray(fq, dtype=np.float64))
@@ -242,6 +242,11 @@
 
     def set_search_rounds(self, on: bool):
         _chk(lib().sonde_engine_set_search_rounds(self._h, 1 if on else 0))
+
+    def set_tail_overlap(self, on: bool) -> bool:
+        f = lib().sonde_engine_set_tail_overlap
+        f.argtypes = [C.c_void_p, C.c_int32]
+        return bool(_chk(f(self._h, 1 if on else 0)))
 
     def count_windows(self, on: bool = True):
         out = np.zeros(3, dtype=np.int64)
```

New measurement: 946,600 Msamples/s. 0.964x the previous value.
